# uzh-rpg/dagr

Hardware: NVIDIA H100
Metric: Mevents/sec (higher is better)
Workload: dtype f32

## Files before the change

dagr_b200/_lib.py:

```python
from __future__ import annotations

import ctypes as C
import os
from pathlib import Path

import torch

_PKG = Path(__file__).resolve().parent
_LIB_PATH = Path(os.environ["DAGR_B200_LIB"]) if os.environ.get("DAGR_B200_LIB") else _PKG / "libdagr_b200.so"
_lib = None

ELL = 16
KU = 15
TABW = 16
L1_TC_WFRAG_FLOATS = 8192

p = C.c_void_p
i32 = C.c_int32
i64 = C.c_int64
f32 = C.c_float


class Geom(C.Structure):
    _fields_ = [("W", i32), ("H", i32), ("B", i32), ("T", i32),
                ("r", i32), ("ncell", i32),
                ("dt_us", i32), ("K", i32), ("Q", i32),
                ("nx1", i32), ("ny1", i32),
                ("CW", i32), ("CH", i32), ("CP", i32),
                ("NK", i32),
                ("xkey", p), ("ykey", p), ("spiral", p), ("posx0", p), ("posy0", p), ("vx0", p), ("vy0", p), ("tabx", p), ("taby", p)]


class Grid(C.Structure):
    _fields_ = [("nx", i32), ("ny", i32), ("B", i32), ("W", i32), ("H", i32),
                ("posxr", p), ("posyr", p)]


class EventWs(C.Structure):
    _fields_ = [(k, i64) for k in ("key", "tmp", "count", "blocksums", "start", "perm", "ti", "xyb", "feat_s", "nbr", "off", "cellmask",
                                   "xa", "wl_hdr", "wl_ids", "x1")]


class PoolWs(C.Structure):
    _fields_ = [(k, i64) for k in ("acc", "possum", "ptmax", "pcnt", "pmask")]


class L1AParams(C.Structure):
    _fields_ = [("w", f32 * (KU * 3 * 16)), ("root", f32 * (3 * 16)),
                ("scale", f32 * 16), ("shift", f32 * 16), ("relu", i32)]


class L1ImgParams(C.Structure):
    _fields_ = [("w", f32 * (KU * 24 * 16)), ("root", f32 * (24 * 16)), ("skip", f32 * (24 * 16)),
                ("scale", f32 * 16), ("shift", f32 * 16), ("sscale", f32 * 16), ("sshift", f32 * 16), ("relu", i32)]


class L1BParams(C.Structure):
    _fields_ = [("w", f32 * (KU * 16 * 16)), ("root", f32 * (16 * 16)), ("skip", f32 * (3 * 16)),
                ("scale", f32 * 16), ("shift", f32 * 16), ("sscale", f32 * 16), ("sshift", f32 * 16),
                ("relu", i32), ("pool_mean", i32), ("xs", i32 * 3), ("ys", i32 * 5), ("den_x", f32), ("den_y", f32)]


_SIGS = {
    "dagr_abi_version": (C.c_int, []),
    "dagr_last_error": (C.c_char_p, []),
    "dagr_scan_blocks": (i64, [i64]),
    "dagr_check_config": (C.c_int, [C.POINTER(Geom), i64, C.c_int, C.c_int, C.c_char_p]),
    "dagr_event_workspace_bytes": (C.c_int, [C.POINTER(Geom), i64, C.POINTER(EventWs)]),
    "dagr_pool_workspace_bytes": (C.c_int, [i64, C.c_int, C.POINTER(PoolWs)]),
    "dagr_downsample_events": (C.c_int, [p, p, p, i64, C.c_int, C.c_int, C.c_int, C.c_int, p, p, p, p, p, p, p, p, p]),
    "dagr_compact_events": (C.c_int, [p, i64, p, p, p, p, C.c_int, C.c_int, p, p, p, p, p, p, p, p, p]),
    "dagr_ingest_events": (C.c_int, [p, p, p, p, i64, C.c_int, C.c_int, C.c_int, C.c_int, i64, C.c_int, p, p, p, p, p, p, p, p, p]),
    "dagr_denormalize_pos": (C.c_int, [p, i64, C.c_int, C.c_int, C.c_int, p, p]),
    "dagr_prepare_events": (C.c_int, [p, p, p, C.c_int, i64, C.c_int, C.c_int, C.c_int, p, p, p, p]),
    "dagr_graph_sort": (C.c_int, [C.POINTER(Geom), p, p, p, i64, p, p, p, p, p, p, p, p, p, p, p]),
    "dagr_graph_sort_ring": (C.c_int, [C.POINTER(Geom), p, p, p, i64, p, p, p, p, p, p, p, p, p, p, p, p]),
    "dagr_stream_push": (C.c_int, [p, p, p, p, p, i64, C.c_int, C.c_int, p]),
    "dagr_stream_push_multi": (C.c_int, [p, p, p, p, p, i64, C.c_int, C.c_int, p]),
    "dagr_graph_sort_rings": (C.c_int, [C.POINTER(Geom), p, p, p, i64, C.c_int, p, p, p, p, p, p, p, p, p, p, p, p]),
    "dagr_graph_search": (C.c_int, [C.POINTER(Geom), i64, p, p, p, p, p, p, p]),
    "dagr_l1_build": (C.c_int, [C.POINTER(Geom), i64, p, p, p, p, p, C.POINTER(L1AParams), p, C.c_int, p, p, p, p, p, p, C.c_int, p]),
    "dagr_xa_permute": (C.c_int, [i64, p, C.c_int, p, p, C.c_int, p]),
    "dagr_l1_x0_image": (C.c_int, [C.POINTER(Geom), i64, p, p, p, C.c_int, C.c_int, p, p]),
    "dagr_l1_x0_image_live": (C.c_int, [C.POINTER(Geom), i64, p, p, p, p, C.c_int, C.c_int, p, p]),
    "dagr_l1_x0_image_planes": (C.c_int, [C.POINTER(Geom), i64, p, p, p, p, C.c_int, C.c_int, C.c_int, p, C.c_int, p, p]),
    "dagr_l1_conv_a_image": (C.c_int, [C.POINTER(Geom), i64, p, p, p, p, p, p, C.POINTER(L1ImgParams), p, p, p, p, C.c_int, p]),
    "dagr_voxel_sample_max": (C.c_int, [C.POINTER(Geom), i64, p, p, p, C.c_int, C.c_int, C.c_int, p, C.c_int, C.c_int, C.c_int, p]),
    "dagr_voxel_sample_max_planes": (C.c_int, [C.POINTER(Geom), i64, p, p, p, C.c_int, C.c_int, C.c_int, C.c_int, p, C.c_int, p, C.c_int,
                                               C.c_int, C.c_int, p]),
    "dagr_graph_export": (C.c_int, [C.POINTER(Geom), i64, p, p, p, p, p, p, p, p, i64, p]),
    "dagr_l1_conv_a": (C.c_int, [C.POINTER(Geom), i64, p, p, p, p, p, C.POINTER(L1AParams), p, p]),
    "dagr_l1_conv_b_pool": (C.c_int, [C.POINTER(Geom), i64, p, p, p, p, p, p, C.POINTER(L1BParams), p, p, p]),
    "dagr_l1_conv_b_pool_voxel": (C.c_int, [C.POINTER(Geom), i64, p, p, p, p, p, p, p, p, C.POINTER(L1BParams), p, C.c_int, p, p, p, p, p, p, p, C.c_int, p, p, C.c_int, p]),
    "dagr_l1_tc_weights": (C.c_int, [p, p, C.c_int, p]),
    "dagr_l1_conv_b_pool_voxel_tc": (C.c_int, [C.POINTER(Geom), i64, p, p, p, p, p, p, p, C.POINTER(L1BParams), p, p, C.c_int, p, p, p, p, p, p, p, C.c_int, p, p, C.c_int, p]),
    "dagr_l1_conv_a_image_tc": (C.c_int, [C.POINTER(Geom), i64, p, p, p, p, p, p, C.POINTER(L1ImgParams), p, p, p, p, p, C.c_int, p]),
    "dagr_l1_conv_a_image_inc": (C.c_int, [C.POINTER(Geom), i64, p, p, p, p, p, p, p, C.POINTER(L1ImgParams), p, C.c_int, p, p, p, p,
                                           C.c_int, p]),
    "dagr_voxel_sample_max_inc": (C.c_int, [C.POINTER(Geom), i64, p, p, p, p, C.c_int, C.c_int, C.c_int, C.c_int, p, p, C.c_int, C.c_int,
                                            C.c_int, p]),
    "dagr_pool1_finalize": (C.c_int, [C.POINTER(Geom), i64, p, p, p, p, C.c_int, p, p, p, p, p, p]),
    "dagr_grid_cat_pos": (C.c_int, [C.POINTER(Grid), p, p, p, C.c_int, p, p]),
    "dagr_grid_conv": (C.c_int, [C.POINTER(Grid), p, p, p, p, C.c_int, C.c_int, C.c_int, p, p, p, p, p, p, C.c_int, f32, f32, p, p]),
    "dagr_grid_linear_bn": (C.c_int, [i64, p, p, C.c_int, C.c_int, p, p, p, p, p]),
    "dagr_grid_pool": (C.c_int, [C.POINTER(Grid), C.POINTER(Grid), p, p, p, p, p, p, p, p, C.c_int, C.c_int,
                                 p, p, p, p, p, p, p, p]),
    "dagr_grid_pool_finalize": (C.c_int, [C.POINTER(Grid), C.c_int, C.c_int, p, p, p, p, p, p, p, p, p, p]),
    "dagr_grid_temporal_filter": (C.c_int, [C.POINTER(Grid), p, p, p, p]),
    "dagr_grid_to_dense": (C.c_int, [C.POINTER(Grid), p, p, C.c_int, C.c_int, p, p, p]),
    "dagr_head_decode": (C.c_int, [p, p, p, C.c_int, C.c_int, C.c_int, C.c_int, C.c_int, C.c_int, C.c_int, p, p]),
    "dagr_head_finish": (C.c_int, [C.POINTER(Grid), p, p, C.c_int, p, C.c_int, p, p, p, C.c_int, C.c_int, C.c_int, C.c_int, p, p]),
    "dagr_head_finish_planes": (C.c_int, [C.POINTER(Grid), p, p, C.c_int, p, C.c_int, p, p, p, C.c_int, C.c_int, C.c_int, C.c_int,
                                          C.c_int, p, C.c_int, p, p]),
    "dagr_postprocess_nms": (C.c_int, [p, C.c_int, C.c_int, C.c_int, f32, f32, C.c_int, C.c_int, C.c_int, p, p, p]),
    "dagr_sample_features": (C.c_int, [p, C.c_int, C.c_int, C.c_int, C.c_int, p, p, p, i64, C.c_int, C.c_int, p,
                                       C.c_int, C.c_int, p]),
    "dagr_sample_features_planes": (C.c_int, [p, C.c_int, p, C.c_int, C.c_int, C.c_int, C.c_int, p, p, p, i64, C.c_int, C.c_int, p,
                                              C.c_int, C.c_int, p]),
    "dagr_masked_lin": (C.c_int, [p, i64, p, p, p, p, C.c_int, C.c_int, C.c_int, p]),
    "dagr_masked_inplace_bn": (C.c_int, [p, i64, p, p, p, p, p, p, C.c_int, f32, p]),
    "dagr_masked_isdiff": (C.c_int, [p, i64, p, p, C.c_int, f32, f32, p]),
}

EXPORTS = tuple(_SIGS.keys())


def lib_path() -> Path:
    return _LIB_PATH


def load():
    global _lib
    if _lib is not None:
        return _lib
    if not os.environ.get("DAGR_B200_LIB"):
        from . import build as _build
        if _build.needs_build():
            try:
                _build.build(force=True)
            except Exception as e:
                if not _LIB_PATH.exists():
                    raise RuntimeError(f"dagr_b200: could not build the CUDA extension: {e}") from e
                import warnings
                warnings.warn(f"dagr_b200: libdagr_b200.so is older than its sources and could not be rebuilt ({e})")
    if not _LIB_PATH.exists():
        raise RuntimeError(f"dagr_b200: CUDA extension {_LIB_PATH} is missing and could not be built; "
                           "there is no CPU fallback")
    lib = C.CDLL(str(_LIB_PATH))
    for name, (res, args) in _SIGS.items():
        fn = getattr(lib, name)
        fn.restype = res
        fn.argtypes = args
    if lib.dagr_abi_version() != 2:
        raise RuntimeError("dagr_b200: ABI version mismatch between python host and libdagr_b200.so")
    _lib = lib
    return lib


def check(code: int, what: str = ""):
    if code != 0:
        msg = load().dagr_last_error()
        raise RuntimeError(f"dagr_b200 {what} failed ({code}): {msg.decode() if msg else ''}")


def ptr(t):
    if t is None:
        return None
    return C.c_void_p(t.data_ptr())


def stream_ptr():
    return C.c_void_p(torch.cuda.current_stream().cuda_stream)


def require_cuda(t: torch.Tensor, name: str):
    if not t.is_cuda:
        raise RuntimeError(f"dagr_b200: `{name}` must be a CUDA tensor (no CPU fallback on the product path)")
    if not t.is_contiguous():
        raise RuntimeError(f"dagr_b200: `{name}` must be contiguous")
```

dagr_b200/csrc/build_l1.cu:

```cuda
#include <type_traits>
#include "common.cuh"

#define BL_THREADS 160
#define BL_CAP 2048
#define BL_CAP_LEAN 1536
#define BL_THREADS_BIG 512
#define BL_CAP_BIG 12288
#define BL_NB 8

struct BLTile {
    int X0, Y0, TW, TH;
    int run_start[3], run_off[3], run_len[3];
    int smin, smax;
    int unsorted;
    int bucketed;
    int maxidx;
};

__host__ __device__ __forceinline__ size_t bl_acc_offset(const dagr_geom_t &g, int cap)
{
    const size_t TW = g.CW + 2 * g.r, TH = g.CH + 2 * g.r, TP = TW * TH;
    const size_t o = (size_t)(2 * g.r + 1) * 32 + (size_t)cap * 12 + TP * 4 + (TW + TH) * 4 + TP * BL_NB * 2 + (size_t)g.ncell * 4;
    return (o + 15) / 16 * 16;
}
static size_t bl_smem_bytes(const dagr_geom_t *g, int cap, int threads)
{
    const size_t TW = g->CW + 2 * g->r, TH = g->CH + 2 * g->r;
    const size_t occ = (size_t)BL_NB * (TW + TH) * 4, order = (size_t)threads * 2;
    return bl_acc_offset(*g, cap) + (size_t)(DAGR_ELL - 1) * threads * 4 + (occ > order ? occ : order) + 16;
}

#define BL_R1 96

template <bool STAGED, int THREADS>
__device__ __forceinline__ void bl_probe(const dagr_geom_t &g, int64_t N, int p, bool active, const int2 me, int eb, int tidx0,
                                         int c_end, const uint32_t *s_pbin, const uint16_t *s_rng, const short *s_sp2,
                                         const int2 *s_ti, const int2 *__restrict__ ti, uint32_t *s_acc,
                                         int32_t *__restrict__ nbr, uint16_t *__restrict__ off, int &n_out)
{
    const int kmax = g.K - 1;
    int n = active ? 0 : kmax;
    for (int c0 = 0; c0 < c_end; c0 += 4) {
        if (__all_sync(0xffffffffu, n >= kmax)) break;
        uint32_t rg[4]; int pix[4];
#pragma unroll
        for (int u = 0; u < 4; u++) {
            const int c = min(c0 + u, g.ncell - 1);
            pix[u] = tidx0 + s_sp2[c];
        }
#pragma unroll
        for (int u = 0; u < 4; u++) rg[u] = s_rng[pix[u] * BL_NB + eb];
#pragma unroll
        for (int u = 0; u < 4; u++) {
            const int c = c0 + u;
            const int lo = rg[u] & 0xff, hi = rg[u] >> 8;
            const int cnt = (c < c_end && n < kmax) ? hi - lo : 0;
            if (!__any_sync(0xffffffffu, cnt > 0)) continue;
            const int base = (int)(s_pbin[pix[u]] >> 8);
            const int vmax = __reduce_max_sync(0xffffffffu, cnt);
            for (int k = 0; k < vmax; k++) {
                if (k < cnt && n < kmax) {
                    const int j = base + hi - 1 - k;
                    const int2 o = STAGED ? s_ti[j] : __ldg(ti + j);
                    if (o.y < me.y && me.x - o.x <= g.dt_us) {
                        if (STAGED) s_acc[n * THREADS + threadIdx.x] = ((uint32_t)j << 10) | (uint32_t)c;
                        else { nbr[(int64_t)n * N + p] = j; off[(int64_t)n * N + p] = (uint16_t)c; }
                        n++;
                    }
                }
            }
        }
    }
    n_out = active ? n : 0;
}


#ifndef BL_SHARED_ADDR
#define BL_SHARED_ADDR 1
#endif
__device__ __forceinline__ uint32_t bl_sa(const void *p) { return (uint32_t)__cvta_generic_to_shared(p); }
__device__ __forceinline__ uint32_t bl_lds32(uint32_t a) { uint32_t v; asm volatile("ld.shared.u32 %0, [%1];" : "=r"(v) : "r"(a) : "memory"); return v; }
__device__ __forceinline__ uint32_t bl_lds16(uint32_t a) { uint32_t v; asm volatile("{ .reg .u16 t; ld.shared.u16 t, [%1]; cvt.u32.u16 %0, t; }" : "=r"(v) : "r"(a) : "memory"); return v; }
__device__ __forceinline__ int bl_lds16s(uint32_t a) { int v; asm volatile("{ .reg .s16 t; ld.shared.s16 t, [%1]; cvt.s32.s16 %0, t; }" : "=r"(v) : "r"(a) : "memory"); return v; }
__device__ __forceinline__ int2 bl_lds64(uint32_t a) { int2 v; asm volatile("ld.shared.v2.s32 {%0, %1}, [%2];" : "=r"(v.x), "=r"(v.y) : "r"(a) : "memory"); return v; }
#ifndef BL_FAST_TABLES
#define BL_FAST_TABLES 1
#endif
__device__ __forceinline__ int bl_div(int t, int d, float inv)
{
#if BL_FAST_TABLES
    if ((unsigned)t >= (1u << 24)) return t / d;
    int q = (int)((float)t * inv);
    const int r = t - q * d;
    if (r < 0) q--; else if (r >= d) q++;
    return q;
#else
    (void)inv;
    return t / d;
#endif
}
__device__ __forceinline__ void bl_sts32(uint32_t a, uint32_t v) { asm volatile("st.shared.u32 [%0], %1;" :: "r"(a), "r"(v) : "memory"); }

template <bool STAGED, int THREADS>
__device__ __forceinline__ void bl_probe_rings(const dagr_geom_t &g, int64_t N, int p, bool active, const int2 me, int eb, int tx0, int ty0,
                                               int TW, int TH, const uint32_t *s_pbin, const uint16_t *s_rng, const uint32_t *s_occ_r,
                                               const uint32_t *s_occ_c, const short *s_sp2, const int2 *s_ti, const int2 *__restrict__ ti, uint32_t *s_acc,
                                               int32_t *__restrict__ nbr, uint16_t *__restrict__ off, int &n_out)
{
    const int kmax = g.K - 1;
    int n = active ? 0 : kmax;
    const uint32_t *occr = s_occ_r + eb * TH, *occc = s_occ_c + eb * TW;
    constexpr bool SA = STAGED && BL_SHARED_ADDR;
    const uint32_t a_rng = bl_sa(s_rng) + 2u * (uint32_t)eb, a_pbin = bl_sa(s_pbin), a_ti = bl_sa(s_ti), a_sp2 = bl_sa(s_sp2);
    const uint32_t a_acc = bl_sa(s_acc) + 4u * threadIdx.x;
    const int dt_us = g.dt_us;
    auto visit = [&](int pix, int c) {
        const uint32_t rg = SA ? bl_lds16(a_rng + (uint32_t)pix * (2u * BL_NB)) : (uint32_t)s_rng[pix * BL_NB + eb];
        const int lo = rg & 0xff, hi = rg >> 8;
        const int base = (int)((SA ? bl_lds32(a_pbin + 4u * (uint32_t)pix) : s_pbin[pix]) >> 8);
        for (int j = base + hi - 1; j >= base + lo && n < kmax; j--) {
            const int2 o = SA ? bl_lds64(a_ti + 8u * (uint32_t)j) : (STAGED ? s_ti[j] : __ldg(ti + j));
            if (o.y < me.y && me.x - o.x <= dt_us) {
                if (SA) bl_sts32(a_acc + (uint32_t)n * (4u * THREADS), ((uint32_t)j << 10) | (uint32_t)c);
                else if (STAGED) s_acc[n * THREADS + threadIdx.x] = ((uint32_t)j << 10) | (uint32_t)c;
                else { nbr[(int64_t)n * N + p] = j; off[(int64_t)n * N + p] = (uint16_t)c; }
                n++;
            }
        }
    };
    if (n < kmax && ((occr[ty0] >> tx0) & 1u)) visit(ty0 * TW + tx0, 0);
    const int tidx0 = ty0 * TW + tx0;
    for (int d = 1; d <= g.r; d++) {
        if (__all_sync(0xffffffffu, n >= kmax)) break;
        const int l2 = 2 * d;
        const uint32_t fm = (l2 >= 32) ? 0xffffffffu : ((1u << l2) - 1u);
        const int cbase = (l2 - 1) * (l2 - 1);
        uint32_t lo = 0, hi = 0;
        if (n < kmax) {
            const uint32_t leg0 = (occc[tx0 + d] >> (ty0 - d + 1)) & fm;
            const uint32_t leg1 = __brev((occr[ty0 + d] >> (tx0 - d)) & fm) >> (32 - l2);
            const uint32_t leg2 = __brev((occc[tx0 - d] >> (ty0 - d)) & fm) >> (32 - l2);
            const uint32_t leg3 = (occr[ty0 - d] >> (tx0 - d + 1)) & fm;
            const unsigned long long m = (unsigned long long)leg0 | ((unsigned long long)leg1 << l2) |
                                         ((unsigned long long)leg2 << (2 * l2)) | ((unsigned long long)leg3 << (3 * l2));
            lo = (uint32_t)m; hi = (uint32_t)(m >> 32);
        }
        while (lo | hi) {
            int i;
            if (lo) { i = __ffs((int)lo) - 1; lo &= lo - 1; }
            else    { i = 32 + __ffs((int)hi) - 1; hi &= hi - 1; }
            visit(tidx0 + (SA ? bl_lds16s(a_sp2 + 2u * (uint32_t)(cbase + i)) : (int)s_sp2[cbase + i]), cbase + i);
            if (n >= kmax) { lo = 0; hi = 0; }
        }
    }
    n_out = active ? n : 0;
}

template <bool STAGED, int THREADS>
__device__ __forceinline__ int bl_probe_coop(const dagr_geom_t &g, int64_t N, int p, const int2 me, int eb, int tidx0, int c_begin,
                                             int n, const uint32_t *s_pbin, const uint16_t *s_rng, const short *s_sp2,
                                             const int2 *s_ti, const int2 *__restrict__ ti, uint32_t *s_acc, int owner,
                                             int32_t *__restrict__ nbr, uint16_t *__restrict__ off)
{
    const int kmax = g.K - 1;
    const int lane = threadIdx.x & 31;
    for (int c0 = c_begin; c0 < g.ncell && n < kmax; c0 += 32) {
        const int c = c0 + lane;
        int cnt = 0, base = 0, hi = 0, acc = 0;
        if (c < g.ncell) {
            const int pix = tidx0 + s_sp2[c];
            const uint32_t rg = s_rng[pix * BL_NB + eb];
            hi = rg >> 8; cnt = hi - (int)(rg & 0xff);
            base = (int)(s_pbin[pix] >> 8);
            for (int k = 0; k < cnt; k++) {
                const int2 o = STAGED ? s_ti[base + hi - 1 - k] : __ldg(ti + base + hi - 1 - k);
                acc += (o.y < me.y && me.x - o.x <= g.dt_us) ? 1 : 0;
            }
        }
        int incl = acc;
#pragma unroll
        for (int d = 1; d < 32; d <<= 1) { const int v = __shfl_up_sync(0xffffffffu, incl, d); if (lane >= d) incl += v; }
        const int tot = __shfl_sync(0xffffffffu, incl, 31);
        if (acc > 0) {
            int slot = n + incl - acc;
            for (int k = 0; k < cnt && slot < kmax; k++) {
                const int j = base + hi - 1 - k;
                const int2 o = STAGED ? s_ti[j] : __ldg(ti + j);
                if (o.y < me.y && me.x - o.x <= g.dt_us) {
                    if (STAGED) s_acc[slot * THREADS + owner] = ((uint32_t)j << 10) | (uint32_t)c;
                    else { nbr[(int64_t)slot * N + p] = j; off[(int64_t)slot * N + p] = (uint16_t)c; }
                    slot++;
                }
            }
        }
        n = min(n + tot, kmax);
    }
    return n;
}

template <int CAP, int THREADS>
__device__ __forceinline__ void bl_voxel(const dagr_geom_t &g, int64_t N, const int32_t *__restrict__ start, const int2 *__restrict__ ti,
                                         const uint32_t *__restrict__ xyb, const float *__restrict__ feat_s,
                                         const dagr_l1a_params_t &P, const int do_conv, const int min_idx, const int32_t *__restrict__ flags,
                                         int32_t *__restrict__ nbr, uint16_t *__restrict__ off, uint32_t *__restrict__ cellmask,
                                         float *__restrict__ xa, const int cell, unsigned char *smem_raw, BLTile &T, uint32_t &s_mask,
                                         int32_t *__restrict__ wl_hdr, int32_t *__restrict__ wl_ids, const int defer)
{
    const int per = g.ny1 * g.nx1;
    const int b = cell / per, rem = cell % per, cy = rem / g.nx1, cx = rem % g.nx1;
    const int p0 = start[(int64_t)cell * g.CP], p1 = start[(int64_t)(cell + 1) * g.CP];
    if (p1 == p0) { if (threadIdx.x == 0 && min_idx <= 0) cellmask[cell] = 0; return; }

    const int TWmax = g.CW + 2 * g.r, THmax = g.CH + 2 * g.r, TPmax = TWmax * THmax, R = 2 * g.r + 1;
    float4 *s_wy = (float4 *)smem_raw;
    float *s_wx = (float *)(s_wy + R);
    float *s_wy4 = s_wx + 3 * R;
    int2 *s_ti = (int2 *)(s_wy4 + R);
    float *s_feat = (float *)(s_ti + CAP);
    uint16_t *s_rng = (uint16_t *)(s_feat + CAP);
    uint32_t *s_pbin = (uint32_t *)(s_rng + TPmax * BL_NB);
    float *s_posx = (float *)(s_pbin + TPmax);
    float *s_posy = s_posx + TWmax;
    uint16_t *s_sp = (uint16_t *)(s_posy + THmax);
    short *s_sp2 = (short *)(s_sp + g.ncell);
    uint32_t *s_acc = (uint32_t *)(smem_raw + bl_acc_offset(g, CAP));
    uint32_t *s_occ_r = s_acc + (DAGR_ELL - 1) * THREADS;
    uint16_t *s_order = (uint16_t *)s_occ_r;

    const int dtw = max(g.dt_us, 1);
    const float dtw_inv = 1.0f / (float)dtw;
    if (threadIdx.x == 0) {
        const int X0 = g.vx0[cx], X1 = g.vx0[cx + 1], Y0 = g.vy0[cy], Y1 = g.vy0[cy + 1];
        T.X0 = X0 - g.r; T.Y0 = Y0 - g.r; T.TW = X1 - X0 + 2 * g.r; T.TH = Y1 - Y0 + 2 * g.r;
        const int clo = max(cx - 1, 0), chi = min(cx + 1, g.nx1 - 1);
        int o = 0;
        for (int rr = 0; rr < 3; rr++) {
            const int ry = cy - 1 + rr;
            if (ry < 0 || ry >= g.ny1) { T.run_start[rr] = 0; T.run_len[rr] = 0; T.run_off[rr] = o; continue; }
            const int64_t c0 = (int64_t)b * per + ry * g.nx1 + clo, c1 = (int64_t)b * per + ry * g.nx1 + chi + 1;
            const int s = start[c0 * g.CP], e = start[c1 * g.CP];
            T.run_start[rr] = s; T.run_len[rr] = e - s; T.run_off[rr] = o;
            o += e - s;
        }
        T.smin = 0x7fffffff; T.smax = -0x7fffffff; T.unsorted = 0; T.maxidx = -1;
        s_mask = 0;
    }
    __syncthreads();
    const int TW = T.TW, TH = T.TH, TP = TW * TH;
    const bool use_rings = TW <= 32 && TH <= 32 && g.r <= 8;
    uint32_t *s_occ_c = s_occ_r + BL_NB * TH;
    const int total = T.run_off[2] + T.run_len[2];
    const bool staged = total <= CAP;
    if (!staged && wl_hdr != nullptr) {
        int slot = 0;
        if (threadIdx.x == 0) slot = atomicAdd(&wl_hdr[0], 1);
        if (defer) { if (threadIdx.x == 0) wl_ids[slot] = cell; return; }
    }
    const int bbase = b * per * g.CP;

    for (int i = threadIdx.x; i < g.ncell; i += blockDim.x) {
        const int dx = g.spiral[2 * i], dy = g.spiral[2 * i + 1];
        s_sp[i] = (uint16_t)((dx + g.r) | ((dy + g.r) << 5));
        s_sp2[i] = (short)(dy * TW + dx);
    }
    for (int i = threadIdx.x; i < R; i += blockDim.x) {
        const float4 tx = __ldg(reinterpret_cast<const float4 *>(g.tabx) + i);
        s_wx[i] = tx.x; s_wx[R + i] = tx.y; s_wx[2 * R + i] = tx.z;
        s_wy[i] = __ldg(reinterpret_cast<const float4 *>(g.taby) + 2 * i);
        s_wy4[i] = __ldg(g.taby + 8 * i + 4);
    }
    for (int i = threadIdx.x; i < TW; i += blockDim.x) {
        const int gx = T.X0 + i;
        s_posx[i] = (gx >= 0 && gx < g.W) ? g.posx0[gx] : 0.f;
    }
    for (int i = threadIdx.x; i < TH; i += blockDim.x) {
        const int gy = T.Y0 + i;
        s_posy[i] = (gy >= 0 && gy < g.H) ? g.posy0[gy] : 0.f;
    }
    for (int i = threadIdx.x; i < TP; i += blockDim.x) {
        const int ty = i / TW, tx = i % TW;
        const int gx = T.X0 + tx, gy = T.Y0 + ty;
        uint32_t v = 0;
        if (gx >= 0 && gx < g.W && gy >= 0 && gy < g.H) {
            const int ky = g.ykey[gy], kx = g.xkey[gx];
            const int k = bbase + ky + kx;
            const int s = start[k], e = start[k + 1];
            if (e > s) {
                const int lo = max(s, e - g.Q);
                const int rr = ky / (g.nx1 * g.CP) - cy + 1;
                const int pos = staged ? (lo - T.run_start[rr] + T.run_off[rr]) : lo;
                v = ((uint32_t)pos << 8) | (uint32_t)(e - lo);
            }
        }
        s_pbin[i] = v;
    }
    if (staged) {
        for (int rr = 0; rr < 3; rr++) {
            const int s = T.run_start[rr], o = T.run_off[rr], len = T.run_len[rr];
            for (int i = threadIdx.x; i < len; i += blockDim.x) {
                s_ti[o + i] = ti[s + i];
                s_feat[o + i] = feat_s[s + i];
            }
        }
    }
    if (use_rings)
        for (int i = threadIdx.x; i < BL_NB * TW; i += blockDim.x) s_occ_c[i] = 0;
    {
        int mn = 0x7fffffff, mx = -0x7fffffff, mi = -1;
        for (int p = p0 + threadIdx.x; p < p1; p += blockDim.x) {
            const int2 r = ti[p];
            if (r.y < min_idx) continue;
            const int sl = bl_div(r.x, dtw, dtw_inv); mn = min(mn, sl); mx = max(mx, sl); mi = max(mi, r.y);
        }
        mn = __reduce_min_sync(0xffffffffu, mn); mx = __reduce_max_sync(0xffffffffu, mx); mi = __reduce_max_sync(0xffffffffu, mi);
        if ((threadIdx.x & 31) == 0) { atomicMin(&T.smin, mn); atomicMax(&T.smax, mx); atomicMax(&T.maxidx, mi); }
    }
    __syncthreads();
    if (T.maxidx < 0) return;
    const int sbase = T.smin - 1;
    bool bucketed = staged && (T.smax - sbase) < BL_NB && (flags == nullptr || flags[0] == 0);
    auto pixel_ranges = [&](int i) -> uint32_t {
        const uint32_t pb = s_pbin[i];
        const int vis = pb & 0xff, base = pb >> 8;
        unsigned char cum[BL_NB + 1];
#pragma unroll
        for (int q = 0; q <= BL_NB; q++) cum[q] = 0;
        if (bucketed) {
            int prev = 0;
            for (int k = 0; k < vis; k++) {
                int bk = bl_div(s_ti[base + k].x, dtw, dtw_inv) - sbase;
                bk = min(max(bk, 0), BL_NB - 1);
                if (bk < prev) T.unsorted = 1;
                prev = bk;
#pragma unroll
                for (int q = 0; q <= BL_NB; q++) cum[q] += (bk < q) ? 1 : 0;
            }
        } else {
#pragma unroll
            for (int q = 1; q <= BL_NB; q++) cum[q] = (unsigned char)vis;
        }
        static_assert(BL_NB == 8, "one uint4 per pixel");
        uint32_t w[4], occ = 0;
#pragma unroll
        for (int e = 0; e < BL_NB; e += 2) {
            const uint32_t r0 = (uint32_t)cum[e > 0 ? e - 1 : 0] | ((uint32_t)cum[e + 1] << 8);
            const uint32_t r1 = (uint32_t)cum[e] | ((uint32_t)cum[e + 2] << 8);
            w[e >> 1] = r0 | (r1 << 16);
            occ |= (cum[e + 1] > cum[e > 0 ? e - 1 : 0] ? 1u : 0u) << e;
            occ |= (cum[e + 2] > cum[e] ? 1u : 0u) << (e + 1);
        }
        reinterpret_cast<uint4 *>(s_rng)[i] = make_uint4(w[0], w[1], w[2], w[3]);
        return occ;
    };
    for (int pass = 0; pass < 2; pass++) {
        if (use_rings) {
            const int lane = threadIdx.x & 31;
            uint32_t colm[BL_NB];
#pragma unroll
            for (int e = 0; e < BL_NB; e++) colm[e] = 0;
            for (int row = threadIdx.x >> 5; row < TH; row += blockDim.x >> 5) {
                const uint32_t occ = lane < TW ? pixel_ranges(row * TW + lane) : 0u;
#pragma unroll
                for (int e = 0; e < BL_NB; e++) {
                    const uint32_t m = __ballot_sync(0xffffffffu, (occ >> e) & 1u);
                    if (lane == e) s_occ_r[e * TH + row] = m;
                    colm[e] |= ((occ >> e) & 1u) << row;
                }
            }
            if (lane < TW) {
#pragma unroll
                for (int e = 0; e < BL_NB; e++)
                    if (colm[e]) atomicOr(&s_occ_c[e * TW + lane], colm[e]);
            }
        } else {
            for (int i = threadIdx.x; i < TP; i += blockDim.x) pixel_ranges(i);
        }
        __syncthreads();
        if (!bucketed || !T.unsorted) break;
        bucketed = false;
        if (use_rings) {
            for (int i = threadIdx.x; i < BL_NB * TW; i += blockDim.x) s_occ_c[i] = 0;
            __syncthreads();
        }
    }
    if (threadIdx.x == 0) T.bucketed = bucketed;
    uint32_t mloc = 0;
    for (int pb = p0; pb < p1; pb += blockDim.x) {
        const int chunk = min((int)blockDim.x, p1 - pb);
        __syncthreads();
        if (!use_rings && (int)threadIdx.x < chunk) {
            const int d = T.run_off[1] - T.run_start[1];
            const int myidx = staged ? s_ti[d + pb + threadIdx.x].y : ti[pb + threadIdx.x].y;
            int rank = 0;
            for (int k = 0; k < chunk; k++) {
                const int oi = staged ? s_ti[d + pb + k].y : __ldg(&ti[pb + k].y);
                rank += (oi < myidx) ? 1 : 0;
            }
            s_order[rank] = (uint16_t)threadIdx.x;
        }
        __syncthreads();
        const int nw = blockDim.x >> 5;
        const int rank = use_rings ? (int)threadIdx.x : (int)(threadIdx.x & 31) * nw + (int)(threadIdx.x >> 5);
        bool active = rank < chunk;
        const int p = pb + (active ? (use_rings ? rank : (int)s_order[rank]) : 0);
        int x = 0, y = 0;
        int2 me = make_int2(0, 0);
        if (active) {
            const uint32_t w = xyb[p];
            x = w & 0xfff; y = (w >> 12) & 0xfff;
            me = ti[p];
            active = me.y >= min_idx;
        }
        const int tx0 = active ? x - T.X0 : g.r, ty0 = active ? y - T.Y0 : g.r;
        int eb = 0;
        if (T.bucketed) eb = min(max(bl_div(me.x, dtw, dtw_inv) - sbase, 0), BL_NB - 1);
        int n;
        const int tidx0 = ty0 * TW + tx0;
        if (use_rings) {
            if (staged) bl_probe_rings<true, THREADS>(g, N, p, active, me, eb, tx0, ty0, TW, TH, s_pbin, s_rng, s_occ_r, s_occ_c, s_sp2, s_ti, ti, s_acc, nbr, off, n);
            else        bl_probe_rings<false, THREADS>(g, N, p, active, me, eb, tx0, ty0, TW, TH, s_pbin, s_rng, s_occ_r, s_occ_c, s_sp2, s_ti, ti, s_acc, nbr, off, n);
        } else {
            if (staged) bl_probe<true, THREADS>(g, N, p, active, me, eb, tidx0, BL_R1 < g.ncell ? BL_R1 : g.ncell, s_pbin, s_rng, s_sp2, s_ti, ti, s_acc, nbr, off, n);
            else        bl_probe<false, THREADS>(g, N, p, active, me, eb, tidx0, BL_R1 < g.ncell ? BL_R1 : g.ncell, s_pbin, s_rng, s_sp2, s_ti, ti, s_acc, nbr, off, n);
            if (BL_R1 < g.ncell) {
                unsigned todo = __ballot_sync(0xffffffffu, active && n < g.K - 1);
                while (todo) {
                    const int src = __ffs(todo) - 1;
                    todo &= todo - 1;
                    const int ep = __shfl_sync(0xffffffffu, p, src);
                    const int2 eme = make_int2(__shfl_sync(0xffffffffu, me.x, src), __shfl_sync(0xffffffffu, me.y, src));
                    const int eeb = __shfl_sync(0xffffffffu, eb, src), etidx = __shfl_sync(0xffffffffu, tidx0, src);
                    const int en = __shfl_sync(0xffffffffu, n, src);
                    const int owner = (int)(threadIdx.x & ~31u) + src;
                    const int nn = staged ? bl_probe_coop<true, THREADS>(g, N, ep, eme, eeb, etidx, BL_R1, en, s_pbin, s_rng, s_sp2, s_ti, ti, s_acc, owner, nbr, off)
                                          : bl_probe_coop<false, THREADS>(g, N, ep, eme, eeb, etidx, BL_R1, en, s_pbin, s_rng, s_sp2, s_ti, ti, s_acc, owner, nbr, off);
                    if ((int)(threadIdx.x & 31) == src) n = nn;
                }
                __syncwarp();
            }
        }
        if (active) nbr[(int64_t)(DAGR_ELL - 1) * N + p] = n;
        const float f0 = active ? feat_s[p] : 0.f, f1 = s_posx[tx0], f2 = s_posy[ty0];
        float A[DAGR_KU][3];
        {
            const int o = g.r;
            const float4 wya = s_wy[o];
            const float wy[5] = {wya.x, wya.y, wya.z, wya.w, s_wy4[o]}, wx[3] = {s_wx[o], s_wx[R + o], s_wx[2 * R + o]};
#pragma unroll
            for (int jy = 0; jy < 5; jy++)
#pragma unroll
                for (int k = 0; k < 3; k++) {
                    const float t = __fmul_rn(wy[jy], wx[k]);
                    A[k + 3 * jy][0] = t * f0; A[k + 3 * jy][1] = t * f1; A[k + 3 * jy][2] = t * f2;
                }
        }
        int txy = (tx0 - g.r) | ((ty0 - g.r) << 16);
        auto edges = [&](auto staged_c) {
            constexpr bool ST = decltype(staged_c)::value;
            for (int q = 0; q < n; q++) {
                const uint32_t e = (uint32_t)q * (uint32_t)N + (uint32_t)p;
                int j, c;
                if (ST) { const uint32_t a = s_acc[q * THREADS + threadIdx.x]; j = (int)(a >> 10); c = (int)(a & 0x3ff); }
                else { j = nbr[e]; c = off[e]; }
                const uint32_t sp = s_sp[c];
                const int dxi = (int)(sp & 31u), dyi = (int)(sp >> 5);
                const int txy_e = txy + dxi + (dyi << 16);
                const int tx = txy_e & 0xffff, ty = txy_e >> 16;
                const int vr = (ty >= g.r) + (ty + g.r >= TH), vc = (tx >= g.r) + (tx + g.r >= TW);
                float e0;
                if (ST) {
                    e0 = s_feat[j];
                    nbr[e] = j - T.run_off[vr] + T.run_start[vr];
                    off[e] = (uint16_t)c;
                } else e0 = __ldg(feat_s + j);
                mloc |= 1u << (vr * 3 + vc);
                const float e1 = s_posx[tx], e2 = s_posy[ty];
                const float4 wya = s_wy[dyi];
                const float wy[5] = {wya.x, wya.y, wya.z, wya.w, s_wy4[dyi]}, wx[3] = {s_wx[dxi], s_wx[R + dxi], s_wx[2 * R + dxi]};
#pragma unroll
                for (int jy = 0; jy < 5; jy++)
#pragma unroll
                    for (int k = 0; k < 3; k++) {
                        const int u = k + 3 * jy;
                        const float t = __fmul_rn(wy[jy], wx[k]);
                        A[u][0] = fmaf(t, e0, A[u][0]);
                        A[u][1] = fmaf(t, e1, A[u][1]);
                        A[u][2] = fmaf(t, e2, A[u][2]);
                    }
            }
        };
        if (staged) edges(std::true_type{});
        else        edges(std::false_type{});

        if (!active || !do_conv) continue;
        int pr = p;
        asm volatile("" : "+r"(txy), "+r"(pr));
        const float r0 = __ldg(feat_s + pr), r1 = s_posx[(txy & 0xffff) + g.r], r2 = s_posy[(txy >> 16) + g.r];
        float o[16];
#pragma unroll
        for (int k = 0; k < 16; k++) o[k] = 0.f;
#pragma unroll
        for (int u = 0; u < DAGR_KU; u++)
#pragma unroll
            for (int ci = 0; ci < 3; ci++)
#pragma unroll
                for (int k = 0; k < 16; k++) o[k] = fmaf(A[u][ci], P.w[u][ci][k], o[k]);
#pragma unroll
        for (int k = 0; k < 16; k++) {
            float r = o[k];
            r = fmaf(r0, P.root[0][k], r);
            r = fmaf(r1, P.root[1][k], r);
            r = fmaf(r2, P.root[2][k], r);
            r = fmaf(r, P.scale[k], P.shift[k]);
            o[k] = P.relu ? fmaxf(r, 0.f) : r;
        }
        const int sw = XA_SWZ(p);
        float4 *dst = reinterpret_cast<float4 *>(xa + (int64_t)p * 8);
        dst[sw] = make_float4(o[0], o[1], o[2], o[3]);
        dst[sw ^ 1] = make_float4(o[4], o[5], o[6], o[7]);
        dst = reinterpret_cast<float4 *>(xa + (N + (int64_t)p) * 8);
        dst[sw] = make_float4(o[8], o[9], o[10], o[11]);
        dst[sw ^ 1] = make_float4(o[12], o[13], o[14], o[15]);
    }
    mloc = __reduce_or_sync(0xffffffffu, mloc) & ~(1u << 4);
    if ((threadIdx.x & 31) == 0 && mloc) atomicOr(&s_mask, mloc);
    __syncthreads();
    if (threadIdx.x == 0) cellmask[cell] = (min_idx > 0 ? cellmask[cell] : 0u) | s_mask;
}



template <int CAP, int MIN_CTAS>
__global__ void __launch_bounds__(BL_THREADS, MIN_CTAS)
k_l1_build(const dagr_geom_t g, int64_t N, const int32_t *__restrict__ start, const int2 *__restrict__ ti,
           const uint32_t *__restrict__ xyb, const float *__restrict__ feat_s,
           const __grid_constant__ dagr_l1a_params_t P, const int do_conv, const int min_idx, const int32_t *__restrict__ flags,
           int32_t *__restrict__ nbr, uint16_t *__restrict__ off, uint32_t *__restrict__ cellmask, float *__restrict__ xa,
           int32_t *__restrict__ wl_hdr, int32_t *__restrict__ wl_ids, const int defer)
{
    extern __shared__ __align__(16) unsigned char smem_raw[];
    __shared__ BLTile T;
    __shared__ uint32_t s_mask;
    bl_voxel<CAP, BL_THREADS>(g, N, start, ti, xyb, feat_s, P, do_conv, min_idx, flags, nbr, off, cellmask, xa,
                              (int)blockIdx.x, smem_raw, T, s_mask, wl_hdr, wl_ids, defer);
}

__global__ void __launch_bounds__(BL_THREADS_BIG, 1)
k_l1_build_dense(const dagr_geom_t g, int64_t N, const int32_t *__restrict__ start, const int2 *__restrict__ ti,
                 const uint32_t *__restrict__ xyb, const float *__restrict__ feat_s,
                 const __grid_constant__ dagr_l1a_params_t P, const int do_conv, const int min_idx, const int32_t *__restrict__ flags,
                 int32_t *__restrict__ nbr, uint16_t *__restrict__ off, uint32_t *__restrict__ cellmask, float *__restrict__ xa,
                 int32_t *__restrict__ wl_hdr, const int32_t *__restrict__ wl_ids)
{
    extern __shared__ __align__(16) unsigned char smem_raw[];
    __shared__ BLTile T;
    __shared__ uint32_t s_mask;
    __shared__ int s_next;
    const int count = wl_hdr[0];
    for (;;) {
        __syncthreads();
        if (threadIdx.x == 0) s_next = atomicAdd(&wl_hdr[1], 1);
        __syncthreads();
        const int i = s_next;
        if (i >= count) break;
        bl_voxel<BL_CAP_BIG, BL_THREADS_BIG>(g, N, start, ti, xyb, feat_s, P, do_conv, min_idx, flags, nbr, off, cellmask, xa,
                                             wl_ids[i], smem_raw, T, s_mask, nullptr, nullptr, 0);
    }
}

extern "C" int dagr_l1_build(const dagr_geom_t *g, int64_t N, const int32_t *start, const int32_t *ti,
                             const uint32_t *xyb, const float *feat_s, const float *tab,
                             const dagr_l1a_params_t *p_host, const int32_t *flags, int min_idx, int32_t *nbr, uint16_t *off,
                             uint32_t *cellmask, float *xa, int32_t *wl_hdr, int32_t *wl_ids, int defer, void *stream)
{
    DAGR_CHECK_ARG(g, "null argument");
    (void)tab;
    static const dagr_l1a_params_t zero_params = {};
    const int do_conv = p_host != nullptr;
    if (!p_host) p_host = &zero_params;
    DAGR_CHECK_ARG(g->K >= 1 && g->K <= DAGR_ELL, "max_neighbors must be in [1,16]");
    DAGR_CHECK_ARG(g->r >= 0 && g->r <= 15 && g->Q <= 255, "radius must be <= 15 px and max_queue_size <= 255");
    DAGR_CHECK_ARG(N < (1ll << 24), "the staged probe packs positions in 24 bits (N < 16.7M per call)");
    const int cells = g->B * g->ny1 * g->nx1;
    const bool deferring = wl_hdr != nullptr && wl_ids != nullptr && defer;
    if (deferring) {
        const size_t smem = bl_smem_bytes(g, BL_CAP, BL_THREADS);
        auto kern = k_l1_build<BL_CAP, 4>;
        DAGR_CUDA(dagr_allow_smem(kern, smem, true));
        kern<<<cells, BL_THREADS, smem, (cudaStream_t)stream>>>(*g, N, start, (const int2 *)ti, xyb, feat_s, *p_host, do_conv, min_idx,
                                                                flags, nbr, off, cellmask, xa, wl_hdr, wl_ids, 1);
    } else {
        const size_t smem = bl_smem_bytes(g, BL_CAP_LEAN, BL_THREADS);
        auto kern = k_l1_build<BL_CAP_LEAN, 5>;
        DAGR_CUDA(dagr_allow_smem(kern, smem, true));
        kern<<<cells, BL_THREADS, smem, (cudaStream_t)stream>>>(*g, N, start, (const int2 *)ti, xyb, feat_s, *p_host, do_conv, min_idx,
                                                                flags, nbr, off, cellmask, xa, wl_hdr, wl_ids, 0);
    }
    DAGR_CHECK_LAUNCH();
    if (deferring) {
        const size_t smem_big = bl_smem_bytes(g, BL_CAP_BIG, BL_THREADS_BIG);
        static int n_sm = 0;
        if (n_sm == 0) {
            int dev = 0;
            DAGR_CUDA(cudaGetDevice(&dev));
            DAGR_CUDA(cudaDeviceGetAttribute(&n_sm, cudaDevAttrMultiProcessorCount, dev));
        }
        DAGR_CUDA(dagr_allow_smem(k_l1_build_dense, smem_big));
        k_l1_build_dense<<<n_sm, BL_THREADS_BIG, smem_big, (cudaStream_t)stream>>>(*g, N, start, (const int2 *)ti, xyb, feat_s,
                                                                                    *p_host, do_conv, min_idx, flags, nbr, off,
                                                                                    cellmask, xa, wl_hdr, wl_ids);
        DAGR_CHECK_LAUNCH();
    }
    return DAGR_OK;
}
```

dagr_b200/csrc/common.cuh:

```cuda
#pragma once
#include <cuda_runtime.h>
#include <stdint.h>
#include <stdio.h>
#include "../../include/dagr_b200.h"

#ifndef __CUDA_ARCH__
#define DAGR_HOST 1
#endif

void dagr_set_error(const char *fmt, ...);

#define DAGR_CHECK_ARG(cond, msg)                                              \
    do { if (!(cond)) { dagr_set_error("%s: %s", __func__, msg); return DAGR_E_ARG; } } while (0)

#define DAGR_CHECK_LAUNCH()                                                    \
    do { cudaError_t e__ = cudaGetLastError();                                 \
         if (e__ != cudaSuccess) { dagr_set_error("%s: %s", __func__, cudaGetErrorString(e__)); \
                                   return DAGR_E_CUDA; } } while (0)

#define DAGR_CUDA(call)                                                        \
    do { cudaError_t e__ = (call);                                             \
         if (e__ != cudaSuccess) { dagr_set_error("%s: %s", __func__, cudaGetErrorString(e__)); \
                                   return DAGR_E_CUDA; } } while (0)

cudaError_t dagr_allow_smem_impl(const void *kernel, size_t bytes, bool max_carveout);
template <class K> static inline cudaError_t dagr_allow_smem(K kernel, size_t bytes, bool max_carveout = false)
{
    return dagr_allow_smem_impl(reinterpret_cast<const void *>(kernel), bytes, max_carveout);
}

static inline int dagr_div_up(int64_t a, int64_t b) { return (int)((a + b - 1) / b); }

struct ImgPlanes {
    const int32_t *plane;
    int stride, n;
};
__device__ __forceinline__ int img_plane(const ImgPlanes &pl, int b)
{
    return min(max(__ldg(pl.plane + (int64_t)b * pl.stride), 0), pl.n - 1);
}

int scan_exclusive(const int *in, int *out, int64_t n, int *blocksums, cudaStream_t st);

#define XA_SWZ(p) ((int)(((p) >> 2) & 1))

__device__ __forceinline__ uint32_t enc_ordered(float f)
{
    uint32_t u = __float_as_uint(f);
    return (u & 0x80000000u) ? ~u : (u | 0x80000000u);
}
__device__ __forceinline__ float dec_ordered(uint32_t e)
{
    uint32_t u = (e & 0x80000000u) ? (e & 0x7fffffffu) : ~e;
    return __uint_as_float(u);
}

__device__ __forceinline__ float2 ffma2(float2 a, float2 b, float2 c) { return make_float2(fmaf(a.x, b.x, c.x), fmaf(a.y, b.y, c.y)); }

__device__ __forceinline__ void spline_basis2(float ax, float ay, int ks, float w[4], int slot[4])
{
    float vx = ax * (float)(ks - 1), vy = ay * (float)(ks - 1);
    float fx = vx - floorf(vx), fy = vy - floorf(vy);
    int ix = (int)vx, iy = (int)vy;
#pragma unroll
    for (int s = 0; s < 4; s++) {
        int kx = s & 1, ky = (s >> 1) & 1;
        int sx = (ix + kx) % ks, sy = (iy + ky) % ks;
        if (sx < 0) sx += ks;
        if (sy < 0) sy += ks;
        slot[s] = sx + ks * sy;
        w[s] = (kx ? fx : 1.f - fx) * (ky ? fy : 1.f - fy);
    }
}
```

dagr_b200/csrc/conv_l1.cu:

```cuda
#include <string.h>
#include "common.cuh"

#define L1_THREADS 128

struct L1Smem {
    float *tab;
    float *posx;
    float *posy;
    short *sp;
};

__device__ __forceinline__ L1Smem l1_smem_init(const dagr_geom_t &g, const float *__restrict__ tab, unsigned char *raw)
{
    L1Smem s;
    s.tab = (float *)raw;
    s.posx = s.tab + g.ncell * DAGR_TABW;
    s.posy = s.posx + g.W;
    s.sp = (short *)(s.posy + g.H);
    for (int i = threadIdx.x; i < g.ncell * DAGR_TABW; i += blockDim.x) s.tab[i] = tab[i];
    for (int i = threadIdx.x; i < g.W; i += blockDim.x) s.posx[i] = g.posx0[i];
    for (int i = threadIdx.x; i < g.H; i += blockDim.x) s.posy[i] = g.posy0[i];
    for (int i = threadIdx.x; i < g.ncell; i += blockDim.x)
        s.sp[i] = (short)(((int)g.spiral[2 * i] & 0xff) | ((int)g.spiral[2 * i + 1] << 8));
    __syncthreads();
    return s;
}

static size_t l1_smem_bytes(const dagr_geom_t *g)
{
    return (size_t)g->ncell * DAGR_TABW * 4 + (size_t)(g->W + g->H) * 4 + (size_t)g->ncell * 2 + 16;
}

__device__ __forceinline__ void load_tab(const float *row, float w[DAGR_KU])
{
    static_assert(DAGR_KU == 15 && DAGR_TABW == 16, "table row layout");
    const float4 a = *reinterpret_cast<const float4 *>(row);
    const float4 b = *reinterpret_cast<const float4 *>(row + 4);
    const float4 c = *reinterpret_cast<const float4 *>(row + 8);
    const float4 d = *reinterpret_cast<const float4 *>(row + 12);
    w[0] = a.x; w[1] = a.y; w[2] = a.z; w[3] = a.w;
    w[4] = b.x; w[5] = b.y; w[6] = b.z; w[7] = b.w;
    w[8] = c.x; w[9] = c.y; w[10] = c.z; w[11] = c.w;
    w[12] = d.x; w[13] = d.y; w[14] = d.z;
}

__global__ void __launch_bounds__(L1_THREADS)
k_l1_conv_a(const dagr_geom_t g, int64_t N, const uint32_t *__restrict__ xyb, const float *__restrict__ feat_s,
            const int32_t *__restrict__ nbr, const uint16_t *__restrict__ off, const float *__restrict__ tab,
            const __grid_constant__ dagr_l1a_params_t P, float *__restrict__ xa)
{
    extern __shared__ __align__(16) unsigned char smem_raw[];
    const L1Smem s = l1_smem_init(g, tab, smem_raw);
    const int64_t p = (int64_t)blockIdx.x * blockDim.x + threadIdx.x;
    if (p >= N) return;

    const uint32_t w = xyb[p];
    const int x = w & 0xfff, y = (w >> 12) & 0xfff;
    const float f0 = feat_s[p], f1 = s.posx[x], f2 = s.posy[y];
    const int n = nbr[(int64_t)(DAGR_ELL - 1) * N + p];

    float A[DAGR_KU][3];
    {
        float t[DAGR_KU];
        load_tab(s.tab, t);
#pragma unroll
        for (int u = 0; u < DAGR_KU; u++) { A[u][0] = t[u] * f0; A[u][1] = t[u] * f1; A[u][2] = t[u] * f2; }
    }
    for (int q = 0; q < n; q++) {
        const int j = nbr[(int64_t)q * N + p];
        const int c = off[(int64_t)q * N + p];
        const int sp = s.sp[c];
        const float e0 = __ldg(feat_s + j);
        const float e1 = s.posx[x + (int)(signed char)(sp & 0xff)];
        const float e2 = s.posy[y + (sp >> 8)];
        float t[DAGR_KU];
        load_tab(s.tab + c * DAGR_TABW, t);
#pragma unroll
        for (int u = 0; u < DAGR_KU; u++) {
            A[u][0] = fmaf(t[u], e0, A[u][0]);
            A[u][1] = fmaf(t[u], e1, A[u][1]);
            A[u][2] = fmaf(t[u], e2, A[u][2]);
        }
    }
    float o[16];
#pragma unroll
    for (int k = 0; k < 16; k++) o[k] = 0.f;
#pragma unroll
    for (int u = 0; u < DAGR_KU; u++)
#pragma unroll
        for (int ci = 0; ci < 3; ci++)
#pragma unroll
            for (int k = 0; k < 16; k++) o[k] = fmaf(A[u][ci], P.w[u][ci][k], o[k]);
#pragma unroll
    for (int k = 0; k < 16; k++) {
        float r = o[k];
        r = fmaf(f0, P.root[0][k], r);
        r = fmaf(f1, P.root[1][k], r);
        r = fmaf(f2, P.root[2][k], r);
        r = fmaf(r, P.scale[k], P.shift[k]);
        o[k] = P.relu ? fmaxf(r, 0.f) : r;
    }
    const int sw = XA_SWZ(p);
    float4 *dst = reinterpret_cast<float4 *>(xa + p * 8);
    dst[sw] = make_float4(o[0], o[1], o[2], o[3]);
    dst[sw ^ 1] = make_float4(o[4], o[5], o[6], o[7]);
    dst = reinterpret_cast<float4 *>(xa + (N + p) * 8);
    dst[sw] = make_float4(o[8], o[9], o[10], o[11]);
    dst[sw ^ 1] = make_float4(o[12], o[13], o[14], o[15]);
}

extern "C" int dagr_l1_conv_a(const dagr_geom_t *g, int64_t N, const uint32_t *xyb, const float *feat_s,
                              const int32_t *nbr, const uint16_t *off, const float *tab,
                              const dagr_l1a_params_t *p_host, float *xa, void *stream)
{
    DAGR_CHECK_ARG(g && p_host, "null argument");
    if (N <= 0) return DAGR_OK;
    size_t smem = l1_smem_bytes(g);
    DAGR_CUDA(dagr_allow_smem(k_l1_conv_a, smem));
    k_l1_conv_a<<<dagr_div_up(N, L1_THREADS), L1_THREADS, smem, (cudaStream_t)stream>>>(
        *g, N, xyb, feat_s, nbr, off, tab, *p_host, xa);
    DAGR_CHECK_LAUNCH();
    return DAGR_OK;
}

__global__ void __launch_bounds__(L1_THREADS)
k_l1_conv_b(const dagr_geom_t g, int64_t N, const uint32_t *__restrict__ xyb, const float *__restrict__ feat_s,
            const float *__restrict__ xa, const int32_t *__restrict__ nbr, const uint16_t *__restrict__ off,
            const float *__restrict__ tab, const __grid_constant__ dagr_l1b_params_t P,
            float *__restrict__ x1, uint32_t *__restrict__ poolmax)
{
    extern __shared__ __align__(16) unsigned char smem_raw[];
    const L1Smem s = l1_smem_init(g, tab, smem_raw);
    const int64_t p = (int64_t)blockIdx.x * blockDim.x + threadIdx.x;
    const bool active = p < N;
    float o[16];
#pragma unroll
    for (int k = 0; k < 16; k++) o[k] = 0.f;
    int cell = -1;
    if (active) {
        const uint32_t w = xyb[p];
        const int x = w & 0xfff, y = (w >> 12) & 0xfff, b = w >> 24;
        cell = b * (g.ny1 * g.nx1) + (__ldg(g.ykey + y) / (g.nx1 * g.CP)) * g.nx1 + __ldg(g.xkey + x) / g.CP;
        const int n = nbr[(int64_t)(DAGR_ELL - 1) * N + p];

#pragma unroll 1
        for (int half = 0; half < 2; half++) {
            float2 A[DAGR_KU][4];
            {
                const float4 *src = reinterpret_cast<const float4 *>(xa + ((int64_t)half * N + p) * 8);
                const float4 t0 = src[XA_SWZ(p)], t1 = src[XA_SWZ(p) ^ 1];
                const float2 v[4] = {make_float2(t0.x, t0.y), make_float2(t0.z, t0.w), make_float2(t1.x, t1.y), make_float2(t1.z, t1.w)};
                float t[DAGR_KU];
                load_tab(s.tab, t);
#pragma unroll
                for (int u = 0; u < DAGR_KU; u++)
#pragma unroll
                    for (int k = 0; k < 4; k++) A[u][k] = make_float2(t[u] * v[k].x, t[u] * v[k].y);
                if (half == 0) {
#pragma unroll
                    for (int k = 0; k < 4; k++)
#pragma unroll
                        for (int c = 0; c < 16; c++) {
                            o[c] = fmaf(v[k].x, P.root[2 * k][c], o[c]);
                            o[c] = fmaf(v[k].y, P.root[2 * k + 1][c], o[c]);
                        }
                } else {
#pragma unroll
                    for (int k = 0; k < 4; k++)
#pragma unroll
                        for (int c = 0; c < 16; c++) {
                            o[c] = fmaf(v[k].x, P.root[8 + 2 * k][c], o[c]);
                            o[c] = fmaf(v[k].y, P.root[8 + 2 * k + 1][c], o[c]);
                        }
                }
            }
            for (int q = 0; q < n; q++) {
                const int j = nbr[(int64_t)q * N + p];
                const int c = off[(int64_t)q * N + p];
                const float4 *src = reinterpret_cast<const float4 *>(xa + ((int64_t)half * N + j) * 8);
                const float4 t0 = __ldg(src + XA_SWZ(j)), t1 = __ldg(src + (XA_SWZ(j) ^ 1));
                const float2 e[4] = {make_float2(t0.x, t0.y), make_float2(t0.z, t0.w), make_float2(t1.x, t1.y), make_float2(t1.z, t1.w)};
                float t[DAGR_KU];
                load_tab(s.tab + c * DAGR_TABW, t);
#pragma unroll
                for (int u = 0; u < DAGR_KU; u++) {
                    const float2 tt = make_float2(t[u], t[u]);
#pragma unroll
                    for (int k = 0; k < 4; k++) A[u][k] = ffma2(tt, e[k], A[u][k]);
                }
            }
            if (half == 0) {
#pragma unroll
                for (int u = 0; u < DAGR_KU; u++)
#pragma unroll
                    for (int k = 0; k < 4; k++)
#pragma unroll
                        for (int c = 0; c < 16; c++) {
                            o[c] = fmaf(A[u][k].x, P.w[u][2 * k][c], o[c]);
                            o[c] = fmaf(A[u][k].y, P.w[u][2 * k + 1][c], o[c]);
                        }
            } else {
#pragma unroll
                for (int u = 0; u < DAGR_KU; u++)
#pragma unroll
                    for (int k = 0; k < 4; k++)
#pragma unroll
                        for (int c = 0; c < 16; c++) {
                            o[c] = fmaf(A[u][k].x, P.w[u][8 + 2 * k][c], o[c]);
                            o[c] = fmaf(A[u][k].y, P.w[u][8 + 2 * k + 1][c], o[c]);
                        }
            }
        }
        const float f0 = feat_s[p], f1 = s.posx[x], f2 = s.posy[y];
#pragma unroll
        for (int c = 0; c < 16; c++) {
            float sk = f0 * P.skip[0][c];
            sk = fmaf(f1, P.skip[1][c], sk);
            sk = fmaf(f2, P.skip[2][c], sk);
            sk = fmaf(sk, P.sscale[c], P.sshift[c]);
            float r = fmaf(o[c], P.scale[c], P.shift[c]) + sk;
            o[c] = P.relu ? fmaxf(r, 0.f) : r;
        }
        if (x1 != nullptr) {
            float4 *dst = reinterpret_cast<float4 *>(x1 + p * 16);
            dst[0] = make_float4(o[0], o[1], o[2], o[3]);
            dst[1] = make_float4(o[4], o[5], o[6], o[7]);
            dst[2] = make_float4(o[8], o[9], o[10], o[11]);
            dst[3] = make_float4(o[12], o[13], o[14], o[15]);
        }
    }
    if (poolmax != nullptr) {
        const int lane = threadIdx.x & 31;
        uint32_t eo[16];
#pragma unroll
        for (int c = 0; c < 16; c++) eo[c] = active ? enc_ordered(o[c]) : 0u;
#pragma unroll
        for (int d = 1; d < 32; d <<= 1) {
            const int oc = __shfl_down_sync(0xffffffffu, cell, d);
            const bool take = (lane + d < 32) && (oc == cell);
#pragma unroll
            for (int c = 0; c < 16; c++) {
                const uint32_t ov = __shfl_down_sync(0xffffffffu, eo[c], d);
                if (take) eo[c] = max(eo[c], ov);
            }
        }
        const int pc = __shfl_up_sync(0xffffffffu, cell, 1);
        const bool head = active && (lane == 0 || pc != cell);
        if (head) {
            uint32_t *dst = poolmax + (int64_t)cell * 16;
#pragma unroll
            for (int c = 0; c < 16; c++) atomicMax(dst + c, eo[c]);
        }
    }
}

extern "C" int dagr_l1_conv_b_pool(const dagr_geom_t *g, int64_t N, const uint32_t *xyb, const float *feat_s,
                                   const float *xa, const int32_t *nbr, const uint16_t *off, const float *tab,
                                   const dagr_l1b_params_t *p_host, float *x1, uint32_t *poolmax, void *stream)
{
    DAGR_CHECK_ARG(g && p_host, "null argument");
    DAGR_CHECK_ARG(p_host->pool_mean == 0, "mean pooling needs the per-voxel kernel (dagr_l1_conv_b_pool_voxel)");
    if (N <= 0) return DAGR_OK;
    size_t smem = l1_smem_bytes(g);
    DAGR_CUDA(dagr_allow_smem(k_l1_conv_b, smem));
    k_l1_conv_b<<<dagr_div_up(N, L1_THREADS), L1_THREADS, smem, (cudaStream_t)stream>>>(
        *g, N, xyb, feat_s, xa, nbr, off, tab, *p_host, x1, poolmax);
    DAGR_CHECK_LAUNCH();
    return DAGR_OK;
}

#define CB2_THREADS 160
#define CB2_CAP 1344
#define CB2_THREADS_BIG 384
#define CB2_CAP_BIG 6144
static_assert(2 * CB2_CAP_BIG <= 16384, "the ELL word keeps 2*row+swizzle in 14 bits");
#define CB2_G 5

__device__ __forceinline__ uint32_t smem_u32(const void *p) { return (uint32_t)__cvta_generic_to_shared(p); }

__device__ __forceinline__ void mbar_init(uint64_t *bar, int count)
{
    asm volatile("mbarrier.init.shared::cta.b64 [%0], %1;" ::"r"(smem_u32(bar)), "r"(count));
    asm volatile("fence.mbarrier_init.release.cluster;" ::: "memory");
}
__device__ __forceinline__ void mbar_expect_tx(uint64_t *bar, uint32_t bytes)
{
    asm volatile("mbarrier.arrive.expect_tx.shared::cta.b64 _, [%0], %1;" ::"r"(smem_u32(bar)), "r"(bytes) : "memory");
}
__device__ __forceinline__ void mbar_wait(uint64_t *bar, uint32_t parity)
{
    asm volatile(
        "{\n"
        ".reg .pred p;\n"
        "WAIT_%=:\n"
        "mbarrier.try_wait.parity.shared::cta.b64 p, [%0], %1;\n"
        "@p bra DONE_%=;\n"
        "bra WAIT_%=;\n"
        "DONE_%=:\n"
        "}\n" ::"r"(smem_u32(bar)), "r"(parity) : "memory");
}
__device__ __forceinline__ void tma_bulk_g2s(void *dst_smem, const void *src_gmem, uint32_t bytes, uint64_t *bar)
{
    asm volatile("cp.async.bulk.shared::cluster.global.mbarrier::complete_tx::bytes [%0], [%1], %2, [%3];" ::"r"(smem_u32(dst_smem)),
                 "l"(src_gmem), "r"(bytes), "r"(smem_u32(bar))
                 : "memory");
}

struct CB2Tile {
    int run_start[3], run_len[3], run_off[3];
};

#ifndef CB2_TC
#define CB2_TC 1
#endif
#define CB2_TC_KSTEPS 16

__device__ __forceinline__ uint32_t tf32_rna(float x)
{
    uint32_t r;
    asm("cvt.rna.tf32.f32 %0, %1;" : "=r"(r) : "f"(x));
    return r;
}
__device__ __forceinline__ void mma_tf32(float2 &c01, float2 &c23, const uint32_t a[4], uint32_t b0, uint32_t b1)
{
    asm("mma.sync.aligned.m16n8k8.row.col.f32.tf32.tf32.f32 {%0, %1, %2, %3}, {%4, %5, %6, %7}, {%8, %9}, {%0, %1, %2, %3};"
        : "+f"(c01.x), "+f"(c01.y), "+f"(c23.x), "+f"(c23.y)
        : "r"(a[0]), "r"(a[1]), "r"(a[2]), "r"(a[3]), "r"(b0), "r"(b1));
}

__device__ __forceinline__ void cb2_tc_kstep(float *xt, const float a[8], const float4 *__restrict__ wf, float2 o2[8])
{
    const int lane = threadIdx.x & 31;
    const float4 w0 = __ldg(wf), w1 = __ldg(wf + 1);
    const uint32_t bh[2][2] = {{__float_as_uint(w0.x), __float_as_uint(w0.y)}, {__float_as_uint(w1.x), __float_as_uint(w1.y)}};
    const uint32_t bl[2][2] = {{__float_as_uint(w0.z), __float_as_uint(w0.w)}, {__float_as_uint(w1.z), __float_as_uint(w1.w)}};
    float *row = xt + 4 * (lane & 15);
    const uint32_t ra = smem_u32(row);
#pragma unroll
    for (int mt = 0; mt < 2; mt++) {
        uint32_t ah[4], al[4];
#pragma unroll
        for (int h = 0; h < 2; h++) {
            __syncwarp();
            if ((lane >> 4) == mt) *reinterpret_cast<float4 *>(row) = make_float4(a[4 * h], a[4 * h + 1], a[4 * h + 2], a[4 * h + 3]);
            __syncwarp();
            uint32_t r0, r1;
            asm volatile("ldmatrix.sync.aligned.m8n8.x2.shared.b16 {%0, %1}, [%2];" : "=r"(r0), "=r"(r1) : "r"(ra) : "memory");
            ah[2 * h] = tf32_rna(__uint_as_float(r0));
            ah[2 * h + 1] = tf32_rna(__uint_as_float(r1));
            al[2 * h] = __float_as_uint(__uint_as_float(r0) - __uint_as_float(ah[2 * h]));
            al[2 * h + 1] = __float_as_uint(__uint_as_float(r1) - __uint_as_float(ah[2 * h + 1]));
        }
        const uint32_t fa[4] = {ah[0], ah[1], ah[2], ah[3]}, fl[4] = {al[0], al[1], al[2], al[3]};
#pragma unroll
        for (int nt = 0; nt < 2; nt++) {
            mma_tf32(o2[4 * mt + 2 * nt], o2[4 * mt + 2 * nt + 1], fl, bh[nt][0], bh[nt][1]);
            mma_tf32(o2[4 * mt + 2 * nt], o2[4 * mt + 2 * nt + 1], fa, bl[nt][0], bl[nt][1]);
            mma_tf32(o2[4 * mt + 2 * nt], o2[4 * mt + 2 * nt + 1], fa, bh[nt][0], bh[nt][1]);
        }
    }
}

__device__ __forceinline__ void cb2_tc_unfrag(float *xt, float2 o2[8])
{
    const int lane = threadIdx.x & 31, g = lane >> 2, t = lane & 3;
    float2 r[8];
#pragma unroll
    for (int mt = 0; mt < 2; mt++)
#pragma unroll
        for (int q = 0; q < 4; q++) {
            __syncwarp();
            if ((t >> 1) == (q & 1)) {
                *reinterpret_cast<float2 *>(xt + 4 * g + 2 * (t & 1)) = o2[4 * mt + 2 * (q >> 1)];
                *reinterpret_cast<float2 *>(xt + 4 * (g + 8) + 2 * (t & 1)) = o2[4 * mt + 2 * (q >> 1) + 1];
            }
            __syncwarp();
            const float4 v = *reinterpret_cast<const float4 *>(xt + 4 * (lane & 15));
            if ((lane >> 4) == mt) { r[2 * q] = make_float2(v.x, v.y); r[2 * q + 1] = make_float2(v.z, v.w); }
        }
#pragma unroll
    for (int c = 0; c < 8; c++) o2[c] = r[c];
}

template <bool STAGED, int half, int grp, int THREADS, bool TC, class PT>
__device__ __forceinline__ void cb2_pass(int64_t N, int p, int n, const float *__restrict__ xa, const float *s_rows,
                                         const float *s_wx, const float4 *s_wy, const float *s_wy4, const uint32_t *s_ell, const uint16_t *s_sp,
                                         const int32_t *__restrict__ nbr, const uint16_t *__restrict__ off,
                                         const PT &P, const float4 *__restrict__ wfrag, float *xt, int own_row, int r, int tix, float2 o2[8])
{
    float2 A[CB2_G][4];
#pragma unroll
    for (int u = 0; u < CB2_G; u++)
#pragma unroll
        for (int k = 0; k < 4; k++) A[u][k] = make_float2(0.f, 0.f);
#define CB2_EDGE_FMA()                                                                                              \
    do {                                                                                                            \
        const float2 e[4] = {make_float2(t0.x, t0.y), make_float2(t0.z, t0.w), make_float2(t1.x, t1.y), make_float2(t1.z, t1.w)}; \
        const float wy[CB2_G] = {wya.x, wya.y, wya.z, wya.w, wy4};                                                  \
        _Pragma("unroll") for (int j = 0; j < CB2_G; j++) {                                                         \
            const float w = __fmul_rn(wy[j], wx);               \
            const float2 tt = make_float2(w, w);                                                                    \
            _Pragma("unroll") for (int k = 0; k < 4; k++) A[j][k] = ffma2(tt, e[k], A[j][k]);                       \
        }                                                                                                           \
    } while (0)
    if constexpr (STAGED) {
        const char *rb = reinterpret_cast<const char *>(s_rows);
        const char *wxb = reinterpret_cast<const char *>(s_wx) + 128 * grp, *wyb = reinterpret_cast<const char *>(s_wy);
        const char *wy4b = reinterpret_cast<const char *>(s_wy4);
#ifndef CB2_UNROLL
#define CB2_UNROLL 1
#endif
        constexpr int kUnroll = CB2_UNROLL;
#pragma unroll kUnroll
        for (int q = 0; q <= n; q++) {
            const uint32_t ell = s_ell[q * THREADS + tix];
            const uint32_t ro = ell & 0x3fff0u, xo = (ell >> 16) & 0x7cu, yo = (ell >> 19) & 0x1f0u;
            const float4 t0 = *reinterpret_cast<const float4 *>(rb + ro), t1 = *reinterpret_cast<const float4 *>(rb + (ro ^ 16u));
            const float wx = *reinterpret_cast<const float *>(wxb + xo);
            const float4 wya = *reinterpret_cast<const float4 *>(wyb + yo);
            const float wy4 = *reinterpret_cast<const float *>(wy4b + (yo >> 2));
            CB2_EDGE_FMA();
        }
    } else {
#pragma unroll 1
        for (int q = -1; q < n; q++) {
            int row, dxi, dyi;
            if (q < 0) { row = p; dxi = r; dyi = r; }
            else {
                row = nbr[(int64_t)q * N + p];
                const uint32_t d = s_sp[off[(int64_t)q * N + p]];
                dxi = (int)(d & 31u); dyi = (int)(d >> 5);
            }
            const int sw = XA_SWZ(row);
            const float4 *src = reinterpret_cast<const float4 *>(xa + ((int64_t)half * N + row) * 8);
            const float4 t0 = src[sw], t1 = src[sw ^ 1];
            const float wx = s_wx[grp * 32 + dxi];
            const float4 wya = s_wy[dyi];
            const float wy4 = s_wy4[dyi];
            CB2_EDGE_FMA();
        }
    }
#undef CB2_EDGE_FMA
    if constexpr (TC) {
        const float4 *wf = wfrag + ((size_t)half * CB2_TC_KSTEPS * 32 + (threadIdx.x & 31)) * 2;
        float2 c2[8];
#pragma unroll
        for (int i = 0; i < 8; i++) c2[i] = make_float2(0.f, 0.f);
#pragma unroll
        for (int j = 0; j < CB2_G; j++) {
            const float a[8] = {A[j][0].x, A[j][0].y, A[j][1].x, A[j][1].y, A[j][2].x, A[j][2].y, A[j][3].x, A[j][3].y};
            cb2_tc_kstep(xt, a, wf + (grp + 3 * j) * 64, c2);
        }
#pragma unroll
        for (int i = 0; i < 8; i++) o2[i] = make_float2(__fadd_rn(o2[i].x, c2[i].x), __fadd_rn(o2[i].y, c2[i].y));
        return;
    }
#pragma unroll
    for (int j = 0; j < CB2_G; j++)
#pragma unroll
        for (int k = 0; k < 4; k++)
#pragma unroll
            for (int c4 = 0; c4 < 4; c4++) {
                const float4 wa = *reinterpret_cast<const float4 *>(&P.w[grp + 3 * j][8 * half + 2 * k][4 * c4]);
                const float4 wb = *reinterpret_cast<const float4 *>(&P.w[grp + 3 * j][8 * half + 2 * k + 1][4 * c4]);
                o2[2 * c4] = ffma2(make_float2(A[j][k].x, A[j][k].x), make_float2(wa.x, wa.y), o2[2 * c4]);
                o2[2 * c4 + 1] = ffma2(make_float2(A[j][k].x, A[j][k].x), make_float2(wa.z, wa.w), o2[2 * c4 + 1]);
                o2[2 * c4] = ffma2(make_float2(A[j][k].y, A[j][k].y), make_float2(wb.x, wb.y), o2[2 * c4]);
                o2[2 * c4 + 1] = ffma2(make_float2(A[j][k].y, A[j][k].y), make_float2(wb.z, wb.w), o2[2 * c4 + 1]);
            }
}

__device__ __forceinline__ float cb2_div_floor(float a, float b)
{
    const float mod = fmodf(a, b);
    float div = __fdiv_rn(__fsub_rn(a, mod), b);
    if ((mod != 0.f) && ((b < 0.f) != (mod < 0.f))) div -= 1.f;
    float fl;
    if (div != 0.f) { fl = floorf(div); if (div - fl > 0.5f) fl += 1.f; }
    else fl = copysignf(0.f, __fdiv_rn(a, b));
    return fl;
}
__device__ __forceinline__ int cb2_round_to_pixel(float mean, int size)
{
    const float inv = __frcp_rn((float)size);
    const int k = (int)cb2_div_floor(__fadd_rn(mean, 1e-5f), inv);
    return min(max(k, 0), size - 1);
}

template <int THREADS>
struct CB2Shared {
    CB2Tile T;
    uint64_t bar;
    float red[THREADS / 32][16];
    long long sum[THREADS / 32][3];
    int tm[THREADS / 32];
    __align__(16) float xt[THREADS / 32][64];
};

template <class PT, int NCH, bool MODE_A, int CAP, int THREADS, bool POOL_MEAN, bool PLAIN, bool TC>
__device__ __forceinline__ void cb2_voxel(const dagr_geom_t &g, int64_t N, const int32_t *__restrict__ start, const uint32_t *__restrict__ xyb,
             const int2 *__restrict__ ti, const float *__restrict__ feat_s, const float *__restrict__ xa,
             const int32_t *__restrict__ nbr, const uint16_t *__restrict__ off,
             const PT &P, const float4 *__restrict__ wfrag, const float *__restrict__ skip_pre_in, const int min_idx_in,
             float *__restrict__ persist_in, float *__restrict__ x1_in, int32_t *__restrict__ cnt, int32_t *__restrict__ pxy,
             float *__restrict__ tmean, float *__restrict__ tmax, float *__restrict__ xg, int ldx,
             float *__restrict__ xa_out, float *__restrict__ skip_out,
             const int cell, unsigned char *smem_raw, CB2Shared<THREADS> &S, uint32_t &parity,
             int32_t *__restrict__ wl_hdr, int32_t *__restrict__ wl_ids, const int defer)
{
    const int min_idx = PLAIN ? 0 : min_idx_in;
    float *const persist = PLAIN ? nullptr : persist_in;
    float *const x1 = PLAIN ? nullptr : x1_in;
    const float *const skip_pre = PLAIN ? nullptr : skip_pre_in;
    const bool relu = PLAIN ? true : (P.relu != 0);
    CB2Tile &T = S.T;
    uint64_t &s_bar = S.bar;
    auto &s_red = S.red;
    auto &s_sum = S.sum;
    auto &s_tm = S.tm;
    float *const xt = S.xt[threadIdx.x >> 5];
    float *s_rows = (float *)smem_raw;
    float *s_wx = s_rows + (size_t)CAP * 8;
    float4 *s_wy = (float4 *)(s_wx + 128);
    float *s_wy4 = (float *)(s_wy + 32);
    uint32_t *s_ell = (uint32_t *)(s_wy + 64);
    uint16_t *s_sp = (uint16_t *)(s_ell + DAGR_ELL * THREADS);
    const int per = g.ny1 * g.nx1;
    const int b = cell / per, rem = cell % per, cy = rem / g.nx1, cx = rem % g.nx1;
    const int p0 = start[(int64_t)cell * g.CP], p1 = start[(int64_t)(cell + 1) * g.CP];
    const int nown = p1 - p0;
    if (nown == 0) {
        if (MODE_A) return;
        if (threadIdx.x == 0) { cnt[cell] = 0; pxy[2 * cell] = 0; pxy[2 * cell + 1] = 0; tmean[cell] = 0.f; tmax[cell] = 0.f; }
        if (threadIdx.x < 16) xg[(int64_t)cell * ldx + threadIdx.x] = 0.f;
        return;
    }
    if (threadIdx.x < 32) {
        const int clo = max(cx - 1, 0), chi = min(cx + 1, g.nx1 - 1);
        const int lane = threadIdx.x, rr = lane >> 1, ry = cy - 1 + rr;
        int v = 0;
        if (lane < 6 && ry >= 0 && ry < g.ny1)
            v = start[((int64_t)b * per + ry * g.nx1 + ((lane & 1) ? chi + 1 : clo)) * g.CP];
        int o = 0;
#pragma unroll
        for (int k = 0; k < 3; k++) {
            const int s0 = __shfl_sync(0xffffffffu, v, 2 * k), e0 = __shfl_sync(0xffffffffu, v, 2 * k + 1);
            const bool ok = (cy - 1 + k >= 0) && (cy - 1 + k < g.ny1);
            if (lane == 0) { T.run_start[k] = ok ? s0 : 0; T.run_len[k] = ok ? e0 - s0 : 0; T.run_off[k] = o; }
            o += ok ? e0 - s0 : 0;
        }
    }
    for (int i = threadIdx.x; i < 2 * g.r + 1; i += blockDim.x) {
        const float4 tx = __ldg(reinterpret_cast<const float4 *>(g.tabx) + i);
        s_wx[i] = tx.x; s_wx[32 + i] = tx.y; s_wx[64 + i] = tx.z;
        s_wy[i] = __ldg(reinterpret_cast<const float4 *>(g.taby) + 2 * i);
        s_wy4[i] = __ldg(g.taby + 8 * i + 4);
    }
    for (int i = threadIdx.x; i < g.ncell; i += blockDim.x)
        s_sp[i] = (uint16_t)(((int)g.spiral[2 * i] + g.r) | (((int)g.spiral[2 * i + 1] + g.r) << 5));
    __syncthreads();
    const int total = T.run_off[2] + T.run_len[2];
    const bool staged = total <= CAP;
    if (!staged && wl_hdr != nullptr) {
        int slot = 0;
        if (threadIdx.x == 0) slot = atomicAdd(&wl_hdr[0], 1);
        if (defer) { if (threadIdx.x == 0) wl_ids[slot] = cell; return; }
    }
    const int s1 = T.run_start[1];
    const int s2 = T.run_len[2] > 0 ? T.run_start[2] : 0x7fffffff;
    const int d0 = T.run_off[0] - T.run_start[0], d1 = T.run_off[1] - T.run_start[1], d2 = T.run_off[2] - T.run_start[2];

    constexpr bool pool_mean = POOL_MEAN && !MODE_A;
    float m[16];
#pragma unroll
    for (int c = 0; c < 16; c++) m[c] = pool_mean ? 0.f : -INFINITY;
    long long sx = 0, sy = 0, st = 0;
    int tm = -2147483647;
    const bool sparse = MODE_A && staged && nown <= 32;
    const int lane_ = threadIdx.x & 31, wid_ = threadIdx.x >> 5;
    for (int pb0 = p0; pb0 < p1; pb0 += blockDim.x) {
        const int p = sparse ? p0 + lane_ : pb0 + threadIdx.x;
        const bool inrange = sparse ? (p < p1 && wid_ < 3) : (p < p1);
        const int tix = sparse ? lane_ : (int)threadIdx.x;
        const bool active = inrange && (min_idx <= 0 || ti[p].y >= min_idx);
        if (min_idx > 0 && !__syncthreads_or(active)) {
            if (inrange) { const uint32_t w0 = xyb[p]; const int t0 = ti[p].x; sx += w0 & 0xfff; sy += (w0 >> 12) & 0xfff; st += t0; tm = max(tm, t0); }
            continue;
        }
        const int n = active ? nbr[(int64_t)(DAGR_ELL - 1) * N + p] : 0;
        if (staged && active && (!sparse || wid_ == 0)) {
            int jj[DAGR_ELL - 1]; int cc[DAGR_ELL - 1];
#pragma unroll
            for (int q = 0; q < DAGR_ELL - 1; q++) {
                jj[q] = (q < n) ? nbr[(int64_t)q * N + p] : 0;
                cc[q] = (q < n) ? (int)off[(int64_t)q * N + p] : 0;
            }
#pragma unroll
            for (int q = 0; q < DAGR_ELL - 1; q++) {
                const int j = jj[q];
                const int row = j + (j >= s2 ? d2 : (j >= s1 ? d1 : d0));
                s_ell[(q + 1) * THREADS + tix] = ((uint32_t)(2 * row + XA_SWZ(j)) << 4) | ((uint32_t)s_sp[cc[q]] << 18);
            }
            s_ell[tix] = ((uint32_t)(2 * (p + d1) + XA_SWZ(p)) << 4) | ((uint32_t)(g.r | (g.r << 5)) << 18);
        }
        float2 o2[8], sk2[MODE_A ? 8 : 1];
#pragma unroll
        for (int k = 0; k < 8; k++) o2[k] = make_float2(0.f, 0.f);
#pragma unroll
        for (int k = 0; k < (MODE_A ? 8 : 1); k++) sk2[k] = make_float2(0.f, 0.f);
#pragma unroll 1
        for (int half = 0; half < NCH; half++) {
            if (staged) {
                __syncthreads();
                if (threadIdx.x == 0) {
                    mbar_expect_tx(&s_bar, (uint32_t)total * 32u);
                    for (int rr = 0; rr < 3; rr++)
                        if (T.run_len[rr] > 0)
                            tma_bulk_g2s(s_rows + (size_t)T.run_off[rr] * 8, xa + ((size_t)half * N + T.run_start[rr]) * 8,
                                         (uint32_t)T.run_len[rr] * 32u, &s_bar);
                }
                mbar_wait(&s_bar, parity);
                parity ^= 1;
            }
            if (TC ? __any_sync(0xffffffffu, active) : active) {
                const int nn = active ? n : -1;
#define CB2_ROOT(H)                                                                                                  \
    do {                                                                                                            \
        const float4 *src = staged ? reinterpret_cast<const float4 *>(s_rows + (int64_t)(p + d1) * 8)               \
                                   : reinterpret_cast<const float4 *>(xa + ((int64_t)(H) * N + p) * 8);             \
        const float4 z4 = make_float4(0.f, 0.f, 0.f, 0.f);                                                         \
        const float4 t0 = active ? src[XA_SWZ(p)] : z4, t1 = active ? src[XA_SWZ(p) ^ 1] : z4;                      \
        const float v[8] = {t0.x, t0.y, t0.z, t0.w, t1.x, t1.y, t1.z, t1.w};                                        \
        if constexpr (TC) {                                                                                         \
            float2 c2[8];                                                                                           \
            _Pragma("unroll") for (int i = 0; i < 8; i++) c2[i] = make_float2(0.f, 0.f);                            \
            cb2_tc_kstep(xt, v, wfrag + (((H) * CB2_TC_KSTEPS + 15) * 32 + lane_) * 2, c2);                         \
            _Pragma("unroll") for (int i = 0; i < 8; i++)                                                           \
                o2[i] = make_float2(__fadd_rn(o2[i].x, c2[i].x), __fadd_rn(o2[i].y, c2[i].y));                      \
        }                                                                                                           \
        _Pragma("unroll") for (int k = 0; k < 8; k++)                                                               \
            _Pragma("unroll") for (int c4 = 0; c4 < 4; c4++) {                                                      \
                if constexpr (!TC) {                                                                                \
                    const float4 w4 = *reinterpret_cast<const float4 *>(&P.root[8 * (H) + k][4 * c4]);              \
                    o2[2 * c4] = ffma2(make_float2(v[k], v[k]), make_float2(w4.x, w4.y), o2[2 * c4]);               \
                    o2[2 * c4 + 1] = ffma2(make_float2(v[k], v[k]), make_float2(w4.z, w4.w), o2[2 * c4 + 1]);       \
                }                                                                                                   \
                if constexpr (MODE_A) {                     \
                    const float4 k4 = *reinterpret_cast<const float4 *>(&P.skip[8 * (H) + k][4 * c4]);              \
                    sk2[2 * c4] = ffma2(make_float2(v[k], v[k]), make_float2(k4.x, k4.y), sk2[2 * c4]);             \
                    sk2[2 * c4 + 1] = ffma2(make_float2(v[k], v[k]), make_float2(k4.z, k4.w), sk2[2 * c4 + 1]);     \
                }                                                                                                   \
            }                                                                                                       \
    } while (0)
                if (!sparse || wid_ == 0) {
                    if (half == 0)      CB2_ROOT(0);
                    else if (half == 1) CB2_ROOT(1);
                    else if constexpr (NCH > 2) CB2_ROOT(2);
                }
#undef CB2_ROOT
#define CB2_PASS(H, G)                                                                                               \
    do {                                                                                                            \
        if (staged) cb2_pass<true, H, G, THREADS, TC>(N, p, nn, xa, s_rows, s_wx, s_wy, s_wy4, s_ell, s_sp, nbr, off, P, wfrag, xt, p + d1, g.r, tix, o2); \
        else        cb2_pass<false, H, G, THREADS, TC>(N, p, nn, xa, s_rows, s_wx, s_wy, s_wy4, s_ell, s_sp, nbr, off, P, wfrag, xt, 0, g.r, tix, o2);     \
    } while (0)
#define CB2_HALF(H)                                                                                                  \
    do {                                                                                                            \
        if (!sparse) { CB2_PASS(H, 0); CB2_PASS(H, 1); CB2_PASS(H, 2); }                                            \
        else if (wid_ == 0) CB2_PASS(H, 0);                                                                         \
        else if (wid_ == 1) CB2_PASS(H, 1);                                                                         \
        else CB2_PASS(H, 2);                                                                                        \
    } while (0)
                if (half == 0)      CB2_HALF(0);
                else if (half == 1) CB2_HALF(1);
                else if constexpr (NCH > 2) CB2_HALF(2);
#undef CB2_HALF
#undef CB2_PASS
            }
        }
        if constexpr (TC) {
            if (__any_sync(0xffffffffu, active)) cb2_tc_unfrag(xt, o2);
        }
        if (sparse) {
            __syncthreads();
            float *s_part = s_rows;
            if (active && wid_ >= 1) {
                float4 *dst = reinterpret_cast<float4 *>(s_part + ((size_t)(wid_ - 1) * 32 + lane_) * 16);
                dst[0] = make_float4(o2[0].x, o2[0].y, o2[1].x, o2[1].y);
                dst[1] = make_float4(o2[2].x, o2[2].y, o2[3].x, o2[3].y);
                dst[2] = make_float4(o2[4].x, o2[4].y, o2[5].x, o2[5].y);
                dst[3] = make_float4(o2[6].x, o2[6].y, o2[7].x, o2[7].y);
            }
            __syncthreads();
            if (active && wid_ == 0) {
#pragma unroll
                for (int w2 = 0; w2 < 2; w2++) {
                    const float4 *src = reinterpret_cast<const float4 *>(s_part + ((size_t)w2 * 32 + lane_) * 16);
#pragma unroll
                    for (int k = 0; k < 4; k++) {
                        const float4 v = src[k];
                        o2[2 * k].x += v.x; o2[2 * k].y += v.y; o2[2 * k + 1].x += v.z; o2[2 * k + 1].y += v.w;
                    }
                }
            }
        }
        const bool owner = !sparse || wid_ == 0;
        if (!MODE_A && inrange && owner) { const uint32_t w0 = xyb[p]; const int t0 = ti[p].x; sx += w0 & 0xfff; sy += (w0 >> 12) & 0xfff; st += t0; tm = max(tm, t0); }
        if (!active || !owner) continue;
        float o[16];
#pragma unroll
        for (int c = 0; c < 8; c++) { o[2 * c] = o2[c].x; o[2 * c + 1] = o2[c].y; }
        if constexpr (MODE_A) {
            float sk[16];
#pragma unroll
            for (int c = 0; c < 8; c++) { sk[2 * c] = sk2[c].x; sk[2 * c + 1] = sk2[c].y; }
            const int sw = XA_SWZ(p);
            {
                const float4 *pp = reinterpret_cast<const float4 *>(xa_out + (int64_t)p * 8);
                const float4 a0 = pp[sw], a1 = pp[sw ^ 1];
                pp = reinterpret_cast<const float4 *>(xa_out + (N + (int64_t)p) * 8);
                const float4 a2 = pp[sw], a3 = pp[sw ^ 1];
                const float part[16] = {a0.x, a0.y, a0.z, a0.w, a1.x, a1.y, a1.z, a1.w, a2.x, a2.y, a2.z, a2.w, a3.x, a3.y, a3.z, a3.w};
                const uint32_t wxy = xyb[p];
                const float f0 = feat_s[p], f1 = __ldg(g.posx0 + (wxy & 0xfff)), f2 = __ldg(g.posy0 + ((wxy >> 12) & 0xfff));
#pragma unroll
                for (int c = 0; c < 16; c++) {
                    o[c] += part[c];
                    sk[c] = fmaf(f0, P.skip[16][c], sk[c]);
                    sk[c] = fmaf(f1, P.skip[17][c], sk[c]);
                    sk[c] = fmaf(f2, P.skip[18][c], sk[c]);
                }
            }
#pragma unroll
            for (int c = 0; c < 16; c++) {
                const float r = fmaf(o[c], P.scale[c], P.shift[c]);
                o[c] = relu ? fmaxf(r, 0.f) : r;
                sk[c] = fmaf(sk[c], P.sscale[c], P.sshift[c]);
            }
            float4 *dst = reinterpret_cast<float4 *>(xa_out + (int64_t)p * 8);
            dst[sw] = make_float4(o[0], o[1], o[2], o[3]);
            dst[sw ^ 1] = make_float4(o[4], o[5], o[6], o[7]);
            dst = reinterpret_cast<float4 *>(xa_out + (N + (int64_t)p) * 8);
            dst[sw] = make_float4(o[8], o[9], o[10], o[11]);
            dst[sw ^ 1] = make_float4(o[12], o[13], o[14], o[15]);
            float4 *sd = reinterpret_cast<float4 *>(skip_out + (int64_t)p * 16);
            sd[0] = make_float4(sk[0], sk[1], sk[2], sk[3]);
            sd[1] = make_float4(sk[4], sk[5], sk[6], sk[7]);
            sd[2] = make_float4(sk[8], sk[9], sk[10], sk[11]);
            sd[3] = make_float4(sk[12], sk[13], sk[14], sk[15]);
            continue;
        }
        const uint32_t wxy = xyb[p];
        const int x = wxy & 0xfff, y = (wxy >> 12) & 0xfff;
        float skv[16];
        if (skip_pre != nullptr) {
            const float4 *sp = reinterpret_cast<const float4 *>(skip_pre + (int64_t)p * 16);
            const float4 a = sp[0], b4 = sp[1], c4 = sp[2], d4 = sp[3];
            skv[0] = a.x; skv[1] = a.y; skv[2] = a.z; skv[3] = a.w; skv[4] = b4.x; skv[5] = b4.y; skv[6] = b4.z; skv[7] = b4.w;
            skv[8] = c4.x; skv[9] = c4.y; skv[10] = c4.z; skv[11] = c4.w; skv[12] = d4.x; skv[13] = d4.y; skv[14] = d4.z; skv[15] = d4.w;
        } else {
            const float f0 = feat_s[p], f1 = __ldg(g.posx0 + x), f2 = __ldg(g.posy0 + y);
#pragma unroll
            for (int c = 0; c < 16; c++) {
                float sk = f0 * P.skip[0][c];
                sk = fmaf(f1, P.skip[1][c], sk);
                sk = fmaf(f2, P.skip[2][c], sk);
                skv[c] = fmaf(sk, P.sscale[c], P.sshift[c]);
            }
        }
#pragma unroll
        for (int c = 0; c < 16; c++) {
            float r = fmaf(o[c], P.scale[c], P.shift[c]) + skv[c];
            r = relu ? fmaxf(r, 0.f) : r;
            o[c] = r;
        }
#pragma unroll
        for (int c = 0; c < 16; c++) m[c] = pool_mean ? m[c] + o[c] : fmaxf(m[c], o[c]);
        if (x1 != nullptr) {
            float4 *dst = reinterpret_cast<float4 *>(x1 + (int64_t)p * 16);
            dst[0] = make_float4(o[0], o[1], o[2], o[3]);
            dst[1] = make_float4(o[4], o[5], o[6], o[7]);
            dst[2] = make_float4(o[8], o[9], o[10], o[11]);
            dst[3] = make_float4(o[12], o[13], o[14], o[15]);
        }
    }
    if (MODE_A) return;
    const int lane = threadIdx.x & 31, wid = threadIdx.x >> 5;
#pragma unroll
    for (int d = 16; d > 0; d >>= 1) {
#pragma unroll
        for (int c = 0; c < 16; c++) {
            const float o2 = __shfl_xor_sync(0xffffffffu, m[c], d);
            m[c] = pool_mean ? m[c] + o2 : fmaxf(m[c], o2);
        }
        sx += __shfl_xor_sync(0xffffffffu, sx, d);
        sy += __shfl_xor_sync(0xffffffffu, sy, d);
        st += __shfl_xor_sync(0xffffffffu, st, d);
        tm = max(tm, __shfl_xor_sync(0xffffffffu, tm, d));
    }
    if (lane == 0) {
#pragma unroll
        for (int c = 0; c < 16; c++) s_red[wid][c] = m[c];
        s_sum[wid][0] = sx; s_sum[wid][1] = sy; s_sum[wid][2] = st; s_tm[wid] = tm;
    }
    __syncthreads();
    const int nw = blockDim.x >> 5;
    if (threadIdx.x < 16) {
        float v = s_red[0][threadIdx.x];
        for (int w2 = 1; w2 < nw; w2++) v = pool_mean ? v + s_red[w2][threadIdx.x] : fmaxf(v, s_red[w2][threadIdx.x]);
        if (pool_mean) v = __fdiv_rn(v, (float)nown);
        if (persist != nullptr) {
            if (min_idx > 0) v = fmaxf(v, persist[(int64_t)cell * 16 + threadIdx.x]);
            persist[(int64_t)cell * 16 + threadIdx.x] = v;
        }
        xg[(int64_t)cell * ldx + threadIdx.x] = v;
    }
    if (threadIdx.x == 32) {
        long long ax = 0, ay = 0, at = 0; int tmx = -2147483647;
        for (int w2 = 0; w2 < nw; w2++) { ax += s_sum[w2][0]; ay += s_sum[w2][1]; at += s_sum[w2][2]; tmx = max(tmx, s_tm[w2]); }
        const float mx = (float)((double)ax / ((double)nown * (double)g.W));
        const float my = (float)((double)ay / ((double)nown * (double)g.H));
        cnt[cell] = nown;
        pxy[2 * cell] = cb2_round_to_pixel(mx, g.W);
        pxy[2 * cell + 1] = cb2_round_to_pixel(my, g.H);
        tmean[cell] = (float)((double)at / ((double)nown * (double)g.T));
        tmax[cell] = __fdiv_rn((float)tmx, (float)g.T);
    }
}


template <class PT, int NCH, bool MODE_A, bool POOL_MEAN, bool PLAIN, bool TC>
__global__ void __launch_bounds__(CB2_THREADS, MODE_A ? 3 : 4)
k_l1_conv_b2(const dagr_geom_t g, int64_t N, const int32_t *__restrict__ start, const uint32_t *__restrict__ xyb,
             const int2 *__restrict__ ti, const float *__restrict__ feat_s, const float *__restrict__ xa,
             const int32_t *__restrict__ nbr, const uint16_t *__restrict__ off,
             const __grid_constant__ PT P, const float4 *__restrict__ wfrag, const float *__restrict__ skip_pre, const int min_idx,
             float *__restrict__ persist, float *__restrict__ x1, int32_t *__restrict__ cnt, int32_t *__restrict__ pxy,
             float *__restrict__ tmean, float *__restrict__ tmax, float *__restrict__ xg, int ldx,
             float *__restrict__ xa_out, float *__restrict__ skip_out, int32_t *__restrict__ wl_hdr, int32_t *__restrict__ wl_ids,
             const int defer)
{
    extern __shared__ __align__(128) unsigned char smem_raw[];
    __shared__ __align__(16) CB2Shared<CB2_THREADS> S;
    if (threadIdx.x == 0) mbar_init(&S.bar, 1);
    uint32_t parity = 0;
    cb2_voxel<PT, NCH, MODE_A, CB2_CAP, CB2_THREADS, POOL_MEAN, PLAIN, TC>(g, N, start, xyb, ti, feat_s, xa, nbr, off, P, wfrag, skip_pre, min_idx,
                                                      persist, x1, cnt, pxy, tmean, tmax, xg, ldx, xa_out, skip_out, (int)blockIdx.x,
                                                      smem_raw, S, parity, wl_hdr, wl_ids, defer);
}

template <class PT, int NCH, bool MODE_A, bool POOL_MEAN, bool PLAIN, bool TC>
__global__ void __launch_bounds__(CB2_THREADS_BIG, 1)
k_l1_conv_b2_dense(const dagr_geom_t g, int64_t N, const int32_t *__restrict__ start, const uint32_t *__restrict__ xyb,
                   const int2 *__restrict__ ti, const float *__restrict__ feat_s, const float *__restrict__ xa,
                   const int32_t *__restrict__ nbr, const uint16_t *__restrict__ off,
                   const __grid_constant__ PT P, const float4 *__restrict__ wfrag, const float *__restrict__ skip_pre, const int min_idx,
                   float *__restrict__ persist, float *__restrict__ x1, int32_t *__restrict__ cnt, int32_t *__restrict__ pxy,
                   float *__restrict__ tmean, float *__restrict__ tmax, float *__restrict__ xg, int ldx,
                   float *__restrict__ xa_out, float *__restrict__ skip_out, int32_t *__restrict__ wl_hdr, const int32_t *__restrict__ wl_ids)
{
    extern __shared__ __align__(128) unsigned char smem_raw[];
    __shared__ __align__(16) CB2Shared<CB2_THREADS_BIG> S;
    __shared__ int s_next;
    if (threadIdx.x == 0) mbar_init(&S.bar, 1);
    uint32_t parity = 0;
    const int count = wl_hdr[0];
    for (;;) {
        __syncthreads();
        if (threadIdx.x == 0) s_next = atomicAdd(&wl_hdr[1], 1);
        __syncthreads();
        const int i = s_next;
        if (i >= count) break;
        cb2_voxel<PT, NCH, MODE_A, CB2_CAP_BIG, CB2_THREADS_BIG, POOL_MEAN, PLAIN, TC>(g, N, start, xyb, ti, feat_s, xa, nbr, off, P, wfrag, skip_pre,
                                                                  min_idx, persist, x1, cnt, pxy, tmean, tmax, xg, ldx, xa_out, skip_out,
                                                                  wl_ids[i], smem_raw, S, parity, nullptr, nullptr, 0);
    }
}

static size_t cb2_smem_bytes(const dagr_geom_t *g, int cap, int threads)
{
    return (size_t)cap * 32 + 96 * 16 + (size_t)DAGR_ELL * threads * 4 + (size_t)g->ncell * 2 + 32;
}

template <class PT, int NCH, bool MODE_A, bool TC, bool POOL_MEAN = false, bool PLAIN = false>
static int cb2_launch(const dagr_geom_t *g, int64_t N, const int32_t *start, const uint32_t *xyb, const int2 *ti, const float *feat_s,
                      const float *xa, const int32_t *nbr, const uint16_t *off, const PT *p_host, const float4 *wfrag, const float *skip_pre,
                      int min_idx, float *persist, float *x1, int32_t *cnt, int32_t *pxy, float *tmean, float *tmax, float *xg, int ldx,
                      float *xa_out, float *skip_out, int32_t *wl_hdr, int32_t *wl_ids, int defer, cudaStream_t st)
{
    const int cells = g->B * g->ny1 * g->nx1;
    const size_t smem = cb2_smem_bytes(g, CB2_CAP, CB2_THREADS);
    auto kern = k_l1_conv_b2<PT, NCH, MODE_A, POOL_MEAN, PLAIN, TC>;
    DAGR_CUDA(dagr_allow_smem(kern, smem, true));
    kern<<<cells, CB2_THREADS, smem, st>>>(*g, N, start, xyb, ti, feat_s, xa, nbr, off, *p_host, wfrag, skip_pre, min_idx, persist, x1, cnt,
                                           pxy, tmean, tmax, xg, ldx, xa_out, skip_out, wl_hdr, wl_ids,
                                           (wl_hdr != nullptr && wl_ids != nullptr && defer) ? 1 : 0);
    DAGR_CHECK_LAUNCH();
    if (wl_hdr != nullptr && wl_ids != nullptr && defer) {
        static int n_sm = 0;
        if (n_sm == 0) {
            int dev = 0;
            DAGR_CUDA(cudaGetDevice(&dev));
            DAGR_CUDA(cudaDeviceGetAttribute(&n_sm, cudaDevAttrMultiProcessorCount, dev));
        }
        const size_t smem_big = cb2_smem_bytes(g, CB2_CAP_BIG, CB2_THREADS_BIG);
        auto kd = k_l1_conv_b2_dense<PT, NCH, MODE_A, POOL_MEAN, PLAIN, TC>;
        DAGR_CUDA(dagr_allow_smem(kd, smem_big));
        kd<<<n_sm, CB2_THREADS_BIG, smem_big, st>>>(*g, N, start, xyb, ti, feat_s, xa, nbr, off, *p_host, wfrag, skip_pre, min_idx, persist,
                                                    x1, cnt, pxy, tmean, tmax, xg, ldx, xa_out, skip_out, wl_hdr, wl_ids);
        DAGR_CHECK_LAUNCH();
    }
    return DAGR_OK;
}

template <bool TC>
static int conv_b_pool_voxel(const dagr_geom_t *g, int64_t N, const int32_t *start, const uint32_t *xyb, const int32_t *ti,
                             const float *feat_s, const float *xa, const int32_t *nbr, const uint16_t *off, const dagr_l1b_params_t *p_host,
                             const float4 *wfrag, const float *skip_pre, int min_idx, float *persist, float *x1, int32_t *cnt,
                             int32_t *pxy, float *tmean, float *tmax, float *xg, int ldx, int32_t *wl_hdr, int32_t *wl_ids, int defer,
                             cudaStream_t st)
{
    DAGR_CHECK_ARG(g && p_host, "null argument");
    DAGR_CHECK_ARG(g->r <= 15, "radius must be <= 15 px (offsets are packed in 5 bits)");
    DAGR_CHECK_ARG(!(p_host->pool_mean && persist), "the running per-voxel aggregate of the event stream is a max (max_pool.py:59-62)");
    if (p_host->pool_mean)
        return cb2_launch<dagr_l1b_params_t, 2, false, TC, true>(g, N, start, xyb, (const int2 *)ti, feat_s, xa, nbr, off, p_host, wfrag,
                                                                 skip_pre, min_idx, persist, x1, cnt, pxy, tmean, tmax, xg, ldx, nullptr,
                                                                 nullptr, wl_hdr, wl_ids, defer, st);
    if (min_idx <= 0 && persist == nullptr && x1 == nullptr && skip_pre == nullptr && p_host->relu)
        return cb2_launch<dagr_l1b_params_t, 2, false, TC, false, true>(g, N, start, xyb, (const int2 *)ti, feat_s, xa, nbr, off, p_host, wfrag,
                                                                        nullptr, 0, nullptr, nullptr, cnt, pxy, tmean, tmax, xg, ldx, nullptr,
                                                                        nullptr, wl_hdr, wl_ids, defer, st);
    return cb2_launch<dagr_l1b_params_t, 2, false, TC>(g, N, start, xyb, (const int2 *)ti, feat_s, xa, nbr, off, p_host, wfrag, skip_pre,
                                                       min_idx, persist, x1, cnt, pxy, tmean, tmax, xg, ldx, nullptr, nullptr, wl_hdr, wl_ids,
                                                       defer, st);
}

extern "C" int dagr_l1_conv_b_pool_voxel(const dagr_geom_t *g, int64_t N, const int32_t *start, const uint32_t *xyb,
                                         const int32_t *ti, const float *feat_s, const float *xa, const int32_t *nbr,
                                         const uint16_t *off, const float *tab, const dagr_l1b_params_t *p_host,
                                         const float *skip_pre, int min_idx, float *persist, float *x1, int32_t *cnt,
                                         int32_t *pxy, float *tmean, float *tmax, float *xg, int ldx, int32_t *wl_hdr, int32_t *wl_ids,
                                         int defer, void *stream)
{
    (void)tab;
    return conv_b_pool_voxel<false>(g, N, start, xyb, ti, feat_s, xa, nbr, off, p_host, nullptr, skip_pre, min_idx, persist, x1, cnt, pxy,
                                    tmean, tmax, xg, ldx, wl_hdr, wl_ids, defer, (cudaStream_t)stream);
}

extern "C" int dagr_l1_conv_b_pool_voxel_tc(const dagr_geom_t *g, int64_t N, const int32_t *start, const uint32_t *xyb,
                                            const int32_t *ti, const float *feat_s, const float *xa, const int32_t *nbr,
                                            const uint16_t *off, const dagr_l1b_params_t *p_host, const float *wfrag,
                                            const float *skip_pre, int min_idx, float *persist, float *x1, int32_t *cnt,
                                            int32_t *pxy, float *tmean, float *tmax, float *xg, int ldx, int32_t *wl_hdr, int32_t *wl_ids,
                                            int defer, void *stream)
{
    DAGR_CHECK_ARG(wfrag, "null weight fragments (dagr_l1_tc_weights)");
    return conv_b_pool_voxel<CB2_TC != 0>(g, N, start, xyb, ti, feat_s, xa, nbr, off, p_host, (const float4 *)wfrag, skip_pre, min_idx,
                                          persist, x1, cnt, pxy, tmean, tmax, xg, ldx, wl_hdr, wl_ids, defer, (cudaStream_t)stream);
}

template <bool TC>
static int conv_a_image(const dagr_geom_t *g, int64_t N, const int32_t *start, const uint32_t *xyb, const float *feat_s, const float *x0,
                        const int32_t *nbr, const uint16_t *off, const dagr_l1img_params_t *p_host, const float4 *wfrag, float *xa,
                        float *skipv, int32_t *wl_hdr, int32_t *wl_ids, int defer, cudaStream_t st)
{
    DAGR_CHECK_ARG(g && p_host && xyb && feat_s, "null argument");
    if (N <= 0) return DAGR_OK;
    DAGR_CHECK_ARG(g->r <= 15, "radius must be <= 15 px (offsets are packed in 5 bits)");
    return cb2_launch<dagr_l1img_params_t, 2, true, TC>(g, N, start, xyb, nullptr, feat_s, x0, nbr, off, p_host, wfrag, nullptr, 0, nullptr,
                                                        nullptr, nullptr, nullptr, nullptr, nullptr, nullptr, 0, xa, skipv, wl_hdr, wl_ids,
                                                        defer, st);
}

extern "C" int dagr_l1_conv_a_image(const dagr_geom_t *g, int64_t N, const int32_t *start, const uint32_t *xyb, const float *feat_s,
                                    const float *x0, const int32_t *nbr,
                                    const uint16_t *off, const dagr_l1img_params_t *p_host, float *xa, float *skipv,
                                    int32_t *wl_hdr, int32_t *wl_ids, int defer, void *stream)
{
    return conv_a_image<false>(g, N, start, xyb, feat_s, x0, nbr, off, p_host, nullptr, xa, skipv, wl_hdr, wl_ids, defer, (cudaStream_t)stream);
}

extern "C" int dagr_l1_conv_a_image_tc(const dagr_geom_t *g, int64_t N, const int32_t *start, const uint32_t *xyb, const float *feat_s,
                                       const float *x0, const int32_t *nbr, const uint16_t *off, const dagr_l1img_params_t *p_host,
                                       const float *wfrag, float *xa, float *skipv, int32_t *wl_hdr, int32_t *wl_ids, int defer, void *stream)
{
    DAGR_CHECK_ARG(wfrag, "null weight fragments (dagr_l1_tc_weights)");
    return conv_a_image<CB2_TC != 0>(g, N, start, xyb, feat_s, x0, nbr, off, p_host, (const float4 *)wfrag, xa, skipv, wl_hdr, wl_ids, defer,
                                     (cudaStream_t)stream);
}

extern "C" int dagr_l1_conv_a_image_inc(const dagr_geom_t *g, int64_t N, const int32_t *start, const uint32_t *xyb, const int32_t *ti,
                                        const float *feat_s, const float *x0, const int32_t *nbr, const uint16_t *off,
                                        const dagr_l1img_params_t *p_host, const float *wfrag, int min_idx, float *xa, float *skipv,
                                        int32_t *wl_hdr, int32_t *wl_ids, int defer, void *stream)
{
    DAGR_CHECK_ARG(g && start && xyb && ti && feat_s && x0 && nbr && off && p_host && wfrag && xa && skipv,
                   "null argument (only wl_hdr / wl_ids may be NULL)");
    DAGR_CHECK_ARG(min_idx >= 0, "min_idx must be >= 0");
    DAGR_CHECK_ARG(N >= 0 && N < (1ll << 31), "N out of range");
    if (N == 0) return DAGR_OK;
    DAGR_CHECK_ARG(g->r <= 15, "radius must be <= 15 px (offsets are packed in 5 bits)");
    return cb2_launch<dagr_l1img_params_t, 2, true, CB2_TC != 0>(g, N, start, xyb, (const int2 *)ti, feat_s, x0, nbr, off, p_host,
                                                                  (const float4 *)wfrag, nullptr, min_idx, nullptr, nullptr, nullptr,
                                                                  nullptr, nullptr, nullptr, nullptr, 0, xa, skipv, wl_hdr, wl_ids, defer,
                                                                  (cudaStream_t)stream);
}

static float tf32_rna_host(float x)
{
    uint32_t u;
    memcpy(&u, &x, 4);
    if ((u & 0x7f800000u) != 0x7f800000u) u = (u + 0x1000u) & 0xffffe000u;
    float r;
    memcpy(&r, &u, 4);
    return r;
}

extern "C" int dagr_l1_tc_weights(const float *w_host, const float *root_host, int cin, float *wfrag_host)
{
    DAGR_CHECK_ARG(w_host && root_host && wfrag_host, "null argument");
    DAGR_CHECK_ARG(cin >= 16, "the tensor-core instances take input channels 0..15");
    for (int half = 0; half < 2; half++)
        for (int s = 0; s < CB2_TC_KSTEPS; s++)
            for (int lane = 0; lane < 32; lane++)
                for (int nt = 0; nt < 2; nt++) {
                    const int g = lane >> 2, t = lane & 3, n = 8 * nt + g;
                    const float *W = s < DAGR_KU ? w_host + (size_t)s * cin * 16 : root_host;
                    const float x0 = W[(8 * half + t) * 16 + n], x1 = W[(8 * half + t + 4) * 16 + n];
                    const float h0 = tf32_rna_host(x0), h1 = tf32_rna_host(x1);
                    float *o = wfrag_host + ((((size_t)half * CB2_TC_KSTEPS + s) * 32 + lane) * 2 + nt) * 4;
                    o[0] = h0; o[1] = h1; o[2] = x0 - h0; o[3] = x1 - h1;
                }
    return DAGR_OK;
}


__global__ void k_xa_permute(int64_t N, const int32_t *__restrict__ perm, int n_old, float *__restrict__ xa_sorted,
                             float *__restrict__ xa_arrival, int scatter)
{
    const int64_t t = (int64_t)blockIdx.x * blockDim.x + threadIdx.x;
    const int64_t p = t >> 2;
    const int q = (int)(t & 3);
    if (p >= N) return;
    const int i = perm[p];
    float4 *srt = reinterpret_cast<float4 *>(xa_sorted + ((int64_t)(q >> 1) * N + p) * 8) + ((q & 1) ^ XA_SWZ(p));
    float4 *arr = reinterpret_cast<float4 *>(xa_arrival + (int64_t)i * 16) + q;
    if (scatter) { if (i >= n_old) *arr = *srt; }
    else         { if (i < n_old) *srt = *arr; }
}

extern "C" int dagr_xa_permute(int64_t N, const int32_t *perm, int n_old, float *xa_sorted, float *xa_arrival, int scatter, void *stream)
{
    if (N <= 0) return DAGR_OK;
    k_xa_permute<<<dagr_div_up(4 * N, 256), 256, 0, (cudaStream_t)stream>>>(N, perm, n_old, xa_sorted, xa_arrival, scatter);
    DAGR_CHECK_LAUNCH();
    return DAGR_OK;
}
```

dagr_b200/engine.py:

```python
from __future__ import annotations

import ctypes as C
import math
from typing import Dict, List, Optional

import torch

from . import _lib
from .geometry import Geometry


def _fold_bn(bn):
    m = bn.module
    scale = (m.weight / torch.sqrt(m.running_var + m.eps)).float()
    shift = (m.bias - m.running_mean * scale).float()
    return scale.contiguous(), shift.contiguous()


def _tc_weights(lib, params, cin: int, device) -> torch.Tensor:
    out = (C.c_float * _lib.L1_TC_WFRAG_FLOATS)()
    _lib.check(lib.dagr_l1_tc_weights(C.cast(params.w, C.c_void_p), C.cast(params.root, C.c_void_p), cin, C.cast(out, C.c_void_p)),
               "dagr_l1_tc_weights")
    return torch.frombuffer(out, dtype=torch.float32).clone().to(device)


def _fill(arr, t: torch.Tensor):
    flat = t.detach().float().cpu().contiguous().view(-1)
    assert flat.numel() == len(arr), (flat.numel(), len(arr))
    C.memmove(arr, flat.data_ptr(), flat.numel() * 4)


class _ConvPack:
    def __init__(self, conv, norm=None, relu=False, dev=None):
        self.cin, self.cout = conv.in_channels, conv.out_channels
        self.weight = conv.weight.detach().float().contiguous().to(dev)
        self.rootT = conv.lin.weight.detach().float().t().contiguous().to(dev)
        self.bias = conv.bias.detach().float().contiguous().to(dev) if conv.bias is not None else None
        if norm is not None:
            s, b = _fold_bn(norm)
            self.scale, self.shift = s.detach().to(dev), b.detach().to(dev)
        else:
            self.scale = self.shift = None
        self.relu = relu


def _merge_packs(a: "_ConvPack", b: "_ConvPack") -> "_ConvPack":
    m = _ConvPack.__new__(_ConvPack)
    assert a.cin == b.cin and a.relu == b.relu and (a.bias is None) == (b.bias is None) and (a.scale is None) == (b.scale is None)
    m.cin, m.cout = a.cin, a.cout + b.cout
    m.weight = torch.cat([a.weight, b.weight], dim=2).contiguous()
    m.rootT = torch.cat([a.rootT, b.rootT], dim=1).contiguous()
    m.bias = None if a.bias is None else torch.cat([a.bias, b.bias]).contiguous()
    m.scale = None if a.scale is None else torch.cat([a.scale, b.scale]).contiguous()
    m.shift = None if a.shift is None else torch.cat([a.shift, b.shift]).contiguous()
    m.relu = a.relu
    return m


class _LayerPack:
    def __init__(self, layer, relu, dev):
        self.a = _ConvPack(layer.conv_block1.conv, layer.conv_block1.norm, relu, dev)
        self.b = _ConvPack(layer.conv_block2.conv, layer.conv_block2.norm, relu, dev)
        self.skipT = layer.conv_block2.lin.mlp.weight.detach().float().t().contiguous().to(dev)
        s, b = _fold_bn(layer.conv_block2.norm_skip)
        self.sscale, self.sshift = s.detach().to(dev), b.detach().to(dev)


class GridState:

    def __init__(self, level, cells, dev):
        self.level = level
        self.cells = cells
        self.cnt = torch.empty(cells, dtype=torch.int32, device=dev)
        self.pxy = torch.empty((cells, 2), dtype=torch.int32, device=dev)
        self.tmean = torch.empty(cells, dtype=torch.float32, device=dev)
        self.tmax = torch.empty(cells, dtype=torch.float32, device=dev)
        self.mask = None
        self.x = None


class _WsView:
    _SLOT_KEYS = ("zero_buf", "grids", "pool", "graph", "graph_warm", "graph_key")

    def __init__(self, base: dict, slot: dict):
        self.base, self.slot = base, slot

    def __getitem__(self, k):
        return self.slot[k] if k in self._SLOT_KEYS else self.base[k]

    def __setitem__(self, k, v):
        (self.slot if k in self._SLOT_KEYS else self.base)[k] = v

    def __contains__(self, k):
        return k in (self.slot if k in self._SLOT_KEYS else self.base)

    def get(self, k, default=None):
        return (self.slot if k in self._SLOT_KEYS else self.base).get(k, default)


class Engine:
    def __init__(self, model):
        self.model = model
        self.lib = _lib.load()
        self._geoms: Dict[tuple, Geometry] = {}
        self._pack = None
        self._pack_key = None
        self._pack_gen = 0
        self._sentinels = None
        self._ws: Dict[tuple, dict] = {}
        self.keep_node_features = False
        self.voxel_conv_b = True
        self.use_graphs = True
        self.fused_build = True
        self.dense_worklists = "auto"
        self._dense = {}
        self.last = {}
        self.launches = 0
        self.prof = None
        self.overlap = False
        self._cstream = None
        self._fstream = None
        self._slot = 0
        self._done = [None, None]
        self._out_slot = {}

    _NKERNELS = dict(dagr_graph_sort=6, dagr_graph_sort_ring=6, dagr_stream_push=2, dagr_graph_sort_rings=6, dagr_stream_push_multi=2, dagr_graph_search=1, dagr_l1_build=2, dagr_graph_export=5, dagr_l1_conv_a=1, dagr_l1_conv_b_pool=1, dagr_l1_conv_b_pool_voxel=2, dagr_l1_conv_b_pool_voxel_tc=2, dagr_l1_x0_image=1, dagr_l1_x0_image_live=1, dagr_xa_permute=1, dagr_l1_conv_a_image=2, dagr_l1_conv_a_image_tc=2, dagr_voxel_sample_max=1,
                     dagr_l1_conv_a_image_inc=2, dagr_voxel_sample_max_inc=1,
                     dagr_l1_x0_image_planes=1, dagr_voxel_sample_max_planes=1, dagr_sample_features_planes=1, dagr_head_finish_planes=1,
                     dagr_pool1_finalize=1, dagr_grid_cat_pos=1, dagr_grid_conv=1, dagr_grid_linear_bn=1, dagr_grid_pool=1,
                     dagr_grid_pool_finalize=1, dagr_grid_temporal_filter=1, dagr_grid_to_dense=1, dagr_head_decode=1, dagr_head_finish=1,
                     dagr_postprocess_nms=1, dagr_sample_features=1, dagr_denormalize_pos=1)

    def _run(self, label, fn, *args):
        if self.prof is not None:
            e0 = torch.cuda.Event(enable_timing=True); e1 = torch.cuda.Event(enable_timing=True)
            e0.record()
        _lib.check(fn(*args), label)
        self.launches += self._NKERNELS.get(fn.__name__, 1)
        if self.prof is not None:
            e1.record()
            self.prof.setdefault(label, []).append((e0, e1))

    def prof_summary(self):
        out = {}
        for k, evs in (self.prof or {}).items():
            ts = [a.elapsed_time(b) for a, b in evs]
            out[k] = dict(ms=sum(ts) / len(ts), calls=len(ts))
        return out

    def geometry(self, W, H, B, device) -> Geometry:
        key = (int(W), int(H), int(B), str(device))
        g = self._geoms.get(key)
        if g is None:
            a = self.model.args
            g = Geometry(W, H, B, radius=a.radius, time_window=self.model.time_window,
                         max_neighbors=a.max_neighbors, max_queue_size=self.model.backbone.events_to_graph.max_queue_size,
                         pooling_dim_at_output=a.pooling_dim_at_output, kernel_size=getattr(a, "kernel_size", 5),
                         device=device)
            self._geoms[key] = g
        return g

    def _params_key(self):
        if self._sentinels is None:
            ts = [t for t in self.model.state_dict().values() if t.dtype.is_floating_point]
            step = max(1, len(ts) // 12)
            self._sentinels = ts[::step] + ts[-1:]
        return tuple((t.data_ptr(), t._version) for t in self._sentinels)

    def invalidate(self):
        self._pack = None
        self._pack_key = None
        self._sentinels = None
        self._pack_gen += 1
        for ws in self._ws.values():
            for sw in ws.get("slots", {}).values():
                sw.pop("graph", None)
                sw.pop("graph_key", None)
                sw["graph_warm"] = 0

    def pack(self, geom: Geometry, device):
        key = (self._params_key(), tuple(geom.slots1), str(device))
        if self._pack is not None and self._pack_key == key:
            return self._pack
        if self._cstream is not None:
            self._cstream.synchronize()
        m = self.model
        bb, hd = m.backbone, m.head
        act = getattr(m.args, "activation", "relu")
        relu = True
        l1 = bb.conv_block1
        ca, cb = l1.conv_block1, l1.conv_block2
        slots = torch.tensor(geom.slots1, dtype=torch.long)
        cin0 = ca.conv.in_channels
        if self.lib.dagr_check_config(C.byref(geom.c_geom), 0, int(cin0), int(ca.conv.out_channels), str(act).encode()) != 0:
            raise NotImplementedError("dagr_b200: " + (self.lib.dagr_last_error() or b"").decode())
        pb = _lib.L1BParams()
        _fill(pb.w, cb.conv.weight.detach().cpu()[slots])
        _fill(pb.root, cb.conv.lin.weight.detach().cpu().t())
        s, b = _fold_bn(cb.norm); _fill(pb.scale, s); _fill(pb.shift, b)
        s, b = _fold_bn(cb.norm_skip); _fill(pb.sscale, s); _fill(pb.sshift, b)
        pb.relu = 1
        pb.pool_mean = 0 if getattr(m.args, "pooling_aggr", "max") == "max" else 1
        for i in range(3):
            pb.xs[i] = geom.slots_x[i]
        for j in range(5):
            pb.ys[j] = geom.slots_y[j]
        pb.den_x, pb.den_y = geom.den1_x, geom.den1_y
        pk = dict(l1b=pb, l1a=None, l1img=None)
        pk["l1b_wfrag"] = _tc_weights(self.lib, pb, 16, device)
        if cin0 == 3:
            pa = _lib.L1AParams()
            _fill(pa.w, ca.conv.weight.detach().cpu()[slots])
            _fill(pa.root, ca.conv.lin.weight.detach().cpu().t())
            s, b = _fold_bn(ca.norm); _fill(pa.scale, s); _fill(pa.shift, b)
            pa.relu = 1
            _fill(pb.skip, cb.lin.mlp.weight.detach().cpu().t())
            pk["l1a"] = pa
        else:
            order = list(range(1, 17)) + [0, 17, 18]
            pi = _lib.L1ImgParams()
            w = torch.zeros(15, 24, 16); w[:, :19] = ca.conv.weight.detach().cpu().float()[slots][:, order]
            r = torch.zeros(24, 16); r[:19] = ca.conv.lin.weight.detach().cpu().float().t()[order]
            k = torch.zeros(24, 16); k[:19] = cb.lin.mlp.weight.detach().cpu().float().t()[order]
            _fill(pi.w, w); _fill(pi.root, r); _fill(pi.skip, k)
            pe = _lib.L1AParams()
            _fill(pe.w, ca.conv.weight.detach().cpu().float()[slots][:, [0, 17, 18]])
            _fill(pe.root, ca.conv.lin.weight.detach().cpu().float().t()[[0, 17, 18]])
            _fill(pe.scale, torch.ones(16)); _fill(pe.shift, torch.zeros(16))
            pe.relu = 0
            pk["l1a_img"] = pe
            s, b = _fold_bn(ca.norm); _fill(pi.scale, s); _fill(pi.shift, b)
            s, b = _fold_bn(cb.norm_skip); _fill(pi.sscale, s); _fill(pi.sshift, b)
            pi.relu = 1
            pk["l1img"] = pi
            pk["l1img_wfrag"] = _tc_weights(self.lib, pi, 24, device)
        pk["layers"] = [_LayerPack(getattr(bb, n), relu, device) for n in ("layer2", "layer3", "layer4", "layer5")]
        heads = []
        for k in range(hd.num_scales):
            sfx = str(k + 1)
            stem, cc, rc = getattr(hd, "stem" + sfx), getattr(hd, "cls_conv" + sfx), getattr(hd, "reg_conv" + sfx)
            hp = dict(stem=_ConvPack(stem.conv, stem.norm, relu, device),
                      cls_conv=_ConvPack(cc.conv, cc.norm, relu, device),
                      reg_conv=_ConvPack(rc.conv, rc.norm, relu, device),
                      cls_pred=_ConvPack(getattr(hd, "cls_pred" + sfx), None, False, device),
                      reg_pred=_ConvPack(getattr(hd, "reg_pred" + sfx), None, False, device),
                      obj_pred=_ConvPack(getattr(hd, "obj_pred" + sfx), None, False, device))
            hp["clsreg_conv"] = _merge_packs(hp["cls_conv"], hp["reg_conv"])
            hp["regobj_pred"] = _merge_packs(hp["reg_pred"], hp["obj_pred"])
            heads.append(hp)
        pk["heads"] = heads
        self._pack_gen += 1
        self._pack, self._pack_key = pk, key
        return pk

    def workspace(self, geom: Geometry, N: int, device):
        key = (id(geom), str(device))
        ws = self._ws.get(key)
        cap = 0 if ws is None else ws["cap"]
        if ws is None or N > cap:
            if self._cstream is not None:
                self._cstream.synchronize()
            cap = max(int(N * 1.25), 1024)
            dev = device
            nscan = max(geom.NK + 1, cap + 1)
            ws = dict(cap=cap)
            sz = _lib.EventWs()
            _lib.check(self.lib.dagr_event_workspace_bytes(C.byref(geom.c_geom), cap, C.byref(sz)), "event_workspace_bytes")
            for name, dt in (("key", torch.int32), ("tmp", torch.int32), ("blocksums", torch.int32), ("start", torch.int32),
                             ("perm", torch.int32), ("ti", torch.int32), ("xyb", torch.int32), ("feat_s", torch.float32),
                             ("nbr", torch.int32), ("off", torch.int16), ("xa", torch.float32)):
                ws[name] = torch.empty(int(getattr(sz, name)) // torch.empty(0, dtype=dt).element_size(), dtype=dt, device=dev)
            ws["ti"] = ws["ti"].view(-1, 2)
            ws["count"] = torch.zeros(int(sz.count) // 4, dtype=torch.int32, device=dev)
            ws["x1"] = None
            C_lv = self.model.backbone.output_channels
            sizes = {}
            off = 0

            def take(name, nbytes):
                nonlocal off
                nbytes = (nbytes + 255) // 256 * 256
                sizes[name] = (off, nbytes)
                off += nbytes

            take("cellmask", int(sz.cellmask))
            take("poolmax", geom.cells1 * 16 * 4)
            bb = self.model.backbone
            fc = list(getattr(getattr(bb, "net", None), "feature_channels", [])) if bb.use_image else []
            for lv in (1, 2, 3):
                cells = geom.cells(lv)
                Cc = C_lv[lv] + (fc[lv + 1] if bb.use_image else 0)
                psz = _lib.PoolWs()
                _lib.check(self.lib.dagr_pool_workspace_bytes(cells, int(Cc), C.byref(psz)), "pool_workspace_bytes")
                take(f"acc{lv}", int(psz.acc))
                take(f"possum{lv}", int(psz.possum))
                take(f"ptmax{lv}", int(psz.ptmax))
                take(f"pcnt{lv}", int(psz.pcnt))
                take(f"pmask{lv}", int(psz.pmask))
            take("wl_hdr", 32)
            for wl in ("wl_build", "wl_conv_a", "wl_conv_b"):
                take(wl, int(sz.wl_ids))
            take("err", 4)
            take("flags", 16)
            ws["zero_buf"] = torch.zeros(off, dtype=torch.uint8, device=dev)
            ws["zero_slices"] = sizes
            grids = []
            for lv in range(4):
                grids.append(GridState(lv, geom.cells(lv), dev))
            ws["grids"] = grids
            ws["pool"] = {}
            self._ws[key] = ws
        return ws

    def _slot_view(self, ws: dict, slot: int, geom: Geometry, dev) -> _WsView:
        slots = ws.setdefault("slots", {})
        sw = slots.get(slot)
        if sw is None:
            if slot == 0:
                sw = dict(zero_buf=ws["zero_buf"], grids=ws["grids"], pool=ws["pool"])
            else:
                sw = dict(zero_buf=torch.zeros_like(ws["zero_buf"]), grids=[GridState(lv, geom.cells(lv), dev) for lv in range(4)],
                          pool={})
            slots[slot] = sw
        return _WsView(ws, sw)

    def join(self):
        cur = torch.cuda.current_stream()
        for ev in self._done:
            if ev is not None:
                cur.wait_event(ev)

    def fence(self):
        if self.overlap and self._cstream is not None and self._out_slot:
            ev = torch.cuda.Event()
            ev.record(self._cstream)
            self._done[next(iter(self._out_slot.values()))] = ev

    def result_stream(self):
        return torch.cuda.stream(self._cstream if (self.overlap and self._cstream is not None) else torch.cuda.current_stream())

    def _dense_policy(self, ws, wl_hdr, fixed: bool):
        if self.dense_worklists is True:
            return [1, 1, 1]
        if self.dense_worklists is False or fixed:
            return [0, 0, 0]
        st = self._dense.get(id(ws.base))
        if st is None:
            st = dict(defer=[0, 0, 0], host=torch.zeros(8, dtype=torch.int32).pin_memory(), event=None, quiet=[0, 0, 0])
            self._dense[id(ws.base)] = st
        if st["event"] is not None and st["event"].query():
            h = st["host"]
            cells = max(1, ws["grids"][0].cells)
            for k in range(3):
                if int(h[2 * k]) * 20 >= cells:
                    st["defer"][k], st["quiet"][k] = 1, 0
                elif st["defer"][k]:
                    st["quiet"][k] += 1
                    if st["quiet"][k] >= 16:
                        st["defer"][k] = 0
            st["event"] = None
        return list(st["defer"])

    def _dense_report(self, ws, wl_hdr):
        st = self._dense.get(id(ws.base))
        if st is None or st["event"] is not None:
            return
        st["host"].copy_(wl_hdr[:8], non_blocking=True)
        ev = torch.cuda.Event()
        ev.record()
        st["event"] = ev

    def _zs(self, ws, name, dtype):
        off, nbytes = ws["zero_slices"][name]
        return ws["zero_buf"][off:off + nbytes].view(dtype)

    def _buf(self, ws, name, shape, dtype, dev):
        t = ws["pool"].get(name)
        n = 1
        for s in shape:
            n *= s
        if t is None or t.numel() < n or t.dtype != dtype:
            t = torch.empty(max(n, 1), dtype=dtype, device=dev)
            ws["pool"][name] = t
        return t[:n].view(*shape)

    def _grid_conv(self, geom, lv, gs: GridState, xin, pack: _ConvPack, skip, out, st, ldin=0):
        level = geom.levels[lv]
        self._run(f"grid_conv_L{lv + 1}_{pack.cin}x{pack.cout}", self.lib.dagr_grid_conv, C.byref(level.grid), _lib.ptr(gs.cnt), _lib.ptr(gs.pxy), _lib.ptr(gs.mask),
                                           _lib.ptr(xin), int(ldin), pack.cin, pack.cout, _lib.ptr(pack.weight), _lib.ptr(pack.rootT),
                                           _lib.ptr(pack.bias), _lib.ptr(pack.scale), _lib.ptr(pack.shift),
                                           _lib.ptr(skip), 1 if pack.relu else 0, level.den_x, level.den_y,
                                           _lib.ptr(out), st)

    def _layer(self, geom, lv, gs: GridState, lp: _LayerPack, ws, name, st, dev):
        level = geom.levels[lv]
        cells = gs.cells
        cx = gs.x.shape[1]
        xin = self._buf(ws, name + "_in", (cells, cx + 2), torch.float32, dev)
        self._run("cat_pos", self.lib.dagr_grid_cat_pos, C.byref(level.grid), _lib.ptr(gs.cnt), _lib.ptr(gs.pxy), _lib.ptr(gs.x), cx,
                                              _lib.ptr(xin), st)
        a = self._buf(ws, name + "_a", (cells, lp.a.cout), torch.float32, dev)
        self._grid_conv(geom, lv, gs, xin, lp.a, None, a, st)
        sk = self._buf(ws, name + "_s", (cells, lp.b.cout), torch.float32, dev)
        self._run("linear_bn", self.lib.dagr_grid_linear_bn, cells, _lib.ptr(gs.cnt), _lib.ptr(xin), cx + 2, lp.b.cout,
                                                _lib.ptr(lp.skipT), _lib.ptr(lp.sscale), _lib.ptr(lp.sshift),
                                                _lib.ptr(sk), st)
        out = self._buf(ws, name + "_o", (cells, lp.b.cout), torch.float32, dev)
        self._grid_conv(geom, lv, gs, a, lp.b, sk, out, st)
        return xin, a, out

    def _pool(self, geom, lv_child, gc: GridState, x, aggr, ws, st, dev, keep_temporal):
        lp = lv_child + 1
        child, parent = geom.levels[lv_child], geom.levels[lp]
        gp: GridState = ws["grids"][lp]
        Cc = x.shape[1]
        acc = self._zs(ws, f"acc{lp}", torch.uint8)
        if gp.cells * Cc * 8 > acc.numel():
            raise RuntimeError(f"dagr_b200: pooling accumulator of level {lp + 1} holds {acc.numel()} bytes, {gp.cells * Cc * 8} needed "
                               f"({Cc} channels)")
        accmax = acc.view(torch.int32) if aggr == 0 else None
        accsum = acc.view(torch.float64) if aggr == 1 else None
        possum = self._zs(ws, f"possum{lp}", torch.float64)
        ptmax = self._zs(ws, f"ptmax{lp}", torch.int32)
        pcnt = self._zs(ws, f"pcnt{lp}", torch.int32)
        pmask = self._zs(ws, f"pmask{lp}", torch.int32)
        err = self._zs(ws, "err", torch.int32)
        self._run("grid_pool", self.lib.dagr_grid_pool, C.byref(child.grid), C.byref(parent.grid), _lib.ptr(parent.cellx_dev),
                                           _lib.ptr(parent.celly_dev), _lib.ptr(gc.cnt), _lib.ptr(gc.pxy),
                                           _lib.ptr(gc.tmean), _lib.ptr(gc.tmax), _lib.ptr(gc.mask), _lib.ptr(x), Cc, aggr,
                                           _lib.ptr(accmax), _lib.ptr(accsum), _lib.ptr(possum), _lib.ptr(ptmax),
                                           _lib.ptr(pcnt), _lib.ptr(pmask), _lib.ptr(err), st)
        gp.x = self._buf(ws, f"gx{lp}", (gp.cells, Cc), torch.float32, dev)
        self._run("grid_pool_finalize", self.lib.dagr_grid_pool_finalize, C.byref(parent.grid), Cc, aggr, _lib.ptr(accmax), _lib.ptr(accsum),
                                                    _lib.ptr(possum), _lib.ptr(ptmax), _lib.ptr(pcnt), _lib.ptr(gp.pxy),
                                                    _lib.ptr(gp.tmean), _lib.ptr(gp.tmax), _lib.ptr(gp.x), st)
        gp.cnt = pcnt[:gp.cells]
        gp.mask = pmask[:gp.cells]
        if keep_temporal:
            self._run("temporal_filter", self.lib.dagr_grid_temporal_filter, C.byref(parent.grid), _lib.ptr(gp.cnt), _lib.ptr(gp.tmax),
                                                          _lib.ptr(gp.mask), st)
        return gp

    @torch.no_grad()
    def _append_image(self, geom, lv, gs, o, feat, ws, st, dev, planes=None):
        cells, Cc, Cf = gs.cells, o.shape[1], int(feat.shape[1])
        xcat = self._buf(ws, f"xcat{lv}", (cells, Cc + Cf), torch.float32, dev)
        xcat[:, :Cc] = o
        pxy = gs.pxy[:cells].long()
        posx = geom.d_posxr[pxy[:, 0]].contiguous()
        posy = geom.d_posyr[pxy[:, 1]].contiguous()
        key = ("bidx", lv)
        if key not in ws:
            per = geom.levels[lv].nx * geom.levels[lv].ny
            ws[key] = (torch.arange(cells, device=dev) // per).int()
        if planes is not None:
            self._run("sample_features", self.lib.dagr_sample_features_planes, _lib.ptr(feat), int(feat.shape[0]), _lib.ptr(planes[0]),
                      int(planes[1]), Cf, int(feat.shape[2]), int(feat.shape[3]), _lib.ptr(posx), _lib.ptr(posy), _lib.ptr(ws[key]), cells,
                      geom.W, geom.H, _lib.ptr(xcat), Cc + Cf, Cc, st)
            return xcat
        self._run("sample_features", self.lib.dagr_sample_features, _lib.ptr(feat), int(feat.shape[0]), Cf, int(feat.shape[2]),
                  int(feat.shape[3]), _lib.ptr(posx), _lib.ptr(posy), _lib.ptr(ws[key]), cells, geom.W, geom.H, _lib.ptr(xcat),
                  Cc + Cf, Cc, st)
        return xcat

    @torch.no_grad()
    def forward_events(self, batch_i32: torch.Tensor, pos_i32: torch.Tensor, feat: torch.Tensor, B: int,
                       W: int, H: int, image_feats=None, image_outs=None, stream_state=None, n_old: int = 0, ring=None,
                       image_event=None, ring_streams=None, image_planes=None):
        for n, t in (("batch", batch_i32), ("pos", pos_i32), ("x", feat)):
            _lib.require_cuda(t, n)
        dev = pos_i32.device
        N = int(batch_i32.shape[0])
        if ring_streams is not None and (ring is None or int(ring_streams) != int(B) or N % int(ring_streams)):
            raise ValueError(f"ring_streams={ring_streams} needs a ring control block, B == ring_streams and N a multiple of it "
                             f"(B={B}, N={N})")
        if image_planes is not None:
            if ring_streams is None or image_feats is None or image_outs is None:
                raise ValueError("image_planes selects per-stream frames of a multi-ring step: it needs ring_streams, image_feats "
                                 "and image_outs")
            if self.keep_node_features:
                raise ValueError("keep_node_features: the dense head maps (dagr_grid_to_dense) have no plane mode")
            plane_tab, plane_stride = image_planes
        geom = self.geometry(W, H, B, dev)
        pk = self.pack(geom, dev)
        ws = self.workspace(geom, N, dev)
        ov = bool(self.overlap and stream_state is None and image_feats is None and self.prof is None and self.use_graphs and ring is None)
        slot = 0
        if ov:
            slot, self._slot = self._slot, self._slot ^ 1
            if self._cstream is None:
                self._cstream = torch.cuda.Stream(device=dev, priority=-1)
            if self._done[slot] is not None:
                torch.cuda.current_stream().wait_event(self._done[slot])
        else:
            self.join()
        ws = self._slot_view(ws, slot, geom, dev)
        st = _lib.stream_ptr()
        lib = self.lib
        g = C.byref(geom.c_geom)
        model = self.model
        kto = bool(getattr(model.args, "keep_temporal_ordering", False))

        ws["zero_buf"].zero_()
        nbr, off = ws["nbr"], ws["off"]
        cellmask = self._zs(ws, "cellmask", torch.int32)
        min_idx, persist = 0, None
        if stream_state is not None:
            stream_state.ensure(geom, N, dev, img_channels=int(image_feats[1].shape[1]) if image_feats is not None else 0)
            cellmask, persist, min_idx = stream_state.cellmask, stream_state.voxmax, int(n_old)
        poolmax = self._zs(ws, "poolmax", torch.int32)
        flags = self._zs(ws, "flags", torch.int32)
        wl_hdr = self._zs(ws, "wl_hdr", torch.int32)
        defer = self._dense_policy(ws, wl_hdr, ring is not None or stream_state is not None)
        if ring is not None and ring_streams is not None:
            self._run("graph_sort", lib.dagr_graph_sort_rings, g, _lib.ptr(batch_i32), _lib.ptr(pos_i32), _lib.ptr(feat), N // ring_streams,
                      int(ring_streams), _lib.ptr(ring), _lib.ptr(ws["key"]), _lib.ptr(ws["tmp"]), _lib.ptr(ws["count"]),
                      _lib.ptr(ws["blocksums"]), _lib.ptr(ws["start"]), _lib.ptr(ws["perm"]), _lib.ptr(ws["ti"]), _lib.ptr(ws["xyb"]),
                      _lib.ptr(ws["feat_s"]), _lib.ptr(flags), st)
        elif ring is not None:
            self._run("graph_sort", lib.dagr_graph_sort_ring, g, _lib.ptr(batch_i32), _lib.ptr(pos_i32), _lib.ptr(feat), N, _lib.ptr(ring),
                      _lib.ptr(ws["key"]), _lib.ptr(ws["tmp"]), _lib.ptr(ws["count"]), _lib.ptr(ws["blocksums"]), _lib.ptr(ws["start"]),
                      _lib.ptr(ws["perm"]), _lib.ptr(ws["ti"]), _lib.ptr(ws["xyb"]), _lib.ptr(ws["feat_s"]), _lib.ptr(flags), st)
        else:
            self._run("graph_sort", lib.dagr_graph_sort, g, _lib.ptr(batch_i32), _lib.ptr(pos_i32), _lib.ptr(feat), N, _lib.ptr(ws["key"]),
                      _lib.ptr(ws["tmp"]), _lib.ptr(ws["count"]), _lib.ptr(ws["blocksums"]),
                      _lib.ptr(ws["start"]), _lib.ptr(ws["perm"]), _lib.ptr(ws["ti"]), _lib.ptr(ws["xyb"]),
                      _lib.ptr(ws["feat_s"]), _lib.ptr(flags), st)
        use_image = image_feats is not None
        if use_image:
            if stream_state is not None and min_idx > 0:
                self._run("xa_gather", lib.dagr_xa_permute, N, _lib.ptr(ws["perm"]), min_idx, _lib.ptr(ws["xa"]),
                          _lib.ptr(stream_state.xa_arr), 0, st)
            self._run("l1_build", lib.dagr_l1_build, g, N, _lib.ptr(ws["start"]), _lib.ptr(ws["ti"]), _lib.ptr(ws["xyb"]),
                      _lib.ptr(ws["feat_s"]), _lib.ptr(geom.d_tab1), C.byref(pk["l1a_img"]), _lib.ptr(flags), min_idx, _lib.ptr(nbr), _lib.ptr(off),
                      _lib.ptr(cellmask), _lib.ptr(ws["xa"]), _lib.ptr(wl_hdr), _lib.ptr(self._zs(ws, "wl_build", torch.int32)), defer[0], st)
            if image_event is not None:
                torch.cuda.current_stream().wait_event(image_event[0])
            f0 = image_feats[0]
            x0 = self._buf(ws, "x0img", (2 * max(N, 1) * 8,), torch.float32, dev)
            skipv = self._buf(ws, "skipv", (max(N, 1), 16), torch.float32, dev)
            if image_planes is not None:
                self._run("l1_x0_image", lib.dagr_l1_x0_image_planes, g, N, _lib.ptr(ws["start"]), _lib.ptr(ws["xyb"]), _lib.ptr(ws["feat_s"]),
                          _lib.ptr(f0), int(f0.shape[2]), int(f0.shape[3]), int(f0.shape[0]), _lib.ptr(plane_tab), int(plane_stride),
                          _lib.ptr(x0), st)
            elif ring is not None:
                self._run("l1_x0_image", lib.dagr_l1_x0_image_live, g, N, _lib.ptr(ws["start"]), _lib.ptr(ws["xyb"]), _lib.ptr(ws["feat_s"]),
                          _lib.ptr(f0), int(f0.shape[2]), int(f0.shape[3]), _lib.ptr(x0), st)
            else:
                self._run("l1_x0_image", lib.dagr_l1_x0_image, g, N, _lib.ptr(ws["xyb"]), _lib.ptr(ws["feat_s"]), _lib.ptr(f0),
                          int(f0.shape[2]), int(f0.shape[3]), _lib.ptr(x0), st)
            if stream_state is not None:
                self._run("l1_conv_a_image_inc", lib.dagr_l1_conv_a_image_inc, g, N, _lib.ptr(ws["start"]), _lib.ptr(ws["xyb"]),
                          _lib.ptr(ws["ti"]), _lib.ptr(ws["feat_s"]), _lib.ptr(x0), _lib.ptr(nbr), _lib.ptr(off), C.byref(pk["l1img"]),
                          _lib.ptr(pk["l1img_wfrag"]), min_idx, _lib.ptr(ws["xa"]), _lib.ptr(skipv), _lib.ptr(wl_hdr[2:]),
                          _lib.ptr(self._zs(ws, "wl_conv_a", torch.int32)), defer[1], st)
                self._run("xa_scatter", lib.dagr_xa_permute, N, _lib.ptr(ws["perm"]), min_idx, _lib.ptr(ws["xa"]),
                          _lib.ptr(stream_state.xa_arr), 1, st)
            else:
                self._run("l1_conv_a_image", lib.dagr_l1_conv_a_image_tc, g, N, _lib.ptr(ws["start"]), _lib.ptr(ws["xyb"]), _lib.ptr(ws["feat_s"]),
                          _lib.ptr(x0), _lib.ptr(nbr), _lib.ptr(off),
                          C.byref(pk["l1img"]), _lib.ptr(pk["l1img_wfrag"]), _lib.ptr(ws["xa"]), _lib.ptr(skipv), _lib.ptr(wl_hdr[2:]),
                          _lib.ptr(self._zs(ws, "wl_conv_a", torch.int32)), defer[1], st)
        elif self.fused_build or stream_state is not None:
            if min_idx > 0:
                self._run("xa_gather", lib.dagr_xa_permute, N, _lib.ptr(ws["perm"]), min_idx, _lib.ptr(ws["xa"]),
                          _lib.ptr(stream_state.xa_arr), 0, st)
            self._run("l1_build", lib.dagr_l1_build, g, N, _lib.ptr(ws["start"]), _lib.ptr(ws["ti"]), _lib.ptr(ws["xyb"]),
                      _lib.ptr(ws["feat_s"]), _lib.ptr(geom.d_tab1), C.byref(pk["l1a"]), _lib.ptr(flags), min_idx, _lib.ptr(nbr),
                      _lib.ptr(off), _lib.ptr(cellmask), _lib.ptr(ws["xa"]), _lib.ptr(wl_hdr), _lib.ptr(self._zs(ws, "wl_build", torch.int32)),
                      defer[0], st)
            if stream_state is not None:
                self._run("xa_scatter", lib.dagr_xa_permute, N, _lib.ptr(ws["perm"]), min_idx, _lib.ptr(ws["xa"]),
                          _lib.ptr(stream_state.xa_arr), 1, st)
        else:
            self._run("graph_search", lib.dagr_graph_search, g, N, _lib.ptr(ws["start"]), _lib.ptr(ws["ti"]), _lib.ptr(ws["xyb"]),
                      _lib.ptr(nbr), _lib.ptr(off), _lib.ptr(cellmask), st)
            self._run("l1_conv_a", lib.dagr_l1_conv_a, g, N, _lib.ptr(ws["xyb"]), _lib.ptr(ws["feat_s"]), _lib.ptr(nbr), _lib.ptr(off),
                      _lib.ptr(geom.d_tab1), C.byref(pk["l1a"]), _lib.ptr(ws["xa"]), st)
        x1 = None
        if self.keep_node_features:
            if ws["x1"] is None or ws["x1"].shape[0] < ws["cap"]:
                ws["x1"] = torch.empty((ws["cap"], 16), dtype=torch.float32, device=dev)
            x1 = ws["x1"]
        g1: GridState = ws["grids"][0]
        c1 = 16 + (int(image_feats[1].shape[1]) if use_image else 0)
        g1.x = self._buf(ws, "gx0", (g1.cells, c1), torch.float32, dev)
        if self.voxel_conv_b or use_image or stream_state is not None:
            self._run("l1_conv_b_pool_voxel", lib.dagr_l1_conv_b_pool_voxel_tc, g, N, _lib.ptr(ws["start"]), _lib.ptr(ws["xyb"]),
                      _lib.ptr(ws["ti"]), _lib.ptr(ws["feat_s"]), _lib.ptr(ws["xa"]), _lib.ptr(nbr), _lib.ptr(off),
                      C.byref(pk["l1b"]), _lib.ptr(pk["l1b_wfrag"]), _lib.ptr(skipv) if use_image else None, min_idx, _lib.ptr(persist),
                      _lib.ptr(x1), _lib.ptr(g1.cnt), _lib.ptr(g1.pxy), _lib.ptr(g1.tmean), _lib.ptr(g1.tmax), _lib.ptr(g1.x), c1,
                      _lib.ptr(wl_hdr[4:]), _lib.ptr(self._zs(ws, "wl_conv_b", torch.int32)), defer[2], st)
            self._dense_report(ws, wl_hdr)
            if use_image and stream_state is not None:
                f1 = image_feats[1]
                self._run("voxel_sample_max_inc", lib.dagr_voxel_sample_max_inc, g, N, _lib.ptr(ws["start"]), _lib.ptr(ws["xyb"]),
                          _lib.ptr(ws["ti"]), _lib.ptr(f1), int(f1.shape[1]), int(f1.shape[2]), int(f1.shape[3]), min_idx,
                          _lib.ptr(stream_state.imgmax), _lib.ptr(g1.x), c1, 16, int(pk["l1b"].pool_mean), st)
            elif image_planes is not None:
                f1 = image_feats[1]
                self._run("voxel_sample_max", lib.dagr_voxel_sample_max_planes, g, N, _lib.ptr(ws["start"]), _lib.ptr(ws["xyb"]), _lib.ptr(f1),
                          int(f1.shape[1]), int(f1.shape[2]), int(f1.shape[3]), int(f1.shape[0]), _lib.ptr(plane_tab), int(plane_stride),
                          _lib.ptr(g1.x), c1, 16, int(pk["l1b"].pool_mean), st)
            elif use_image:
                f1 = image_feats[1]
                self._run("voxel_sample_max", lib.dagr_voxel_sample_max, g, N, _lib.ptr(ws["start"]), _lib.ptr(ws["xyb"]), _lib.ptr(f1),
                          int(f1.shape[1]), int(f1.shape[2]), int(f1.shape[3]), _lib.ptr(g1.x), c1, 16, int(pk["l1b"].pool_mean), st)
        else:
            self._run("l1_conv_b_pool", lib.dagr_l1_conv_b_pool, g, N, _lib.ptr(ws["xyb"]), _lib.ptr(ws["feat_s"]), _lib.ptr(ws["xa"]),
                      _lib.ptr(nbr), _lib.ptr(off), _lib.ptr(geom.d_tab1), C.byref(pk["l1b"]), _lib.ptr(x1), _lib.ptr(poolmax), st)
            self._run("pool1_finalize", lib.dagr_pool1_finalize, g, N, _lib.ptr(ws["start"]), _lib.ptr(ws["xyb"]), _lib.ptr(ws["ti"]),
                      _lib.ptr(poolmax), 16, _lib.ptr(g1.cnt), _lib.ptr(g1.pxy), _lib.ptr(g1.tmean), _lib.ptr(g1.tmax),
                      _lib.ptr(g1.x), st)
        g1.mask = cellmask[:g1.cells]
        if kto and stream_state is not None:
            step_mask = self._zs(ws, "cellmask", torch.int32)
            step_mask[:g1.cells].copy_(cellmask[:g1.cells])
            g1.mask = step_mask[:g1.cells]
        if kto:
            self._run("temporal_filter", lib.dagr_grid_temporal_filter, C.byref(geom.levels[0].grid), _lib.ptr(g1.cnt), _lib.ptr(g1.tmax),
                                                     _lib.ptr(g1.mask), st)
        def coarse(st):
            aggr_cfg = 0 if getattr(model.args, "pooling_aggr", "max") == "max" else 1
            lay = pk["layers"]
            inter = {}
            def cat_img(lv, gs, o, k):
                return self._append_image(geom, lv, gs, o, image_feats[k], ws, st, dev, image_planes) if use_image else o

            _, _, o2 = self._layer(geom, 0, g1, lay[0], ws, "layer2", st, dev)
            if use_image and image_event is not None:
                torch.cuda.current_stream().wait_event(image_event[1])
            g2 = self._pool(geom, 0, g1, cat_img(0, g1, o2, 2), aggr_cfg, ws, st, dev, kto)
            _, _, o3 = self._layer(geom, 1, g2, lay[1], ws, "layer3", st, dev)
            g3 = self._pool(geom, 1, g2, cat_img(1, g2, o3, 3), aggr_cfg, ws, st, dev, kto)
            _, _, o4 = self._layer(geom, 2, g3, lay[2], ws, "layer4", st, dev)
            nc = model.backbone.num_classes
            nscale = model.head.num_scales
            A = sum(geom.levels[lv].nx * geom.levels[lv].ny for lv in ((2, 3) if nscale == 2 else (3,)))
            out = self._buf(ws, "decoded", (B, A, 5 + nc), torch.float32, dev)
            dense_all = [None] * nscale

            def head_scale(k, lv, gs, xo, a0, st):
                hp = pk["heads"][k]
                level = geom.levels[lv]
                cells = gs.cells
                nm = f"head{k}"
                stem = self._buf(ws, nm + "_stem", (cells, hp["stem"].cout), torch.float32, dev)
                self._grid_conv(geom, lv, gs, xo, hp["stem"], None, stem, st)
                Cf = hp["cls_conv"].cout
                cr = self._buf(ws, nm + "_cr", (cells, 2 * Cf), torch.float32, dev)
                self._grid_conv(geom, lv, gs, stem, hp["clsreg_conv"], None, cr, st)
                ocls = self._buf(ws, nm + "_cls", (cells, nc), torch.float32, dev)
                self._grid_conv(geom, lv, gs, cr, hp["cls_pred"], None, ocls, st, ldin=2 * Cf)
                oro = self._buf(ws, nm + "_regobj", (cells, 5), torch.float32, dev)
                self._grid_conv(geom, lv, gs, cr[:, Cf:], hp["regobj_pred"], None, oro, st, ldin=2 * Cf)
                adds = {}
                for name in ("cls", "reg", "obj"):
                    adds[name] = image_outs[name + "_output"][k].float().contiguous() if image_outs is not None else None
                stride = model.backbone.strides[k]
                if image_planes is not None:
                    self._run("head_finish", lib.dagr_head_finish_planes, C.byref(level.grid), _lib.ptr(gs.cnt), _lib.ptr(ocls), nc,
                              _lib.ptr(oro), 5, _lib.ptr(adds["cls"]), _lib.ptr(adds["reg"]), _lib.ptr(adds["obj"]), nc, int(stride), a0, A,
                              int(adds["cls"].shape[0]), _lib.ptr(plane_tab), int(plane_stride), _lib.ptr(out), st)
                    dense_all[k] = {}
                    return
                self._run("head_finish", lib.dagr_head_finish, C.byref(level.grid), _lib.ptr(gs.cnt), _lib.ptr(ocls), nc, _lib.ptr(oro), 5,
                          _lib.ptr(adds["cls"]), _lib.ptr(adds["reg"]), _lib.ptr(adds["obj"]), nc, int(stride), a0, A, _lib.ptr(out), st)
                dense = {}
                if self.keep_node_features:
                    for name, src, c0, cw, ld in (("cls", ocls, 0, nc, nc), ("reg", oro, 0, 4, 5), ("obj", oro, 4, 1, 5)):
                        d = self._buf(ws, nm + "_d" + name, (B, cw, level.ny, level.nx), torch.float32, dev)
                        self._run("to_dense", lib.dagr_grid_to_dense, C.byref(level.grid), _lib.ptr(gs.cnt), _lib.ptr(src[:, c0:]), cw, ld,
                                  _lib.ptr(adds[name]), _lib.ptr(d), st)
                        dense[name] = d
                dense_all[k] = dense

            join_ev = None
            if nscale == 2:
                cur = torch.cuda.current_stream()
                if self._fstream is None:
                    self._fstream = torch.cuda.Stream(device=dev, priority=-1)
                fork_ev = torch.cuda.Event()
                fork_ev.record(cur)
                with torch.cuda.stream(self._fstream):
                    self._fstream.wait_event(fork_ev)
                    head_scale(0, 2, g3, o4, 0, _lib.stream_ptr())
                    join_ev = torch.cuda.Event()
                    join_ev.record(self._fstream)
            g4 = self._pool(geom, 2, g3, cat_img(2, g3, o4, 4), 1, ws, st, dev, kto)
            _, _, o5 = self._layer(geom, 3, g4, lay[3], ws, "layer5", st, dev)
            inter.update(o2=o2, o3=o3, o4=o4, o5=o5)
            a0 = geom.levels[2].nx * geom.levels[2].ny if nscale == 2 else 0
            head_scale(nscale - 1, 3, g4, o5, a0, st)
            if join_ev is not None:
                torch.cuda.current_stream().wait_event(join_ev)
            return out, [g1, g2, g3, g4], inter, dense_all

        gkey = (id(ws.base), slot, self._pack_gen, B, kto, cellmask.data_ptr(), bool(self.keep_node_features))

        def run_coarse():
            if self.use_graphs and self.prof is None and not use_image and ring is None:
                cached = ws.get("graph")
                if cached is not None and cached[0] == gkey:
                    cached[1].replay()
                    self.launches += cached[3]
                    return cached[2]
                l0 = self.launches
                res = coarse(_lib.stream_ptr())
                nk = self.launches - l0
                ws["graph_warm"] = ws.get("graph_warm", 0) + 1
                if ws["graph_warm"] >= 2 and ws.get("graph_key") == gkey:
                    torch.cuda.synchronize()
                    gr = torch.cuda.CUDAGraph()
                    with torch.cuda.graph(gr, stream=self._cstream if ov else None):
                        res_c = coarse(_lib.stream_ptr())
                    self.launches -= nk
                    ws["graph"] = (gkey, gr, res_c, nk)
                ws["graph_key"] = gkey
                return res
            return coarse(st)

        if ov:
            fine_done = torch.cuda.Event()
            fine_done.record()
            with torch.cuda.stream(self._cstream):
                self._cstream.wait_event(fine_done)
                out, grids, inter, dense_all = run_coarse()
                ev = torch.cuda.Event()
                ev.record()
            self._done[slot] = ev
            self._out_slot = {out.data_ptr(): slot}
        else:
            out, grids, inter, dense_all = run_coarse()
            self._out_slot = {}
        g1, g2, g3, g4 = grids
        self.last = dict(geom=geom, ws=ws, N=N, grids=[g1, g2, g3, g4], inter=inter, dense=dense_all, x1=x1)
        return out

    def xa_rows(self):
        L = self.last
        N, xa = L["N"], L["ws"]["xa"]
        rows = torch.cat([xa[:N * 8].view(N, 8), xa[N * 8:2 * N * 8].view(N, 8)], dim=1).clone()
        sw = ((torch.arange(N, device=rows.device) >> 2) & 1).bool()
        r = rows[sw].view(-1, 2, 2, 4)
        rows[sw] = r.flip(2).reshape(-1, 16)
        return rows

    @torch.no_grad()
    def postprocess(self, decoded: torch.Tensor, conf_thre, nms_thre, width, height, filtering=True):
        B, A, D = decoded.shape
        nc = D - 5
        dev = decoded.device
        slot = self._out_slot.get(decoded.data_ptr()) if self.overlap else None
        if slot is None:
            det = torch.empty((B, A, 6), dtype=torch.float32, device=dev)
            ndet = torch.empty(B, dtype=torch.int32, device=dev)
            self._run("postprocess_nms", self.lib.dagr_postprocess_nms, _lib.ptr(decoded), B, A, nc, float(conf_thre), float(nms_thre),
                      int(width), int(height), 1 if filtering else 0, _lib.ptr(det), _lib.ptr(ndet), _lib.stream_ptr())
            return det, ndet
        sw = self.last["ws"]
        det = self._buf(sw, "post_det", (B, A, 6), torch.float32, dev)
        ndet = self._buf(sw, "post_ndet", (B,), torch.int32, dev)
        with torch.cuda.stream(self._cstream):
            self._run("postprocess_nms", self.lib.dagr_postprocess_nms, _lib.ptr(decoded), B, A, nc, float(conf_thre), float(nms_thre),
                      int(width), int(height), 1 if filtering else 0, _lib.ptr(det), _lib.ptr(ndet), _lib.stream_ptr())
            ev = torch.cuda.Event()
            ev.record()
        self._done[slot] = ev
        return det, ndet

    @torch.no_grad()
    def export_edges(self):
        L = self.last
        geom, ws, N = L["geom"], L["ws"], L["N"]
        dev = ws["perm"].device
        if N == 0:
            return torch.zeros((2, 0), dtype=torch.long, device=dev)
        cap = geom.K * N
        inv = torch.empty(N, dtype=torch.int32, device=dev)
        rowptr = torch.empty(N + 1, dtype=torch.int32, device=dev)
        es = torch.empty(cap, dtype=torch.int64, device=dev)
        ed = torch.empty(cap, dtype=torch.int64, device=dev)
        self._run("graph_export", self.lib.dagr_graph_export, C.byref(geom.c_geom), N, _lib.ptr(ws["perm"]), _lib.ptr(ws["ti"]),
                                              _lib.ptr(ws["nbr"]), _lib.ptr(inv), _lib.ptr(rowptr), _lib.ptr(ws["blocksums"]),
                                              _lib.ptr(es), _lib.ptr(ed), cap, _lib.stream_ptr())
        E = int(rowptr[N].item())
        return torch.stack([es[:E], ed[:E]])
```

include/dagr_b200.h:

```cpp
#ifndef DAGR_B200_H
#define DAGR_B200_H

#include <stdint.h>
#include <stddef.h>

#ifdef __cplusplus
extern "C" {
#endif

#define DAGR_ABI_VERSION 2

#define DAGR_OK            0
#define DAGR_E_ARG        -1
#define DAGR_E_CUDA       -2
#define DAGR_E_UNSUPPORTED -3

#define DAGR_ELL 16
#define DAGR_KU  15
#define DAGR_TABW 16
#define DAGR_RING_CTL 8

int         dagr_abi_version(void);
const char *dagr_last_error(void);

typedef struct {
    int32_t W, H, B, T;
    int32_t r, ncell;
    int32_t dt_us, K, Q;
    int32_t nx1, ny1;
    int32_t CW, CH, CP;
    int32_t NK;
    const int32_t *xkey;
    const int32_t *ykey;
    const int8_t  *spiral;
    const float   *posx0;
    const float   *posy0;
    const int32_t *vx0;
    const int32_t *vy0;
    const float   *tabx;
    const float   *taby;
} dagr_geom_t;

typedef struct {
    int64_t key, tmp, count, blocksums, start, perm, ti, xyb, feat_s;
    int64_t nbr, off, cellmask, xa;
    int64_t wl_hdr, wl_ids;
    int64_t x1;
} dagr_event_ws_t;
typedef struct { int64_t acc, possum, ptmax, pcnt, pmask; } dagr_pool_ws_t;
int dagr_check_config(const dagr_geom_t *g, int64_t N, int cin0, int cout0, const char *activation);
int dagr_event_workspace_bytes(const dagr_geom_t *g, int64_t N, dagr_event_ws_t *out);
int dagr_pool_workspace_bytes(int64_t parent_cells, int channels, dagr_pool_ws_t *out);

int dagr_denormalize_pos(const float *pos , int64_t N, int W, int H, int T,
                         int32_t *pos_i32 , void *stream);
int dagr_prepare_events(const float *pos , const int64_t *batch , const float *x , int ldx, int64_t N,
                        int W, int H, int T, int32_t *pos_i32 , int32_t *batch_i32 , float *feat ,
                        void *stream);

int64_t dagr_scan_blocks(int64_t n);

int dagr_graph_sort(const dagr_geom_t *g, const int32_t *batch, const int32_t *pos, const float *feat,
                    int64_t N, int32_t *key, int32_t *tmp, int32_t *count, int32_t *blocksums,
                    int32_t *start, int32_t *perm, int32_t *ti, uint32_t *xyb, float *feat_s,
                    int32_t *flags ,
                    void *stream);

int dagr_graph_sort_ring(const dagr_geom_t *g, const int32_t *batch, const int32_t *pos, const float *feat,
                         int64_t capacity, const int32_t *ctl, int32_t *key, int32_t *tmp, int32_t *count,
                         int32_t *blocksums, int32_t *start, int32_t *perm, int32_t *ti, uint32_t *xyb, float *feat_s,
                         int32_t *flags, void *stream);
int dagr_stream_push(int32_t *ctl, const int32_t *stage, int32_t *batch, int32_t *pos, float *feat, int64_t capacity,
                     int max_chunk, int sample, void *stream);

int dagr_stream_push_multi(int32_t *ctl, const int32_t *stage, int32_t *batch, int32_t *pos, float *feat, int64_t capacity,
                           int streams, int max_chunk, void *stream);
int dagr_graph_sort_rings(const dagr_geom_t *g, const int32_t *batch, const int32_t *pos, const float *feat,
                          int64_t capacity, int streams, const int32_t *ctl, int32_t *key, int32_t *tmp, int32_t *count,
                          int32_t *blocksums, int32_t *start, int32_t *perm, int32_t *ti, uint32_t *xyb, float *feat_s,
                          int32_t *flags, void *stream);

int dagr_graph_search(const dagr_geom_t *g, int64_t N, const int32_t *start, const int32_t *ti,
                      const uint32_t *xyb, int32_t *nbr, uint16_t *off, uint32_t *cellmask,
                      void *stream);

struct dagr_l1a_params_s;
int dagr_l1_build(const dagr_geom_t *g, int64_t N, const int32_t *start, const int32_t *ti,
                  const uint32_t *xyb, const float *feat_s, const float *tab,
                  const struct dagr_l1a_params_s *p_host, const int32_t *flags ,
                  int min_idx ,
                  int32_t *nbr, uint16_t *off, uint32_t *cellmask, float *xa,
                  int32_t *wl_hdr ,
                  int32_t *wl_ids ,
                  int defer ,
                  void *stream);

int dagr_xa_permute(int64_t N, const int32_t *perm, int n_old, float *xa_sorted, float *xa_arrival, int scatter, void *stream);

int dagr_l1_x0_image(const dagr_geom_t *g, int64_t N, const uint32_t *xyb, const float *feat_s,
                     const float *img0 , int h, int w, float *x0, void *stream);
int dagr_l1_x0_image_live(const dagr_geom_t *g, int64_t N, const int32_t *start, const uint32_t *xyb, const float *feat_s,
                          const float *img0 , int h, int w, float *x0, void *stream);

typedef struct {
    float w[DAGR_KU][24][16];
    float root[24][16];
    float skip[24][16];
    float scale[16], shift[16];
    float sscale[16], sshift[16];
    int32_t relu;
} dagr_l1img_params_t;

int dagr_l1_conv_a_image(const dagr_geom_t *g, int64_t N, const int32_t *start, const uint32_t *xyb, const float *feat_s,
                         const float *x0, const int32_t *nbr,
                         const uint16_t *off, const dagr_l1img_params_t *p_host ,
                         float *xa, float *skipv,
                         int32_t *wl_hdr, int32_t *wl_ids, int defer ,
                         void *stream);

int dagr_voxel_sample_max(const dagr_geom_t *g, int64_t N, const int32_t *start, const uint32_t *xyb,
                          const float *img , int C, int h, int w, float *xg, int ldx, int c0, int pool_mean,
                          void *stream);

int dagr_graph_export(const dagr_geom_t *g, int64_t N, const int32_t *perm, const int32_t *ti,
                      const int32_t *nbr, int32_t *inv, int32_t *rowptr, int32_t *blocksums,
                      int64_t *edge_src , int64_t *edge_dst , int64_t cap,
                      void *stream);

typedef struct dagr_l1a_params_s {
    float w[DAGR_KU][3][16];
    float root[3][16];
    float scale[16], shift[16];
    int32_t relu;
} dagr_l1a_params_t;

typedef struct {
    float w[DAGR_KU][16][16];
    float root[16][16];
    float skip[3][16];
    float scale[16], shift[16];
    float sscale[16], sshift[16];
    int32_t relu;
    int32_t pool_mean;
    int32_t xs[3], ys[5];
    float den_x, den_y;
} dagr_l1b_params_t;

int dagr_l1_conv_a(const dagr_geom_t *g, int64_t N, const uint32_t *xyb, const float *feat_s,
                   const int32_t *nbr, const uint16_t *off, const float *tab,
                   const dagr_l1a_params_t *p_host, float *xa , void *stream);

int dagr_l1_conv_b_pool(const dagr_geom_t *g, int64_t N, const uint32_t *xyb, const float *feat_s,
                        const float *xa, const int32_t *nbr, const uint16_t *off, const float *tab,
                        const dagr_l1b_params_t *p_host, float *x1, uint32_t *poolmax, void *stream);

int dagr_l1_conv_b_pool_voxel(const dagr_geom_t *g, int64_t N, const int32_t *start, const uint32_t *xyb,
                              const int32_t *ti, const float *feat_s, const float *xa, const int32_t *nbr,
                              const uint16_t *off, const float *tab, const dagr_l1b_params_t *p_host,
                              const float *skip_pre ,
                              int min_idx ,
                              float *persist ,
                              float *x1, int32_t *cnt, int32_t *pxy, float *tmean, float *tmax, float *xg,
                              int ldx ,
                              int32_t *wl_hdr ,
                              int32_t *wl_ids ,
                              int defer ,
                              void *stream);

#define DAGR_L1_TC_WFRAG_FLOATS 8192
int dagr_l1_tc_weights(const float *w_host ,
                       const float *root_host , int cin ,
                       float *wfrag_host );
int dagr_l1_conv_b_pool_voxel_tc(const dagr_geom_t *g, int64_t N, const int32_t *start, const uint32_t *xyb,
                                 const int32_t *ti, const float *feat_s, const float *xa, const int32_t *nbr,
                                 const uint16_t *off, const dagr_l1b_params_t *p_host, const float *wfrag,
                                 const float *skip_pre, int min_idx, float *persist,
                                 float *x1, int32_t *cnt, int32_t *pxy, float *tmean, float *tmax, float *xg, int ldx,
                                 int32_t *wl_hdr, int32_t *wl_ids, int defer, void *stream);
int dagr_l1_conv_a_image_tc(const dagr_geom_t *g, int64_t N, const int32_t *start, const uint32_t *xyb, const float *feat_s,
                            const float *x0, const int32_t *nbr, const uint16_t *off, const dagr_l1img_params_t *p_host,
                            const float *wfrag, float *xa, float *skipv, int32_t *wl_hdr, int32_t *wl_ids, int defer, void *stream);

int dagr_l1_conv_a_image_inc(const dagr_geom_t *g, int64_t N, const int32_t *start, const uint32_t *xyb, const int32_t *ti,
                             const float *feat_s, const float *x0, const int32_t *nbr, const uint16_t *off,
                             const dagr_l1img_params_t *p_host, const float *wfrag, int min_idx, float *xa, float *skipv,
                             int32_t *wl_hdr, int32_t *wl_ids, int defer, void *stream);
int dagr_voxel_sample_max_inc(const dagr_geom_t *g, int64_t N, const int32_t *start, const uint32_t *xyb, const int32_t *ti,
                              const float *img , int C, int h, int w, int min_idx, float *persist, float *xg, int ldx,
                              int c0, int pool_mean, void *stream);

typedef struct {
    int32_t nx, ny, B;
    int32_t W, H;
    const float *posxr;
    const float *posyr;
} dagr_grid_t;

int dagr_pool1_finalize(const dagr_geom_t *g, int64_t N, const int32_t *start, const uint32_t *xyb,
                        const int32_t *ti, const uint32_t *poolmax, int C,
                        int32_t *cnt, int32_t *pxy, float *tmean, float *tmax, float *x, void *stream);

int dagr_grid_cat_pos(const dagr_grid_t *gr, const int32_t *cnt, const int32_t *pxy, const float *x,
                      int Cx, float *xin, void *stream);

int dagr_grid_conv(const dagr_grid_t *gr, const int32_t *cnt, const int32_t *pxy, const uint32_t *mask,
                   const float *xin, int ldin ,
                   int Cin, int Cout, const float *weight, const float *rootT,
                   const float *bias, const float *scale, const float *shift, const float *skip,
                   int relu, float den_x, float den_y, float *out, void *stream);

int dagr_grid_linear_bn(int64_t cells, const int32_t *cnt, const float *xin, int Cin, int Cout,
                        const float *wT, const float *scale, const float *shift,
                        float *out, void *stream);

int dagr_grid_pool(const dagr_grid_t *child, const dagr_grid_t *parent, const int32_t *cellx,
                   const int32_t *celly, const int32_t *cnt, const int32_t *pxy, const float *tmean,
                   const float *tmax, const uint32_t *mask, const float *x, int C, int aggr,
                   uint32_t *accmax, double *accsum, double *possum, uint32_t *ptmax, int32_t *pcnt,
                   uint32_t *pmask, int32_t *err_flag, void *stream);

int dagr_grid_pool_finalize(const dagr_grid_t *parent, int C, int aggr, const uint32_t *accmax,
                            const double *accsum, const double *possum, const uint32_t *ptmax,
                            const int32_t *pcnt, int32_t *pxy, float *tmean, float *tmax, float *x,
                            void *stream);

int dagr_grid_temporal_filter(const dagr_grid_t *gr, const int32_t *cnt, const float *tmax,
                              uint32_t *mask, void *stream);

int dagr_grid_to_dense(const dagr_grid_t *gr, const int32_t *cnt, const float *x, int C, int ldx ,
                       const float *add , float *dense, void *stream);

int dagr_head_decode(const float *reg, const float *obj, const float *cls, int B, int nc, int h, int w,
                     int stride, int a0, int A, float *out, void *stream);

int dagr_head_finish(const dagr_grid_t *gr, const int32_t *cnt, const float *cls, int ldc, const float *regobj, int ldr,
                     const float *add_cls, const float *add_reg, const float *add_obj, int nc, int stride, int a0, int A,
                     float *out, void *stream);

int dagr_postprocess_nms(const float *pred, int B, int A, int nc, float conf_thre, float nms_thre,
                         int width, int height, int filtering, float *det, int32_t *ndet, void *stream);

int dagr_sample_features(const float *img, int Bi, int C, int h, int w, const float *posx, const float *posy,
                         const int32_t *bidx, int64_t n, int width, int height, float *out, int ldo, int c0,
                         void *stream);

int dagr_l1_x0_image_planes(const dagr_geom_t *g, int64_t N, const int32_t *start, const uint32_t *xyb, const float *feat_s,
                            const float *img0, int h, int w, int nplanes, const int32_t *plane, int plane_stride, float *x0,
                            void *stream);
int dagr_voxel_sample_max_planes(const dagr_geom_t *g, int64_t N, const int32_t *start, const uint32_t *xyb, const float *img, int C,
                                 int h, int w, int nplanes, const int32_t *plane, int plane_stride, float *xg, int ldx, int c0,
                                 int pool_mean, void *stream);
int dagr_sample_features_planes(const float *img, int nplanes, const int32_t *plane, int plane_stride, int C, int h, int w,
                                const float *posx, const float *posy, const int32_t *bidx, int64_t n, int width, int height,
                                float *out, int ldo, int c0, void *stream);
int dagr_head_finish_planes(const dagr_grid_t *gr, const int32_t *cnt, const float *cls, int ldc, const float *regobj, int ldr,
                            const float *add_cls, const float *add_reg, const float *add_obj, int nc, int stride, int a0, int A,
                            int nplanes, const int32_t *plane, int plane_stride, float *out, void *stream);

int dagr_masked_lin(const int64_t *idx, int64_t K, const float *x_in, float *x_out, const float *weight,
                    const float *bias , int Cin, int Cout, int add, void *stream);
int dagr_masked_inplace_bn(const int64_t *idx, int64_t K, const float *x, float *x_out, const float *mean,
                           const float *var, const float *weight, const float *bias, int C, float eps,
                           void *stream);
int dagr_masked_isdiff(int64_t *idx_inout, int64_t K, const float *a, const float *b, int C, float atol,
                       float rtol, void *stream);

int dagr_downsample_events(const uint16_t *x, const uint16_t *y, const int8_t *p, int64_t N, int fx, int fy,
                           int out_w, int out_h, float *change_map, int32_t *cell, int32_t *tmp, int32_t *sorted,
                           int32_t *count, int32_t *start, int32_t *blocksums, uint8_t *mask, void *stream);
int dagr_compact_events(const uint8_t *mask, int64_t N, const uint16_t *x, const uint16_t *y, const int64_t *t,
                        const int8_t *p, int fx, int fy, int32_t *flag, int32_t *pos, int32_t *blocksums,
                        uint16_t *xo, uint16_t *yo, int64_t *to, int8_t *po, int32_t *n_out, void *stream);
int dagr_ingest_events(const uint16_t *x, const uint16_t *y, const int64_t *t, const int8_t *p, int64_t N,
                       int p_is_01, int W, int H, int T, int64_t t_cut, int sample, int32_t *flag, int32_t *pos,
                       int32_t *blocksums, unsigned long long *tlast, int32_t *batch_out, int32_t *pos_out,
                       float *feat_out, int32_t *n_out, void *stream);

#ifdef __cplusplus
}
#endif
#endif
```

Baseline: 550.3.

## Run fused L1 conv-A in graph build on tensor cores via 3xTF32 MMA

Adds a TC variant of the L1 build kernel. It stages each thread's 48 accumulated spline-slot and root inputs through shared memory, loads them with ldmatrix, and multiplies them with pre-split hi/lo TF32 weight fragments using mma.sync. This replaces the per-thread scalar 48x16 FMA conv. Weight fragments are precomputed on the host and the engine now calls the TC entry point. The cost is extra shared-memory traffic, warp-synchronous staging that also covers inactive lanes, and possible register pressure.

```diff
diff --git a/dagr_b200/_lib.py b/dagr_b200/_lib.py
--- a/dagr_b200/_lib.py
+++ b/dagr_b200/_lib.py
@@ -14,6 +14,7 @@
 KU = 15
 TABW = 16
 L1_TC_WFRAG_FLOATS = 8192
+L1A_TC_WFRAG_FLOATS = 1536
 
 p = C.c_void_p
 i32 = C.c_int32
@@ -80,6 +81,8 @@
     "dagr_graph_sort_rings": (C.c_int, [C.POINTER(Geom), p, p, p, i64, C.c_int, p, p, p, p, p, p, p, p, p, p, p, p]),
     "dagr_graph_search": (C.c_int, [C.POINTER(Geom), i64, p, p, p, p, p, p, p]),
     "dagr_l1_build": (C.c_int, [C.POINTER(Geom), i64, p, p, p, p, p, C.POINTER(L1AParams), p, C.c_int, p, p, p, p, p, p, C.c_int, p]),
+    "dagr_l1a_tc_weights": (C.c_int, [C.POINTER(L1AParams), p]),
+    "dagr_l1_build_tc": (C.c_int, [C.POINTER(Geom), i64, p, p, p, p, C.POINTER(L1AParams), p, p, C.c_int, p, p, p, p, p, p, C.c_int, p]),
     "dagr_xa_permute": (C.c_int, [i64, p, C.c_int, p, p, C.c_int, p]),
     "dagr_l1_x0_image": (C.c_int, [C.POINTER(Geom), i64, p, p, p, C.c_int, C.c_int, p, p]),
     "dagr_l1_x0_image_live": (C.c_int, [C.POINTER(Geom), i64, p, p, p, p, C.c_int, C.c_int, p, p]),
diff --git a/dagr_b200/csrc/build_l1.cu b/dagr_b200/csrc/build_l1.cu
--- a/dagr_b200/csrc/build_l1.cu
+++ b/dagr_b200/csrc/build_l1.cu
@@ -198,10 +198,50 @@
     return n;
 }
 
-template <int CAP, int THREADS>
+#define BL_TC_KSTEPS 6
+static_assert(8 * BL_TC_KSTEPS == 3 * DAGR_KU + 3 && BL_TC_KSTEPS * 32 * 2 * 4 == DAGR_L1A_TC_WFRAG_FLOATS, "48 = 45 slot + 3 root inputs");
+
+#define BL_TC_PARK0 38
+
+template <int s>
+__device__ __forceinline__ void bl_tc_inputs(const float (&A)[DAGR_KU][3], const float pk[3 * DAGR_KU - BL_TC_PARK0], const float rt[3],
+                                             float v[8])
+{
+#pragma unroll
+    for (int j = 0; j < 8; j++) {
+        const int k = 8 * s + j;
+        v[j] = k < BL_TC_PARK0 ? A[k / 3][k % 3] : k < 3 * DAGR_KU ? pk[k - BL_TC_PARK0] : rt[k - 3 * DAGR_KU];
+    }
+}
+
+template <int s, int THREADS>
+__device__ __forceinline__ void bl_tc_kstep(const float v[8], uint32_t xw, const float4 *__restrict__ wfrag, float2 c[8])
+{
+    const uint32_t lane = threadIdx.x & 31;
+    const uint32_t row = xw + (lane >> 3) * (THREADS * 4) + 16 * (lane & 7);
+    __syncwarp();
+    asm volatile("st.shared.v4.f32 [%0], {%1, %2, %3, %4};" :: "r"(row), "f"(v[0]), "f"(v[1]), "f"(v[2]), "f"(v[3]) : "memory");
+    asm volatile("st.shared.v4.f32 [%0], {%1, %2, %3, %4};" :: "r"(row + 4 * THREADS * 4), "f"(v[4]), "f"(v[5]), "f"(v[6]), "f"(v[7])
+                 : "memory");
+    __syncwarp();
+    const uint32_t la = xw + (4 * (lane >> 4) + ((lane >> 3) & 1)) * (THREADS * 4) + 16 * (lane & 7);
+#pragma unroll
+    for (int mt = 0; mt < 2; mt++) {
+        uint32_t r[4], ah[4], al[4];
+        ldsm_x4(la + 2 * mt * THREADS * 4, r);
+#pragma unroll
+        for (int i = 0; i < 4; i++) tf32_split(r[i], ah[i], al[i]);
+#pragma unroll
+        for (int nt = 0; nt < 2; nt++)
+            mma_3xtf32(c[4 * mt + 2 * nt], c[4 * mt + 2 * nt + 1], ah, al, __ldg(wfrag + (s * 32 + lane) * 2 + nt));
+    }
+}
+
+template <int CAP, int THREADS, bool TC>
 __device__ __forceinline__ void bl_voxel(const dagr_geom_t &g, int64_t N, const int32_t *__restrict__ start, const int2 *__restrict__ ti,
                                          const uint32_t *__restrict__ xyb, const float *__restrict__ feat_s,
-                                         const dagr_l1a_params_t &P, const int do_conv, const int min_idx, const int32_t *__restrict__ flags,
+                                         const dagr_l1a_params_t &P, const float4 *__restrict__ wfrag, const int do_conv, const int min_idx,
+                                         const int32_t *__restrict__ flags,
                                          int32_t *__restrict__ nbr, uint16_t *__restrict__ off, uint32_t *__restrict__ cellmask,
                                          float *__restrict__ xa, const int cell, unsigned char *smem_raw, BLTile &T, uint32_t &s_mask,
                                          int32_t *__restrict__ wl_hdr, int32_t *__restrict__ wl_ids, const int defer)
@@ -492,6 +532,58 @@
         if (staged) edges(std::true_type{});
         else        edges(std::false_type{});
 
+        if constexpr (TC) {
+            if (!do_conv || !__any_sync(0xffffffffu, active)) continue;
+            const uint32_t xw = bl_sa(s_acc) + 4u * (threadIdx.x & ~31u);
+            float2 c[8];
+#pragma unroll
+            for (int i = 0; i < 8; i++) c[i] = make_float2(0.f, 0.f);
+            constexpr int NPK = 3 * DAGR_KU - BL_TC_PARK0;
+            const uint32_t own = bl_sa(s_acc) + 4u * threadIdx.x;
+#pragma unroll
+            for (int j = 0; j < NPK; j++) {
+                const int k = BL_TC_PARK0 + j;
+                bl_sts32(own + (8 + j) * THREADS * 4, __float_as_uint(A[k / 3][k % 3]));
+            }
+            float rt[3] = {0.f, 0.f, 0.f}, pk[NPK], v[8];
+#pragma unroll
+            for (int j = 0; j < NPK; j++) pk[j] = 0.f;
+            bl_tc_inputs<0>(A, pk, rt, v); bl_tc_kstep<0, THREADS>(v, xw, wfrag, c);
+            bl_tc_inputs<1>(A, pk, rt, v); bl_tc_kstep<1, THREADS>(v, xw, wfrag, c);
+            bl_tc_inputs<2>(A, pk, rt, v); bl_tc_kstep<2, THREADS>(v, xw, wfrag, c);
+            bl_tc_inputs<3>(A, pk, rt, v); bl_tc_kstep<3, THREADS>(v, xw, wfrag, c);
+#pragma unroll
+            for (int j = 0; j < NPK; j++) pk[j] = __uint_as_float(bl_lds32(own + (8 + j) * THREADS * 4));
+            bl_tc_inputs<4>(A, pk, rt, v); bl_tc_kstep<4, THREADS>(v, xw, wfrag, c);
+            int pr = p;
+            asm volatile("" : "+r"(txy), "+r"(pr));
+            rt[0] = __ldg(feat_s + pr); rt[1] = s_posx[(txy & 0xffff) + g.r]; rt[2] = s_posy[(txy >> 16) + g.r];
+            bl_tc_inputs<5>(A, pk, rt, v); bl_tc_kstep<5, THREADS>(v, xw, wfrag, c);
+            const int lane = threadIdx.x & 31, gq = lane >> 2, t = lane & 3;
+            const int pv = active ? p : -1;
+            float2 sc[2], sh[2];
+#pragma unroll
+            for (int nt = 0; nt < 2; nt++) {
+                sc[nt] = *reinterpret_cast<const float2 *>(&P.scale[8 * nt + 2 * t]);
+                sh[nt] = *reinterpret_cast<const float2 *>(&P.shift[8 * nt + 2 * t]);
+            }
+#pragma unroll
+            for (int mt = 0; mt < 2; mt++)
+#pragma unroll
+                for (int hr = 0; hr < 2; hr++) {
+                    const int q = __shfl_sync(0xffffffffu, pv, 16 * mt + 8 * hr + gq);
+#pragma unroll
+                    for (int nt = 0; nt < 2; nt++) {
+                        const float2 o = c[4 * mt + 2 * nt + hr];
+                        float r0 = fmaf(o.x, sc[nt].x, sh[nt].x), r1 = fmaf(o.y, sc[nt].y, sh[nt].y);
+                        if (P.relu) { r0 = fmaxf(r0, 0.f); r1 = fmaxf(r1, 0.f); }
+                        if (q >= 0)
+                            *reinterpret_cast<float2 *>(xa + ((int64_t)nt * N + q) * 8 + (((t >> 1) ^ XA_SWZ(q)) << 2) + 2 * (t & 1)) =
+                                make_float2(r0, r1);
+                    }
+                }
+            continue;
+        }
         if (!active || !do_conv) continue;
         int pr = p;
         asm volatile("" : "+r"(txy), "+r"(pr));
@@ -530,27 +622,28 @@
 
 
 
-template <int CAP, int MIN_CTAS>
+template <int CAP, int MIN_CTAS, bool TC>
 __global__ void __launch_bounds__(BL_THREADS, MIN_CTAS)
 k_l1_build(const dagr_geom_t g, int64_t N, const int32_t *__restrict__ start, const int2 *__restrict__ ti,
            const uint32_t *__restrict__ xyb, const float *__restrict__ feat_s,
-           const __grid_constant__ dagr_l1a_params_t P, const int do_conv, const int min_idx, const int32_t *__restrict__ flags,
-           int32_t *__restrict__ nbr, uint16_t *__restrict__ off, uint32_t *__restrict__ cellmask, float *__restrict__ xa,
-           int32_t *__restrict__ wl_hdr, int32_t *__restrict__ wl_ids, const int defer)
+           const __grid_constant__ dagr_l1a_params_t P, const float4 *__restrict__ wfrag, const int do_conv, const int min_idx,
+           const int32_t *__restrict__ flags, int32_t *__restrict__ nbr, uint16_t *__restrict__ off, uint32_t *__restrict__ cellmask,
+           float *__restrict__ xa, int32_t *__restrict__ wl_hdr, int32_t *__restrict__ wl_ids, const int defer)
 {
     extern __shared__ __align__(16) unsigned char smem_raw[];
     __shared__ BLTile T;
     __shared__ uint32_t s_mask;
-    bl_voxel<CAP, BL_THREADS>(g, N, start, ti, xyb, feat_s, P, do_conv, min_idx, flags, nbr, off, cellmask, xa,
-                              (int)blockIdx.x, smem_raw, T, s_mask, wl_hdr, wl_ids, defer);
-}
-
+    bl_voxel<CAP, BL_THREADS, TC>(g, N, start, ti, xyb, feat_s, P, wfrag, do_conv, min_idx, flags, nbr, off, cellmask, xa,
+                                  (int)blockIdx.x, smem_raw, T, s_mask, wl_hdr, wl_ids, defer);
+}
+
+template <bool TC>
 __global__ void __launch_bounds__(BL_THREADS_BIG, 1)
 k_l1_build_dense(const dagr_geom_t g, int64_t N, const int32_t *__restrict__ start, const int2 *__restrict__ ti,
                  const uint32_t *__restrict__ xyb, const float *__restrict__ feat_s,
-                 const __grid_constant__ dagr_l1a_params_t P, const int do_conv, const int min_idx, const int32_t *__restrict__ flags,
-                 int32_t *__restrict__ nbr, uint16_t *__restrict__ off, uint32_t *__restrict__ cellmask, float *__restrict__ xa,
-                 int32_t *__restrict__ wl_hdr, const int32_t *__restrict__ wl_ids)
+                 const __grid_constant__ dagr_l1a_params_t P, const float4 *__restrict__ wfrag, const int do_conv, const int min_idx,
+                 const int32_t *__restrict__ flags, int32_t *__restrict__ nbr, uint16_t *__restrict__ off,
+                 uint32_t *__restrict__ cellmask, float *__restrict__ xa, int32_t *__restrict__ wl_hdr, const int32_t *__restrict__ wl_ids)
 {
     extern __shared__ __align__(16) unsigned char smem_raw[];
     __shared__ BLTile T;
@@ -563,18 +656,18 @@
         __syncthreads();
         const int i = s_next;
         if (i >= count) break;
-        bl_voxel<BL_CAP_BIG, BL_THREADS_BIG>(g, N, start, ti, xyb, feat_s, P, do_conv, min_idx, flags, nbr, off, cellmask, xa,
-                                             wl_ids[i], smem_raw, T, s_mask, nullptr, nullptr, 0);
-    }
-}
-
-extern "C" int dagr_l1_build(const dagr_geom_t *g, int64_t N, const int32_t *start, const int32_t *ti,
-                             const uint32_t *xyb, const float *feat_s, const float *tab,
-                             const dagr_l1a_params_t *p_host, const int32_t *flags, int min_idx, int32_t *nbr, uint16_t *off,
-                             uint32_t *cellmask, float *xa, int32_t *wl_hdr, int32_t *wl_ids, int defer, void *stream)
+        bl_voxel<BL_CAP_BIG, BL_THREADS_BIG, TC>(g, N, start, ti, xyb, feat_s, P, wfrag, do_conv, min_idx, flags, nbr, off, cellmask, xa,
+                                                 wl_ids[i], smem_raw, T, s_mask, nullptr, nullptr, 0);
+    }
+}
+
+template <bool TC>
+static int l1_build_launch(const dagr_geom_t *g, int64_t N, const int32_t *start, const int32_t *ti, const uint32_t *xyb,
+                           const float *feat_s, const dagr_l1a_params_t *p_host, const float4 *wfrag, const int32_t *flags,
+                           int min_idx, int32_t *nbr, uint16_t *off, uint32_t *cellmask, float *xa, int32_t *wl_hdr,
+                           int32_t *wl_ids, int defer, cudaStream_t st)
 {
     DAGR_CHECK_ARG(g, "null argument");
-    (void)tab;
     static const dagr_l1a_params_t zero_params = {};
     const int do_conv = p_host != nullptr;
     if (!p_host) p_host = &zero_params;
@@ -585,16 +678,16 @@
     const bool deferring = wl_hdr != nullptr && wl_ids != nullptr && defer;
     if (deferring) {
         const size_t smem = bl_smem_bytes(g, BL_CAP, BL_THREADS);
-        auto kern = k_l1_build<BL_CAP, 4>;
+        auto kern = k_l1_build<BL_CAP, 4, TC>;
         DAGR_CUDA(dagr_allow_smem(kern, smem, true));
-        kern<<<cells, BL_THREADS, smem, (cudaStream_t)stream>>>(*g, N, start, (const int2 *)ti, xyb, feat_s, *p_host, do_conv, min_idx,
-                                                                flags, nbr, off, cellmask, xa, wl_hdr, wl_ids, 1);
+        kern<<<cells, BL_THREADS, smem, st>>>(*g, N, start, (const int2 *)ti, xyb, feat_s, *p_host, wfrag, do_conv, min_idx, flags, nbr,
+                                              off, cellmask, xa, wl_hdr, wl_ids, 1);
     } else {
         const size_t smem = bl_smem_bytes(g, BL_CAP_LEAN, BL_THREADS);
-        auto kern = k_l1_build<BL_CAP_LEAN, 5>;
+        auto kern = k_l1_build<BL_CAP_LEAN, 5, TC>;
         DAGR_CUDA(dagr_allow_smem(kern, smem, true));
-        kern<<<cells, BL_THREADS, smem, (cudaStream_t)stream>>>(*g, N, start, (const int2 *)ti, xyb, feat_s, *p_host, do_conv, min_idx,
-                                                                flags, nbr, off, cellmask, xa, wl_hdr, wl_ids, 0);
+        kern<<<cells, BL_THREADS, smem, st>>>(*g, N, start, (const int2 *)ti, xyb, feat_s, *p_host, wfrag, do_conv, min_idx, flags, nbr,
+                                              off, cellmask, xa, wl_hdr, wl_ids, 0);
     }
     DAGR_CHECK_LAUNCH();
     if (deferring) {
@@ -605,11 +698,48 @@
             DAGR_CUDA(cudaGetDevice(&dev));
             DAGR_CUDA(cudaDeviceGetAttribute(&n_sm, cudaDevAttrMultiProcessorCount, dev));
         }
-        DAGR_CUDA(dagr_allow_smem(k_l1_build_dense, smem_big));
-        k_l1_build_dense<<<n_sm, BL_THREADS_BIG, smem_big, (cudaStream_t)stream>>>(*g, N, start, (const int2 *)ti, xyb, feat_s,
-                                                                                    *p_host, do_conv, min_idx, flags, nbr, off,
-                                                                                    cellmask, xa, wl_hdr, wl_ids);
+        auto kd = k_l1_build_dense<TC>;
+        DAGR_CUDA(dagr_allow_smem(kd, smem_big));
+        kd<<<n_sm, BL_THREADS_BIG, smem_big, st>>>(*g, N, start, (const int2 *)ti, xyb, feat_s, *p_host, wfrag, do_conv, min_idx, flags,
+                                                   nbr, off, cellmask, xa, wl_hdr, wl_ids);
         DAGR_CHECK_LAUNCH();
     }
     return DAGR_OK;
 }
+
+extern "C" int dagr_l1_build(const dagr_geom_t *g, int64_t N, const int32_t *start, const int32_t *ti,
+                             const uint32_t *xyb, const float *feat_s, const float *tab,
+                             const dagr_l1a_params_t *p_host, const int32_t *flags, int min_idx, int32_t *nbr, uint16_t *off,
+                             uint32_t *cellmask, float *xa, int32_t *wl_hdr, int32_t *wl_ids, int defer, void *stream)
+{
+    (void)tab;
+    return l1_build_launch<false>(g, N, start, ti, xyb, feat_s, p_host, nullptr, flags, min_idx, nbr, off, cellmask, xa, wl_hdr,
+                                  wl_ids, defer, (cudaStream_t)stream);
+}
+
+extern "C" int dagr_l1_build_tc(const dagr_geom_t *g, int64_t N, const int32_t *start, const int32_t *ti,
+                                const uint32_t *xyb, const float *feat_s, const dagr_l1a_params_t *p_host, const float *wfrag,
+                                const int32_t *flags, int min_idx, int32_t *nbr, uint16_t *off, uint32_t *cellmask, float *xa,
+                                int32_t *wl_hdr, int32_t *wl_ids, int defer, void *stream)
+{
+    DAGR_CHECK_ARG(p_host && wfrag, "null params / weight fragments (dagr_l1a_tc_weights); the adjacency-only form is "
+                                    "dagr_l1_build with p_host = NULL");
+    return l1_build_launch<true>(g, N, start, ti, xyb, feat_s, p_host, (const float4 *)wfrag, flags, min_idx, nbr, off, cellmask, xa,
+                                 wl_hdr, wl_ids, defer, (cudaStream_t)stream);
+}
+
+extern "C" int dagr_l1a_tc_weights(const dagr_l1a_params_t *p_host, float *wfrag_host)
+{
+    DAGR_CHECK_ARG(p_host && wfrag_host, "null argument");
+    auto B = [&](int k, int n) { return k < 3 * DAGR_KU ? p_host->w[k / 3][k % 3][n] : p_host->root[k - 3 * DAGR_KU][n]; };
+    for (int s = 0; s < BL_TC_KSTEPS; s++)
+        for (int lane = 0; lane < 32; lane++)
+            for (int nt = 0; nt < 2; nt++) {
+                const int gq = lane >> 2, t = lane & 3, n = 8 * nt + gq;
+                const float x0 = B(8 * s + t, n), x1 = B(8 * s + t + 4, n);
+                const float h0 = tf32_rna_host(x0), h1 = tf32_rna_host(x1);
+                float *o = wfrag_host + (((size_t)s * 32 + lane) * 2 + nt) * 4;
+                o[0] = h0; o[1] = h1; o[2] = x0 - h0; o[3] = x1 - h1;
+            }
+    return DAGR_OK;
+}
diff --git a/dagr_b200/csrc/common.cuh b/dagr_b200/csrc/common.cuh
--- a/dagr_b200/csrc/common.cuh
+++ b/dagr_b200/csrc/common.cuh
@@ -2,6 +2,7 @@
 #include <cuda_runtime.h>
 #include <stdint.h>
 #include <stdio.h>
+#include <string.h>
 #include "../../include/dagr_b200.h"
 
 #ifndef __CUDA_ARCH__
@@ -57,6 +58,42 @@
 
 __device__ __forceinline__ float2 ffma2(float2 a, float2 b, float2 c) { return make_float2(fmaf(a.x, b.x, c.x), fmaf(a.y, b.y, c.y)); }
 
+__device__ __forceinline__ void tf32_split(uint32_t x, uint32_t &hi, uint32_t &lo)
+{
+    hi = (x + 0x1000u) & 0xffffe000u;
+    lo = __float_as_uint(__uint_as_float(x) - __uint_as_float(hi));
+}
+__device__ __forceinline__ void mma_tf32(float2 &c01, float2 &c23, const uint32_t a[4], uint32_t b0, uint32_t b1)
+{
+    asm("mma.sync.aligned.m16n8k8.row.col.f32.tf32.tf32.f32 {%0, %1, %2, %3}, {%4, %5, %6, %7}, {%8, %9}, {%0, %1, %2, %3};"
+        : "+f"(c01.x), "+f"(c01.y), "+f"(c23.x), "+f"(c23.y)
+        : "r"(a[0]), "r"(a[1]), "r"(a[2]), "r"(a[3]), "r"(b0), "r"(b1));
+}
+__device__ __forceinline__ void mma_3xtf32(float2 &c01, float2 &c23, const uint32_t ah[4], const uint32_t al[4], const float4 b)
+{
+    mma_tf32(c01, c23, al, __float_as_uint(b.x), __float_as_uint(b.y));
+    mma_tf32(c01, c23, ah, __float_as_uint(b.z), __float_as_uint(b.w));
+    mma_tf32(c01, c23, ah, __float_as_uint(b.x), __float_as_uint(b.y));
+}
+__device__ __forceinline__ void ldsm_x2(uint32_t saddr, uint32_t &r0, uint32_t &r1)
+{
+    asm volatile("ldmatrix.sync.aligned.m8n8.x2.shared.b16 {%0, %1}, [%2];" : "=r"(r0), "=r"(r1) : "r"(saddr) : "memory");
+}
+__device__ __forceinline__ void ldsm_x4(uint32_t saddr, uint32_t r[4])
+{
+    asm volatile("ldmatrix.sync.aligned.m8n8.x4.shared.b16 {%0, %1, %2, %3}, [%4];"
+                 : "=r"(r[0]), "=r"(r[1]), "=r"(r[2]), "=r"(r[3]) : "r"(saddr) : "memory");
+}
+static inline float tf32_rna_host(float x)
+{
+    uint32_t u;
+    memcpy(&u, &x, 4);
+    if ((u & 0x7f800000u) != 0x7f800000u) u = (u + 0x1000u) & 0xffffe000u;
+    float r;
+    memcpy(&r, &u, 4);
+    return r;
+}
+
 __device__ __forceinline__ void spline_basis2(float ax, float ay, int ks, float w[4], int slot[4])
 {
     float vx = ax * (float)(ks - 1), vy = ay * (float)(ks - 1);
diff --git a/dagr_b200/csrc/conv_l1.cu b/dagr_b200/csrc/conv_l1.cu
--- a/dagr_b200/csrc/conv_l1.cu
+++ b/dagr_b200/csrc/conv_l1.cu
@@ -315,19 +315,6 @@
 #endif
 #define CB2_TC_KSTEPS 16
 
-__device__ __forceinline__ uint32_t tf32_rna(float x)
-{
-    uint32_t r;
-    asm("cvt.rna.tf32.f32 %0, %1;" : "=r"(r) : "f"(x));
-    return r;
-}
-__device__ __forceinline__ void mma_tf32(float2 &c01, float2 &c23, const uint32_t a[4], uint32_t b0, uint32_t b1)
-{
-    asm("mma.sync.aligned.m16n8k8.row.col.f32.tf32.tf32.f32 {%0, %1, %2, %3}, {%4, %5, %6, %7}, {%8, %9}, {%0, %1, %2, %3};"
-        : "+f"(c01.x), "+f"(c01.y), "+f"(c23.x), "+f"(c23.y)
-        : "r"(a[0]), "r"(a[1]), "r"(a[2]), "r"(a[3]), "r"(b0), "r"(b1));
-}
-
 __device__ __forceinline__ void cb2_tc_kstep(float *xt, const float a[8], const float4 *__restrict__ wf, float2 o2[8])
 {
     const int lane = threadIdx.x & 31;
@@ -345,11 +332,9 @@
             if ((lane >> 4) == mt) *reinterpret_cast<float4 *>(row) = make_float4(a[4 * h], a[4 * h + 1], a[4 * h + 2], a[4 * h + 3]);
             __syncwarp();
             uint32_t r0, r1;
-            asm volatile("ldmatrix.sync.aligned.m8n8.x2.shared.b16 {%0, %1}, [%2];" : "=r"(r0), "=r"(r1) : "r"(ra) : "memory");
-            ah[2 * h] = tf32_rna(__uint_as_float(r0));
-            ah[2 * h + 1] = tf32_rna(__uint_as_float(r1));
-            al[2 * h] = __float_as_uint(__uint_as_float(r0) - __uint_as_float(ah[2 * h]));
-            al[2 * h + 1] = __float_as_uint(__uint_as_float(r1) - __uint_as_float(ah[2 * h + 1]));
+            ldsm_x2(ra, r0, r1);
+            tf32_split(r0, ah[2 * h], al[2 * h]);
+            tf32_split(r1, ah[2 * h + 1], al[2 * h + 1]);
         }
         const uint32_t fa[4] = {ah[0], ah[1], ah[2], ah[3]}, fl[4] = {al[0], al[1], al[2], al[3]};
 #pragma unroll
@@ -1006,16 +991,6 @@
                                                                   (cudaStream_t)stream);
 }
 
-static float tf32_rna_host(float x)
-{
-    uint32_t u;
-    memcpy(&u, &x, 4);
-    if ((u & 0x7f800000u) != 0x7f800000u) u = (u + 0x1000u) & 0xffffe000u;
-    float r;
-    memcpy(&r, &u, 4);
-    return r;
-}
-
 extern "C" int dagr_l1_tc_weights(const float *w_host, const float *root_host, int cin, float *wfrag_host)
 {
     DAGR_CHECK_ARG(w_host && root_host && wfrag_host, "null argument");
diff --git a/dagr_b200/engine.py b/dagr_b200/engine.py
--- a/dagr_b200/engine.py
+++ b/dagr_b200/engine.py
@@ -21,6 +21,12 @@
     out = (C.c_float * _lib.L1_TC_WFRAG_FLOATS)()
     _lib.check(lib.dagr_l1_tc_weights(C.cast(params.w, C.c_void_p), C.cast(params.root, C.c_void_p), cin, C.cast(out, C.c_void_p)),
                "dagr_l1_tc_weights")
+    return torch.frombuffer(out, dtype=torch.float32).clone().to(device)
+
+
+def _l1a_tc_weights(lib, params, device) -> torch.Tensor:
+    out = (C.c_float * _lib.L1A_TC_WFRAG_FLOATS)()
+    _lib.check(lib.dagr_l1a_tc_weights(C.byref(params), C.cast(out, C.c_void_p)), "dagr_l1a_tc_weights")
     return torch.frombuffer(out, dtype=torch.float32).clone().to(device)
 
 
@@ -124,7 +130,7 @@
         self._done = [None, None]
         self._out_slot = {}
 
-    _NKERNELS = dict(dagr_graph_sort=6, dagr_graph_sort_ring=6, dagr_stream_push=2, dagr_graph_sort_rings=6, dagr_stream_push_multi=2, dagr_graph_search=1, dagr_l1_build=2, dagr_graph_export=5, dagr_l1_conv_a=1, dagr_l1_conv_b_pool=1, dagr_l1_conv_b_pool_voxel=2, dagr_l1_conv_b_pool_voxel_tc=2, dagr_l1_x0_image=1, dagr_l1_x0_image_live=1, dagr_xa_permute=1, dagr_l1_conv_a_image=2, dagr_l1_conv_a_image_tc=2, dagr_voxel_sample_max=1,
+    _NKERNELS = dict(dagr_graph_sort=6, dagr_graph_sort_ring=6, dagr_stream_push=2, dagr_graph_sort_rings=6, dagr_stream_push_multi=2, dagr_graph_search=1, dagr_l1_build=2, dagr_l1_build_tc=2, dagr_graph_export=5, dagr_l1_conv_a=1, dagr_l1_conv_b_pool=1, dagr_l1_conv_b_pool_voxel=2, dagr_l1_conv_b_pool_voxel_tc=2, dagr_l1_x0_image=1, dagr_l1_x0_image_live=1, dagr_xa_permute=1, dagr_l1_conv_a_image=2, dagr_l1_conv_a_image_tc=2, dagr_voxel_sample_max=1,
                      dagr_l1_conv_a_image_inc=2, dagr_voxel_sample_max_inc=1,
                      dagr_l1_x0_image_planes=1, dagr_voxel_sample_max_planes=1, dagr_sample_features_planes=1, dagr_head_finish_planes=1,
                      dagr_pool1_finalize=1, dagr_grid_cat_pos=1, dagr_grid_conv=1, dagr_grid_linear_bn=1, dagr_grid_pool=1,
@@ -216,6 +222,7 @@
             pa.relu = 1
             _fill(pb.skip, cb.lin.mlp.weight.detach().cpu().t())
             pk["l1a"] = pa
+            pk["l1a_wfrag"] = _l1a_tc_weights(self.lib, pa, device)
         else:
             order = list(range(1, 17)) + [0, 17, 18]
             pi = _lib.L1ImgParams()
@@ -229,6 +236,7 @@
             _fill(pe.scale, torch.ones(16)); _fill(pe.shift, torch.zeros(16))
             pe.relu = 0
             pk["l1a_img"] = pe
+            pk["l1a_img_wfrag"] = _l1a_tc_weights(self.lib, pe, device)
             s, b = _fold_bn(ca.norm); _fill(pi.scale, s); _fill(pi.shift, b)
             s, b = _fold_bn(cb.norm_skip); _fill(pi.sscale, s); _fill(pi.sshift, b)
             pi.relu = 1
@@ -531,8 +539,8 @@
             if stream_state is not None and min_idx > 0:
                 self._run("xa_gather", lib.dagr_xa_permute, N, _lib.ptr(ws["perm"]), min_idx, _lib.ptr(ws["xa"]),
                           _lib.ptr(stream_state.xa_arr), 0, st)
-            self._run("l1_build", lib.dagr_l1_build, g, N, _lib.ptr(ws["start"]), _lib.ptr(ws["ti"]), _lib.ptr(ws["xyb"]),
-                      _lib.ptr(ws["feat_s"]), _lib.ptr(geom.d_tab1), C.byref(pk["l1a_img"]), _lib.ptr(flags), min_idx, _lib.ptr(nbr), _lib.ptr(off),
+            self._run("l1_build", lib.dagr_l1_build_tc, g, N, _lib.ptr(ws["start"]), _lib.ptr(ws["ti"]), _lib.ptr(ws["xyb"]),
+                      _lib.ptr(ws["feat_s"]), C.byref(pk["l1a_img"]), _lib.ptr(pk["l1a_img_wfrag"]), _lib.ptr(flags), min_idx, _lib.ptr(nbr), _lib.ptr(off),
                       _lib.ptr(cellmask), _lib.ptr(ws["xa"]), _lib.ptr(wl_hdr), _lib.ptr(self._zs(ws, "wl_build", torch.int32)), defer[0], st)
             if image_event is not None:
                 torch.cuda.current_stream().wait_event(image_event[0])
@@ -565,8 +573,8 @@
             if min_idx > 0:
                 self._run("xa_gather", lib.dagr_xa_permute, N, _lib.ptr(ws["perm"]), min_idx, _lib.ptr(ws["xa"]),
                           _lib.ptr(stream_state.xa_arr), 0, st)
-            self._run("l1_build", lib.dagr_l1_build, g, N, _lib.ptr(ws["start"]), _lib.ptr(ws["ti"]), _lib.ptr(ws["xyb"]),
-                      _lib.ptr(ws["feat_s"]), _lib.ptr(geom.d_tab1), C.byref(pk["l1a"]), _lib.ptr(flags), min_idx, _lib.ptr(nbr),
+            self._run("l1_build", lib.dagr_l1_build_tc, g, N, _lib.ptr(ws["start"]), _lib.ptr(ws["ti"]), _lib.ptr(ws["xyb"]),
+                      _lib.ptr(ws["feat_s"]), C.byref(pk["l1a"]), _lib.ptr(pk["l1a_wfrag"]), _lib.ptr(flags), min_idx, _lib.ptr(nbr),
                       _lib.ptr(off), _lib.ptr(cellmask), _lib.ptr(ws["xa"]), _lib.ptr(wl_hdr), _lib.ptr(self._zs(ws, "wl_build", torch.int32)),
                       defer[0], st)
             if stream_state is not None:
diff --git a/include/dagr_b200.h b/include/dagr_b200.h
--- a/include/dagr_b200.h
+++ b/include/dagr_b200.h
@@ -150,6 +150,13 @@
                    const int32_t *nbr, const uint16_t *off, const float *tab,
                    const dagr_l1a_params_t *p_host, float *xa , void *stream);
 
+#define DAGR_L1A_TC_WFRAG_FLOATS 1536
+int dagr_l1a_tc_weights(const dagr_l1a_params_t *p_host, float *wfrag_host );
+int dagr_l1_build_tc(const dagr_geom_t *g, int64_t N, const int32_t *start, const int32_t *ti,
+                     const uint32_t *xyb, const float *feat_s, const dagr_l1a_params_t *p_host, const float *wfrag,
+                     const int32_t *flags, int min_idx, int32_t *nbr, uint16_t *off, uint32_t *cellmask, float *xa,
+                     int32_t *wl_hdr, int32_t *wl_ids, int defer, void *stream);
+
 int dagr_l1_conv_b_pool(const dagr_geom_t *g, int64_t N, const uint32_t *xyb, const float *feat_s,
                         const float *xa, const int32_t *nbr, const uint16_t *off, const float *tab,
                         const dagr_l1b_params_t *p_host, float *x1, uint32_t *poolmax, void *stream);
```

After: 579.4, median of 6. 5.3% higher.
